# realtimeradio/caltech-bifrost-dsp

Hardware: AMD Instinct MI355X
Metric: xengine_ingest_gbps_704in_96ch (higher is better)
Workload: dtype int8 (4+4-bit samples) -> int32

## Files before the change

caltech-bifrost-dsp_amd/csrc/ring.hip:

```cpp
#include <time.h>

#include <atomic>
#include <chrono>
#include <condition_variable>
#include <deque>
#include <map>
#include <memory>
#include <mutex>
#include <string>
#include <vector>

#include "xeng_common.h"

namespace xeng {

struct RingCore;

struct Buf {
    std::atomic<long> refs{1};
    void* ptr = nullptr;
    size_t nbytes = 0;
    int space = XENG_SPACE_SYSTEM;
    int dev = -1;
    bool owned = true;
    RingCore* ring = nullptr;
    Stamp stamp;
    unsigned long long hook_stamp[2] = {0, 0};
};

struct Chunk {
    uint64_t offset;
    size_t nbytes;
    Buf* buf;
    size_t boff;
};

struct Seq {
    long long index = 0, time_tag = 0;
    int nringlet = 1;
    std::string header;
    std::deque<Chunk> chunks;
    uint64_t committed = 0;
    bool ended = false;
};

struct Reader {
    bool open = false, guarantee = true, in_seq = false;
    long long seq_index = 0;
    uint64_t offset = 0;
};

struct RingCore {
    std::atomic<long> refs{1};
    std::mutex mu;
    std::condition_variable cv;
    std::string name;
    int space = XENG_SPACE_SYSTEM;
    std::deque<std::unique_ptr<Seq>> seqs;
    long long seq_base = 0;
    long long nseq = 0;
    Seq* open_seq = nullptr;
    bool writing_ended = false, destroyed = false;
    std::vector<Reader> readers;
    size_t capacity = 0, live_bytes = 0;
    std::mutex pool_mu;
    std::map<size_t, std::deque<Buf*>> pool;
    std::vector<Buf*> graveyard;
    size_t pool_bytes = 0;
    xengRingStampNowFn hook_now = nullptr;
    xengRingStampDoneFn hook_done = nullptr;
    xengRingStampWaitFn hook_wait = nullptr;
    void* hook_user = nullptr;
    bool recycle_system = false;
    unsigned stream_mask = 0;
    std::atomic<unsigned> declared{0}, users{0};
    bool writer_seen = false;
    std::atomic<size_t> owned_bytes{0};
    std::atomic<unsigned long long> n_alloc{0}, n_free{0}, n_reuse{0}, n_stamp_wait{0}, n_skipped{0};
};

static void ring_unref(RingCore* r) {
    if (r->refs.fetch_sub(1) == 1) delete r;
}

static size_t own_limit(const RingCore* r, size_t nbytes) { return 8 * std::max(r->capacity, 2 * nbytes); }

static bool pooled_space(const RingCore* r) { return r->space != XENG_SPACE_SYSTEM || r->hook_now || r->recycle_system; }

static int raw_alloc(int space, size_t nbytes, void** out) {
    const size_t n = nbytes ? nbytes : 1;
    if (space == XENG_SPACE_SYSTEM) {
        void* p = nullptr;
        if (posix_memalign(&p, 64, (n + 63) & ~(size_t)63) != 0 || !p) XENG_FAIL(XENG_STATUS_MEM_ALLOC_FAILED, "ring: out of host memory (%zu bytes)", n);
        memset(p, 0, n);
        *out = p;
        return XENG_STATUS_SUCCESS;
    }
    int rc = xengMalloc(out, n, space);
    if (rc) return rc;
    rc = xengMemset(*out, 0, n);
    if (rc) { (void)xengFree(*out, space); *out = nullptr; }
    return rc;
}

static void raw_free(int space, void* p) {
    if (!p) return;
    if (space == XENG_SPACE_SYSTEM) free(p);
    else (void)xengFree(p, space);
}

static unsigned effective_mask(const RingCore* r) {
    const unsigned m = r->stream_mask;
    if (!m || r->declared.load() < r->users.load()) return (unsigned)STAMP_ALL;
    return m;
}

static void buf_stamp(Buf* b) {
    RingCore* r = b->ring;
    if (r->hook_now) r->hook_now(r->hook_user, b->hook_stamp);
    else if (b->space != XENG_SPACE_SYSTEM) {
        (void)stamp_now(&b->stamp, b->ptr, effective_mask(r), b->dev);
    }
}

static void buf_poll(Buf* b, bool* done, bool* waitable) {
    RingCore* r = b->ring;
    *done = true;
    *waitable = true;
    if (r->hook_done) {
        *done = r->hook_done(r->hook_user, b->hook_stamp) != 0;
        return;
    }
    if (b->space == XENG_SPACE_SYSTEM) return;
    if (stamp_poll(b->stamp, done, waitable) != XENG_STATUS_SUCCESS) { *done = false; *waitable = false; }
}

static int buf_wait(Buf* b) {
    RingCore* r = b->ring;
    r->n_stamp_wait++;
    if (r->hook_wait) { r->hook_wait(r->hook_user, b->hook_stamp); return XENG_STATUS_SUCCESS; }
    if (b->space == XENG_SPACE_SYSTEM) return XENG_STATUS_SUCCESS;
    return stamp_wait(b->stamp);
}

static void buf_destroy(Buf* b, bool may_wait) {
    RingCore* r = b->ring;
    if (b->owned && b->ptr) {
        bool done = true, waitable = true;
        buf_poll(b, &done, &waitable);
        if (!done && may_wait && waitable) done = buf_wait(b) == XENG_STATUS_SUCCESS;
        if (done) {
            raw_free(b->space, b->ptr);
            r->n_free++;
        }
        r->owned_bytes -= b->nbytes;
    }
    delete b;
    ring_unref(r);
}

static void buf_release(Buf* b) {
    if (b->refs.fetch_sub(1) != 1) return;
    RingCore* r = b->ring;
    if (!b->owned) { delete b; ring_unref(r); return; }
    if (!pooled_space(r)) { raw_free(b->space, b->ptr); r->n_free++; r->owned_bytes -= b->nbytes; delete b; ring_unref(r); return; }
    buf_stamp(b);
    {
        std::lock_guard<std::mutex> lk(r->pool_mu);
        if (!r->destroyed) {
            if (r->owned_bytes.load() > own_limit(r, b->nbytes)) {
                r->graveyard.push_back(b);
            } else {
                r->pool[b->nbytes].push_back(b);
                r->pool_bytes += b->nbytes;
            }
            return;
        }
    }
    buf_destroy(b, true);
}

static void bury(RingCore* r) {
    std::vector<Buf*> dead;
    {
        std::lock_guard<std::mutex> lk(r->pool_mu);
        dead.swap(r->graveyard);
    }
    for (Buf* b : dead) buf_destroy(b, true);
}

static int buf_obtain(RingCore* r, size_t nbytes, int may_block, Buf** out) {
    *out = nullptr;
    if (pooled_space(r)) {
        Buf* cand = nullptr;
        {
            std::lock_guard<std::mutex> lk(r->pool_mu);
            auto it = r->pool.find(nbytes);
            if (it != r->pool.end() && !it->second.empty()) {
                cand = it->second.front();
                it->second.pop_front();
                r->pool_bytes -= nbytes;
            }
        }
        if (cand) {
            bool done, waitable;
            buf_poll(cand, &done, &waitable);
            const bool grow = !done && r->owned_bytes.load() + nbytes <= own_limit(r, nbytes) && !r->hook_now;
            if (!done && waitable && may_block && !grow) done = buf_wait(cand) == XENG_STATUS_SUCCESS;
            if (done) {
                *out = cand;
            } else {
                std::lock_guard<std::mutex> lk(r->pool_mu);
                if (waitable) r->pool[nbytes].push_front(cand);
                else r->pool[nbytes].push_back(cand);
                r->pool_bytes += nbytes;
                if (waitable && !may_block && !grow) return XENG_STATUS_WOULD_BLOCK;
            }
        }
        if (*out) {
            (*out)->refs.store(1);
            r->n_reuse++;
            return XENG_STATUS_SUCCESS;
        }
    }
    if (!may_block && (r->space != XENG_SPACE_SYSTEM || nbytes > (1u << 20))) return XENG_STATUS_WOULD_BLOCK;
    void* p = nullptr;
    int rc = raw_alloc(r->space, nbytes, &p);
    if (rc) return rc;
    Buf* b = new Buf();
    b->ptr = p; b->nbytes = nbytes; b->space = r->space; b->ring = r;
    if (r->space != XENG_SPACE_SYSTEM && hipGetDevice(&b->dev) != hipSuccess) { (void)hipGetLastError(); b->dev = -1; }
    r->refs.fetch_add(1);
    r->n_alloc++;
    r->owned_bytes += nbytes;
    *out = b;
    return XENG_STATUS_SUCCESS;
}

static Seq* seq_at(RingCore* r, long long index) {
    if (index < r->seq_base || index >= r->seq_base + (long long)r->seqs.size()) return nullptr;
    return r->seqs[(size_t)(index - r->seq_base)].get();
}

static void drop_chunk(RingCore* r, Seq* s, std::vector<Buf*>* released) {
    Chunk c = s->chunks.front();
    s->chunks.pop_front();
    r->live_bytes -= c.nbytes;
    released->push_back(c.buf);
}

static void gc(RingCore* r, std::vector<Buf*>* released) {
    bool any = false;
    long long lo_seq = 0;
    uint64_t lo_off = 0;
    for (const Reader& rd : r->readers) {
        if (!rd.open) continue;
        if (!any || rd.seq_index < lo_seq || (rd.seq_index == lo_seq && rd.offset < lo_off)) { lo_seq = rd.seq_index; lo_off = rd.offset; }
        any = true;
    }
    if (!any) return;
    while (!r->seqs.empty() && r->seq_base < lo_seq) {
        Seq* s = r->seqs.front().get();
        while (!s->chunks.empty()) drop_chunk(r, s, released);
        if (s == r->open_seq) break;
        r->seqs.pop_front();
        r->seq_base++;
    }
    if (Seq* s = seq_at(r, lo_seq))
        while (!s->chunks.empty() && s->chunks.front().offset + s->chunks.front().nbytes <= lo_off) drop_chunk(r, s, released);
}

static bool drop_oldest(RingCore* r, std::vector<Buf*>* released) {
    for (auto& sp : r->seqs)
        if (!sp->chunks.empty()) { drop_chunk(r, sp.get(), released); return true; }
    r->live_bytes = 0;
    return false;
}

static void release_all(std::vector<Buf*>& v) {
    for (Buf* b : v) buf_release(b);
    v.clear();
}

static int wait_for_room(RingCore* r, std::unique_lock<std::mutex>& lk, size_t nbytes, int nonblocking, int may_block) {
    if (r->capacity == 0) r->capacity = 4 * nbytes;
    std::vector<Buf*> released;
    for (;;) {
        const size_t cap = std::max(r->capacity, nbytes);
        if (r->live_bytes + nbytes <= cap) break;
        gc(r, &released);
        if (r->live_bytes + nbytes <= cap) break;
        bool guaranteed = false;
        for (const Reader& rd : r->readers) guaranteed |= rd.open && rd.guarantee;
        if (!guaranteed) {
            if (!drop_oldest(r, &released)) break;
            continue;
        }
        if (nonblocking || !may_block || r->destroyed) {
            lk.unlock(); release_all(released); lk.lock();
            if (r->destroyed) XENG_FAIL(XENG_STATUS_INVALID_STATE, "ring '%s' was destroyed", r->name.c_str());
            if (nonblocking) XENG_FAIL(XENG_STATUS_WOULD_BLOCK, "ring '%s' full", r->name.c_str());
            return XENG_STATUS_WOULD_BLOCK;
        }
        if (!released.empty()) { lk.unlock(); release_all(released); lk.lock(); continue; }
        r->cv.wait_for(lk, std::chrono::milliseconds(100));
    }
    if (!released.empty()) { lk.unlock(); release_all(released); lk.lock(); }
    return XENG_STATUS_SUCCESS;
}

static int copy_bytes(int space, void* dst, const void* src, size_t n) {
    if (space == XENG_SPACE_SYSTEM) { memcpy(dst, src, n); return XENG_STATUS_SUCCESS; }
    return xengMemcpy(dst, src, n);
}

}

using namespace xeng;

#define RING_ARG(r_) \
    RingCore* r = (RingCore*)(r_); \
    if (!r) XENG_FAIL(XENG_STATUS_INVALID_ARGUMENT, "ring: null handle")

extern "C" {

int xengRingCreate(xengRing** ring, const char* name, int space) {
    if (!ring) XENG_FAIL(XENG_STATUS_INVALID_ARGUMENT, "RingCreate: null handle pointer");
    if (space != XENG_SPACE_SYSTEM && space != XENG_SPACE_CUDA && space != XENG_SPACE_CUDA_HOST)
        XENG_FAIL(XENG_STATUS_INVALID_ARGUMENT, "RingCreate: unknown space %d", space);
    RingCore* r = new RingCore();
    r->name = name ? name : "";
    r->space = space;
    *ring = (xengRing*)r;
    return XENG_STATUS_SUCCESS;
}

int xengRingDestroy(xengRing* ring) {
    RING_ARG(ring);
    std::vector<Buf*> released;
    {
        std::unique_lock<std::mutex> lk(r->mu);
        if (r->destroyed) return XENG_STATUS_SUCCESS;
        r->destroyed = true;
        r->writing_ended = true;
        for (auto& sp : r->seqs) {
            sp->ended = true;
            while (!sp->chunks.empty()) drop_chunk(r, sp.get(), &released);
        }
        r->open_seq = nullptr;
        r->cv.notify_all();
    }
    release_all(released);
    std::vector<Buf*> dead;
    {
        std::lock_guard<std::mutex> lk(r->pool_mu);
        for (auto& kv : r->pool)
            for (Buf* b : kv.second) dead.push_back(b);
        r->pool.clear();
        r->pool_bytes = 0;
        for (Buf* b : r->graveyard) dead.push_back(b);
        r->graveyard.clear();
    }
    for (Buf* b : dead) buf_destroy(b, true);
    ring_unref(r);
    return XENG_STATUS_SUCCESS;
}

int xengRingSetStampHooks(xengRing* ring, xengRingStampNowFn now, xengRingStampDoneFn done, xengRingStampWaitFn wait, void* user) {
    RING_ARG(ring);
    std::lock_guard<std::mutex> lk(r->pool_mu);
    r->hook_now = now; r->hook_done = done; r->hook_wait = wait; r->hook_user = user;
    return XENG_STATUS_SUCCESS;
}

int xengRingDeclareStreams(xengRing* ring, unsigned classes) {
    RING_ARG(ring);
    std::lock_guard<std::mutex> lk(r->pool_mu);
    r->stream_mask |= classes & (STAMP_ALL | STAMP_XGPU_OUT);
    r->declared.fetch_add(1);
    return XENG_STATUS_SUCCESS;
}

int xengRingGetStampClasses(xengRing* ring, unsigned* classes, unsigned* declared, unsigned* users) {
    RING_ARG(ring);
    if (classes) *classes = effective_mask(r);
    if (declared) *declared = r->declared.load();
    if (users) *users = r->users.load();
    return XENG_STATUS_SUCCESS;
}

int xengRingSetRecycle(xengRing* ring, int on) {
    RING_ARG(ring);
    std::lock_guard<std::mutex> lk(r->pool_mu);
    r->recycle_system = on != 0;
    return XENG_STATUS_SUCCESS;
}

int xengRingResize(xengRing* ring, size_t contig_bytes, size_t total_span) {
    RING_ARG(ring);
    const size_t want = total_span ? total_span : 4 * contig_bytes;
    std::lock_guard<std::mutex> lk(r->mu);
    r->capacity = std::max(r->capacity, std::max(want, contig_bytes));
    return XENG_STATUS_SUCCESS;
}

int xengRingGetInfo(xengRing* ring, size_t* capacity, size_t* live_bytes, size_t* pool_bytes, int* nreaders, long long* nseq,
                    unsigned long long counters[5]) {
    RING_ARG(ring);
    {
        std::lock_guard<std::mutex> lk(r->mu);
        if (capacity) *capacity = r->capacity;
        if (live_bytes) *live_bytes = r->live_bytes;
        if (nreaders) {
            int n = 0;
            for (const Reader& rd : r->readers) n += rd.open;
            *nreaders = n;
        }
        if (nseq) *nseq = r->nseq;
    }
    if (pool_bytes) {
        std::lock_guard<std::mutex> lk(r->pool_mu);
        *pool_bytes = r->pool_bytes;
    }
    if (counters) {
        counters[0] = r->n_alloc; counters[1] = r->n_free; counters[2] = r->n_reuse; counters[3] = r->n_stamp_wait; counters[4] = r->n_skipped;
    }
    return XENG_STATUS_SUCCESS;
}

int xengRingBeginSequence(xengRing* ring, long long time_tag, const void* header, size_t header_len, int nringlet, long long* seq) {
    RING_ARG(ring);
    if (!seq) XENG_FAIL(XENG_STATUS_INVALID_ARGUMENT, "BeginSequence: null seq");
    std::lock_guard<std::mutex> lk(r->mu);
    if (r->destroyed) XENG_FAIL(XENG_STATUS_INVALID_STATE, "ring '%s' was destroyed", r->name.c_str());
    if (r->open_seq) r->open_seq->ended = true;
    if (!r->writer_seen) { r->writer_seen = true; r->users.fetch_add(1); }
    std::unique_ptr<Seq> s(new Seq());
    s->index = r->nseq++;
    s->time_tag = time_tag;
    s->nringlet = nringlet;
    if (header && header_len) s->header.assign((const char*)header, header_len);
    r->open_seq = s.get();
    *seq = s->index;
    if (r->seqs.empty()) r->seq_base = s->index;
    r->seqs.push_back(std::move(s));
    r->cv.notify_all();
    return XENG_STATUS_SUCCESS;
}

int xengRingEndSequence(xengRing* ring, long long seq) {
    RING_ARG(ring);
    std::lock_guard<std::mutex> lk(r->mu);
    if (Seq* s = seq_at(r, seq)) {
        s->ended = true;
        if (r->open_seq == s) r->open_seq = nullptr;
    }
    r->cv.notify_all();
    return XENG_STATUS_SUCCESS;
}

int xengRingEndWriting(xengRing* ring) {
    RING_ARG(ring);
    std::lock_guard<std::mutex> lk(r->mu);
    if (r->open_seq) { r->open_seq->ended = true; r->open_seq = nullptr; }
    r->writing_ended = true;
    r->cv.notify_all();
    return XENG_STATUS_SUCCESS;
}

int xengRingReserve(xengRing* ring, long long seq, size_t nbytes, int nonblocking, int may_block, void** data, long long* span) {
    RING_ARG(ring);
    if (!data || !span) XENG_FAIL(XENG_STATUS_INVALID_ARGUMENT, "Reserve: null output");
    if (may_block) bury(r);
    {
        std::unique_lock<std::mutex> lk(r->mu);
        Seq* s = seq < 0 ? r->open_seq : seq_at(r, seq);
        if (!s || s->ended) XENG_FAIL(XENG_STATUS_INVALID_STATE, "WriteSpan: no open sequence on ring '%s'", r->name.c_str());
        int rc = wait_for_room(r, lk, nbytes, nonblocking, may_block);
        if (rc) return rc;
    }
    Buf* b = nullptr;
    int rc = buf_obtain(r, nbytes, may_block, &b);
    if (rc) return rc;
    *data = b->ptr;
    *span = (long long)(intptr_t)b;
    return XENG_STATUS_SUCCESS;
}

int xengRingCommit(xengRing* ring, long long seq, long long span, size_t nbytes) {
    RING_ARG(ring);
    Buf* b = (Buf*)(intptr_t)span;
    if (!b || b->ring != r) XENG_FAIL(XENG_STATUS_INVALID_ARGUMENT, "Commit: not a span of ring '%s'", r->name.c_str());
    if (nbytes > b->nbytes) XENG_FAIL(XENG_STATUS_INVALID_ARGUMENT, "Commit: %zu bytes of a %zu-byte span", nbytes, b->nbytes);
    if (nbytes == 0) return XENG_STATUS_SUCCESS;
    std::lock_guard<std::mutex> lk(r->mu);
    Seq* s = seq < 0 ? r->open_seq : seq_at(r, seq);
    if (!s) return XENG_STATUS_SUCCESS;
    b->refs.fetch_add(1);
    s->chunks.push_back(Chunk{s->committed, nbytes, b, 0});
    s->committed += nbytes;
    r->live_bytes += nbytes;
    r->cv.notify_all();
    return XENG_STATUS_SUCCESS;
}

int xengRingCommitExternal(xengRing* ring, long long seq, void* data, size_t nbytes, int may_block) {
    RING_ARG(ring);
    if (!data || nbytes == 0) XENG_FAIL(XENG_STATUS_INVALID_ARGUMENT, "CommitExternal: empty span");
    std::unique_lock<std::mutex> lk(r->mu);
    Seq* s = seq < 0 ? r->open_seq : seq_at(r, seq);
    if (!s || s->ended) XENG_FAIL(XENG_STATUS_INVALID_STATE, "commit_external: no open sequence on ring '%s'", r->name.c_str());
    int rc = wait_for_room(r, lk, nbytes, 0, may_block);
    if (rc) return rc;
    s = seq < 0 ? r->open_seq : seq_at(r, seq);
    if (!s) XENG_FAIL(XENG_STATUS_INVALID_STATE, "commit_external: the sequence is gone (ring '%s')", r->name.c_str());
    Buf* b = new Buf();
    b->ptr = data; b->nbytes = nbytes; b->space = r->space; b->owned = false; b->ring = r;
    r->refs.fetch_add(1);
    s->chunks.push_back(Chunk{s->committed, nbytes, b, 0});
    s->committed += nbytes;
    r->live_bytes += nbytes;
    r->cv.notify_all();
    return XENG_STATUS_SUCCESS;
}

int xengRingOpenReader(xengRing* ring, int guarantee, int* reader) {
    RING_ARG(ring);
    if (!reader) XENG_FAIL(XENG_STATUS_INVALID_ARGUMENT, "OpenReader: null reader");
    std::lock_guard<std::mutex> lk(r->mu);
    size_t k = 0;
    while (k < r->readers.size() && r->readers[k].open) k++;
    if (k == r->readers.size()) r->readers.emplace_back();
    Reader& rd = r->readers[k];
    rd = Reader();
    rd.open = true;
    r->users.fetch_add(1);
    rd.guarantee = guarantee != 0;
    rd.seq_index = r->nseq;
    for (auto& sp : r->seqs)
        if (!sp->chunks.empty() || !sp->ended) { rd.seq_index = sp->index; break; }
    *reader = (int)k;
    return XENG_STATUS_SUCCESS;
}

int xengRingCloseReader(xengRing* ring, int reader) {
    RING_ARG(ring);
    std::vector<Buf*> released;
    {
        std::lock_guard<std::mutex> lk(r->mu);
        if (reader < 0 || reader >= (int)r->readers.size()) XENG_FAIL(XENG_STATUS_INVALID_ARGUMENT, "CloseReader: bad reader %d", reader);
        r->readers[reader].open = false;
        gc(r, &released);
        r->cv.notify_all();
    }
    release_all(released);
    return XENG_STATUS_SUCCESS;
}

int xengRingNextSequence(xengRing* ring, int reader, int may_block, long long* seq, long long* time_tag, int* nringlet,
                         const void** header, size_t* header_len) {
    RING_ARG(ring);
    std::vector<Buf*> released;
    int rc = XENG_STATUS_SUCCESS;
    {
        std::unique_lock<std::mutex> lk(r->mu);
        if (reader < 0 || reader >= (int)r->readers.size() || !r->readers[reader].open)
            XENG_FAIL(XENG_STATUS_INVALID_ARGUMENT, "NextSequence: bad reader %d", reader);
        Reader* rd = &r->readers[reader];
        if (rd->in_seq) {
            rd->in_seq = false;
            rd->seq_index++;
            rd->offset = 0;
            gc(r, &released);
            r->cv.notify_all();
        }
        for (;;) {
            rd = &r->readers[reader];
            if (rd->seq_index < r->seq_base) rd->seq_index = r->seq_base;
            if (rd->seq_index < r->nseq) break;
            if (r->writing_ended || r->destroyed) { rc = XENG_STATUS_END_OF_DATA; break; }
            if (!may_block) { rc = XENG_STATUS_WOULD_BLOCK; break; }
            r->cv.wait_for(lk, std::chrono::milliseconds(100));
        }
        if (rc == XENG_STATUS_SUCCESS) {
            Seq* s = seq_at(r, rd->seq_index);
            rd->in_seq = true;
            rd->offset = 0;
            if (seq) *seq = s->index;
            if (time_tag) *time_tag = s->time_tag;
            if (nringlet) *nringlet = s->nringlet;
            if (header) *header = s->header.data();
            if (header_len) *header_len = s->header.size();
        }
    }
    release_all(released);
    return rc;
}

static int acquire_common(xengRing* ring, int reader, size_t advance, size_t gulp_nbytes, int may_block, int max_parts, void** data,
                          size_t* nbytes, long long* span, int* nparts, size_t* skipped) {
    RING_ARG(ring);
    if (!data || !nbytes || !span || gulp_nbytes == 0) XENG_FAIL(XENG_STATUS_INVALID_ARGUMENT, "Acquire: bad argument");
    std::vector<Buf*> released;
    std::vector<Chunk> pieces;
    int rc = XENG_STATUS_SUCCESS;
    size_t n = 0, skip_total = 0;
    {
        std::unique_lock<std::mutex> lk(r->mu);
        if (reader < 0 || reader >= (int)r->readers.size() || !r->readers[reader].open || !r->readers[reader].in_seq)
            XENG_FAIL(XENG_STATUS_INVALID_ARGUMENT, "Acquire: reader %d has no open sequence", reader);
        if (advance) {
            r->readers[reader].offset += advance;
            gc(r, &released);
            r->cv.notify_all();
        }
        for (;;) {
            Reader& rd = r->readers[reader];
            Seq* s = seq_at(r, rd.seq_index);
            if (!s) { rc = XENG_STATUS_END_OF_DATA; break; }
            const uint64_t lo = s->chunks.empty() ? s->committed : s->chunks.front().offset;
            if (rd.offset < lo) {
                const uint64_t sk = ((lo - rd.offset + gulp_nbytes - 1) / gulp_nbytes) * gulp_nbytes;
                rd.offset += sk;
                skip_total += sk;
                r->n_skipped += sk;
            }
            const uint64_t avail = s->committed > rd.offset ? s->committed - rd.offset : 0;
            if (avail >= gulp_nbytes || s->ended || r->destroyed) {
                n = (size_t)std::min<uint64_t>(avail, gulp_nbytes);
                if (n == 0) { rc = XENG_STATUS_END_OF_DATA; break; }
                for (const Chunk& c : s->chunks) {
                    if (c.offset >= rd.offset + n) break;
                    const uint64_t a = std::max<uint64_t>(rd.offset, c.offset), b = std::min<uint64_t>(rd.offset + n, c.offset + c.nbytes);
                    if (a < b) {
                        c.buf->refs.fetch_add(1);
                        pieces.push_back(Chunk{a, (size_t)(b - a), c.buf, c.boff + (size_t)(a - c.offset)});
                    }
                }
                break;
            }
            if (!may_block) { rc = XENG_STATUS_WOULD_BLOCK; break; }
            r->cv.wait_for(lk, std::chrono::milliseconds(100));
        }
    }
    release_all(released);
    if (skipped) *skipped = skip_total;
    if (rc) return rc;
    if ((int)pieces.size() <= max_parts) {
        for (size_t k = 0; k < pieces.size(); k++) {
            data[k] = (uint8_t*)pieces[k].buf->ptr + pieces[k].boff;
            nbytes[k] = pieces[k].nbytes;
            span[k] = (long long)(intptr_t)pieces[k].buf;
        }
        if (nparts) *nparts = (int)pieces.size();
        return XENG_STATUS_SUCCESS;
    }
    if (!may_block) {
        for (Chunk& c : pieces) buf_release(c.buf);
        return XENG_STATUS_WOULD_BLOCK;
    }
    *nbytes = n;
    if (nparts) *nparts = 1;
    Buf* g = nullptr;
    rc = buf_obtain(r, n, 1, &g);
    size_t pos = 0;
    for (Chunk& c : pieces) {
        if (!rc) rc = copy_bytes(r->space, (uint8_t*)g->ptr + pos, (const uint8_t*)c.buf->ptr + c.boff, c.nbytes);
        pos += c.nbytes;
        buf_release(c.buf);
    }
    if (rc) { if (g) buf_release(g); return rc; }
    *data = g->ptr;
    *span = (long long)(intptr_t)g;
    return XENG_STATUS_SUCCESS;
}

int xengRingAcquire(xengRing* ring, int reader, size_t advance, size_t gulp_nbytes, int may_block, void** data, size_t* nbytes,
                    long long* span, size_t* skipped) {
    return acquire_common(ring, reader, advance, gulp_nbytes, may_block, 1, data, nbytes, span, nullptr, skipped);
}

int xengRingAcquireParts(xengRing* ring, int reader, size_t advance, size_t gulp_nbytes, int may_block, void* data[2], size_t nbytes[2],
                         long long span[2], int* nparts, size_t* skipped) {
    if (!nparts) XENG_FAIL(XENG_STATUS_INVALID_ARGUMENT, "AcquireParts: null nparts");
    return acquire_common(ring, reader, advance, gulp_nbytes, may_block, 2, data, nbytes, span, nparts, skipped);
}

int xengRingSpanRelease(long long span) {
    Buf* b = (Buf*)(intptr_t)span;
    if (!b) XENG_FAIL(XENG_STATUS_INVALID_ARGUMENT, "SpanRelease: null span");
    buf_release(b);
    return XENG_STATUS_SUCCESS;
}

}
```

caltech-bifrost-dsp_amd/csrc/xcorr.hip:

```cpp
#include <algorithm>
#include <cstdlib>
#include <map>
#include <mutex>
#include <vector>

#include "xcorr_kernels.h"
#include "slab.h"
#include "xeng_common.h"

namespace xeng {

struct XgpuConfig {
    int nstand = 352, npol = 2, nchan = 96, ntime_gulp = 480, max_gulps = 0;
};

struct XgpuContext {
    bool live = false;
    int gpu = 0;
    XgpuConfig cfg;
    int ncu = 256;
    int ninput = 0, nblk64 = 0, gkt = 0, cap_kt = 0, cap_gulps = 0, kt_stage = 1;
    int ct_pitch = 0;
    bool raw = false;
    bool kloop16 = false;
    FragGroup* fgroups_dev = nullptr;
    int nfg = 0;
    WorkList work;
    WorkList work_pairs;
    size_t gulp_bytes = 0;
    const uint8_t* gulp_ptr[XC_MAX_GULPS] = {};
    int64_t per_chan = 0, matlen = 0;
    uint8_t* stash[2] = {nullptr, nullptr};
    size_t stash_bytes = 0;
    int cur = 0;
    WgDesc* descs_dev = nullptr;
    int nwg = 0;
    hipStream_t stream = nullptr;
    static constexpr int NMM = 8;
    hipStream_t stream_mm2[NMM] = {};
    int nmm = 2;
    unsigned long long nlaunch = 0;
    hipStream_t stream_mm = nullptr;
    struct Writer { unsigned long long seq; int stream; };
    std::map<const void*, Writer> writers;
    static constexpr int NEV = 256;
    hipEvent_t ev_ring[NEV] = {};
    const void* ring_buf[NEV][2] = {};
    unsigned long long last_seq[NMM] = {};
    hipEvent_t ev_ct = nullptr;
    unsigned long long staging_seen = ~0ull;
    unsigned long long area_seq[2] = {0, 0};
    unsigned long long dump_seq[4] = {0, 0, 0, 0};
    unsigned long long ndump = 0;
    int nfilled = 0;
    bool acc_started = false;
    void* acc_out = nullptr;
    uint8_t* in_dev = nullptr;
    int32_t* out_dev = nullptr;
    unsigned long long* stamps = nullptr;
    GulpDesc* gdesc_dev[2] = {nullptr, nullptr};
    SlabArgs* gargs_dev[2] = {nullptr, nullptr};
    SlabSite slab_site;
    SlabIndexSite slab_index;
    SlabIndexJob slab_job;
    int slab_forced = 0;
    int slab_hint_seen = 0;
    int slab_recent_irr[8] = {}, slab_recent_n[8] = {}, slab_recent_pos = 0;
    unsigned long long slab_tables_until = 0;
    int slab_force_tables = -1;
    bool slab_mode = false;
    EventTimer timer;
};

static std::mutex g_mu;
static XgpuConfig g_cfg;
static XgpuContext g_ctx;
static unsigned long long g_epoch = 1;
static unsigned long long g_ctx_gen = 1;

static int destroy_locked() {
    XgpuContext& x = g_ctx;
    (void)hipSetDevice(x.gpu);
    if (x.stream) (void)hipStreamSynchronize(x.stream);
    for (int b = 0; b < XgpuContext::NMM; b++) {
        if (x.stream_mm2[b]) (void)hipStreamSynchronize(x.stream_mm2[b]);
    }
    for (int k = 0; k < XgpuContext::NEV; k++)
        if (x.ev_ring[k]) (void)hipEventDestroy(x.ev_ring[k]);
    for (int b = 0; b < 2; b++)
        if (x.stash[b]) (void)hipFree(x.stash[b]);
    if (x.ev_ct) (void)hipEventDestroy(x.ev_ct);
    if (x.descs_dev) (void)hipFree(x.descs_dev);
    if (x.fgroups_dev) (void)hipFree(x.fgroups_dev);
    if (x.work.dev) (void)hipFree(x.work.dev);
    if (x.work_pairs.dev) (void)hipFree(x.work_pairs.dev);
    if (x.in_dev) (void)hipFree(x.in_dev);
    if (x.stamps) (void)hipFree(x.stamps);
    if (x.out_dev) (void)hipFree(x.out_dev);
    for (int b = 0; b < 2; b++)
        if (x.gdesc_dev[b]) (void)hipFree(x.gdesc_dev[b]);
    for (int b = 0; b < 2; b++)
        if (x.gargs_dev[b]) (void)hipFree(x.gargs_dev[b]);
    slab_site_destroy(&x.slab_site);
    slab_index_site_destroy(&x.slab_index);
    x.timer.destroy();
    x = XgpuContext();
    g_epoch++;
    g_ctx_gen++;
    return XENG_STATUS_SUCCESS;
}

static void launch_xcorr(const XcorrParams& p, hipStream_t s, bool raw, int grid_size, bool kloop16) {
    if (raw) {
        const dim3 grid(grid_size);
        if (kloop16 && !p.acc2_mode && !(p.gdesc && p.by_table)) {
            if (p.gdesc) hipLaunchKernelGGL(HIP_KERNEL_NAME(xcorr_fused16_kernel<true>), grid, dim3(512), 0, s, p);
            else hipLaunchKernelGGL(HIP_KERNEL_NAME(xcorr_fused16_kernel<>), grid, dim3(512), 0, s, p);
            return;
        }
        if (p.gdesc && p.by_table) {
            if (p.acc2_mode) hipLaunchKernelGGL(HIP_KERNEL_NAME(xcorr_fused_kernel<true, true, true>), grid, dim3(256), 0, s, p);
            else hipLaunchKernelGGL(HIP_KERNEL_NAME(xcorr_fused_kernel<false, true, true>), grid, dim3(256), 0, s, p);
            return;
        }
        if (p.gdesc) {
            if (p.acc2_mode) hipLaunchKernelGGL(HIP_KERNEL_NAME(xcorr_fused_kernel<true, true>), grid, dim3(256), 0, s, p);
            else hipLaunchKernelGGL(HIP_KERNEL_NAME(xcorr_fused_kernel<false, true>), grid, dim3(256), 0, s, p);
            return;
        }
        if (p.acc2_mode) hipLaunchKernelGGL(HIP_KERNEL_NAME(xcorr_fused_kernel<true>), grid, dim3(256), 0, s, p);
        else hipLaunchKernelGGL(HIP_KERNEL_NAME(xcorr_fused_kernel<>), grid, dim3(256), 0, s, p);
        return;
    }
    hipLaunchKernelGGL(xcorr_mfma_kernel, dim3(p.nchan * p.nwg), dim3(256), 0, s, p);
}

static hipEvent_t launch_event(unsigned long long seq) {
    XgpuContext& x = g_ctx;
    if (seq == 0 || x.nlaunch - seq >= (unsigned long long)XgpuContext::NEV) return nullptr;
    return x.ev_ring[seq % XgpuContext::NEV];
}

static int order_after_writer(hipStream_t s, int self, const void* buf) {
    XgpuContext& x = g_ctx;
    auto it = x.writers.find(buf);
    if (it == x.writers.end() || it->second.stream == self) return XENG_STATUS_SUCCESS;
    if (hipEvent_t ev = launch_event(it->second.seq)) XENG_HIP(hipStreamWaitEvent(s, ev, 0));
    return XENG_STATUS_SUCCESS;
}

static int flush_locked(void* out, bool dump, void* acc = nullptr, int acc_mode = 0) {
    XgpuContext& x = g_ctx;
    if (x.nfilled == 0) return XENG_STATUS_SUCCESS;
    if (!dump) { acc = nullptr; acc_mode = 0; }
    if (x.acc_started && x.acc_out != out)
        XENG_FAIL(XENG_STATUS_INVALID_STATE,
                  "xgpu: output buffer changed inside one integration (partial sums live in %p, got %p)",
                  x.acc_out, out);
    int nkt = x.nfilled * x.gkt;
    const int rem = x.raw ? 0 : nkt % x.kt_stage;
    if (rem) {
        const int padk = x.kt_stage - rem;
        XENG_HIP(hipMemset2DAsync(x.stash[x.cur] + (size_t)nkt * KT_BYTES, (size_t)x.cap_kt * KT_BYTES, 0,
                                  (size_t)padk * KT_BYTES, (size_t)x.cfg.nchan * x.nblk64, x.stream));
        stream_tick(STREAM_XGPU);
        nkt += padk;
    }
    const bool slab_tables = x.slab_mode && x.slab_index.tab32 != nullptr;
    bool slab_by_table = false;
    if (slab_tables) {
        x.slab_job.ngulp = x.nfilled;
        {
            const int seen = *(volatile int*)x.slab_index.hint_host;
            x.slab_recent_irr[x.slab_recent_pos] = seen - x.slab_hint_seen;
            x.slab_recent_n[x.slab_recent_pos] = x.nfilled;
            x.slab_recent_pos = (x.slab_recent_pos + 1) & 7;
            x.slab_hint_seen = seen;
            int irr = 0, n = 0;
            for (int k = 0; k < 8; k++) { irr += x.slab_recent_irr[k]; n += x.slab_recent_n[k]; }
            if (4 * irr > n) x.slab_tables_until = x.nlaunch + 16;
            slab_by_table = x.slab_force_tables > 0 || (x.slab_force_tables < 0 && x.nlaunch < x.slab_tables_until);
        }
        if (int rcs = slab_index_enqueue(x.stream, x.slab_index, x.cur, x.slab_job, slab_by_table, x.gdesc_dev[x.cur], x.gargs_dev[x.cur])) return rcs;
        staging_stream_touched();
    } else if (x.slab_mode) {
        if (int rcs = slab_fallback_enqueue(x.stream, x.gdesc_dev[x.cur], x.gargs_dev[x.cur], x.nfilled)) return rcs;
        staging_stream_touched();
    }
    XcorrParams p;
    p.stash = x.stash[x.cur]; p.out = (int32_t*)out; p.descs = x.descs_dev;
    p.nwg = x.raw ? x.nfg : x.nwg; p.nchan = x.cfg.nchan; p.nblk64 = x.nblk64; p.cap_kt = x.cap_kt; p.nkt = nkt;
    p.nstand = x.cfg.nstand; p.per_chan = x.per_chan; p.matlen = x.matlen;
    p.accumulate = x.acc_started ? 1 : 0;
    p.stamps = x.stamps;
    p.spg = x.raw ? x.cfg.ntime_gulp / (XC_KT * 32) : 0;
    p.ninput = x.ninput;
    p.fgroups = x.fgroups_dev; p.work = x.work.dev; p.maxi = x.work.maxi; p.nstage = nkt / XC_KT;
    p.acc2 = (int32_t*)acc; p.acc2_mode = acc ? acc_mode : 0;
    p.gdesc = slab_tables ? x.gdesc_dev[x.cur] : nullptr;
    p.by_table = slab_by_table ? 1 : 0;
    if (slab_tables && !diag_env("XENG_SLAB_PLAIN_ORDER")) { p.work = x.work_pairs.dev; p.maxi = x.work_pairs.maxi; }
    for (int g = 0; g < XC_MAX_GULPS; g++) p.gulps[g] = g < x.nfilled ? x.gulp_ptr[g] : nullptr;
    const int si = (int)(x.nlaunch++ % x.nmm);
    hipStream_t smm = x.stream_mm2[si];
    if (const unsigned long long ops = staging_stream_ops(); ops != x.staging_seen) {
        XENG_HIP(hipEventRecord(x.ev_ct, x.stream));
        XENG_HIP(hipStreamWaitEvent(smm, x.ev_ct, 0));
        x.staging_seen = ops;
    }
    const unsigned long long seq = x.nlaunch;
    {
        const int k = (int)(seq % XgpuContext::NEV);
        if (seq > (unsigned long long)XgpuContext::NEV) {
            if (hipEventQuery(x.ev_ring[k]) != hipSuccess) {
                (void)hipGetLastError();
                XENG_HIP(hipEventSynchronize(x.ev_ring[k]));
            }
            for (const void* buf : x.ring_buf[k]) {
                auto it = buf ? x.writers.find(buf) : x.writers.end();
                if (it != x.writers.end() && it->second.seq == seq - XgpuContext::NEV) x.writers.erase(it);
            }
        }
        x.ring_buf[k][0] = out; x.ring_buf[k][1] = acc;
    }
    for (const void* buf : {(const void*)out, (const void*)acc}) {
        if (!buf) continue;
        int rc = order_after_writer(smm, si, buf);
        if (rc) return rc;
        x.writers[buf] = XgpuContext::Writer{seq, si};
    }
    int slot = x.timer.begin(smm, 1);
    launch_xcorr(p, smm, x.raw, fused_grid(x.cfg.nchan, x.nfg, x.ncu), x.kloop16);
    x.timer.end(smm, slot);
    XENG_HIP(hipGetLastError());
    XENG_HIP(hipEventRecord(x.ev_ring[seq % XgpuContext::NEV], smm));
    x.area_seq[x.cur] = seq;
    x.last_seq[si] = seq;
    if (dump) {
        x.dump_seq[x.ndump & 3] = seq;
        x.ndump++;
    }
    x.cur ^= 1;
    x.nfilled = 0;
    x.slab_mode = false;
    x.acc_started = !dump;
    x.acc_out = dump ? nullptr : out;
    return XENG_STATUS_SUCCESS;
}

struct PendingWait {
    int gpu = 0;
    hipStream_t staging = nullptr;
    hipEvent_t dump = nullptr;
};

static int wait_unlocked(const PendingWait& w) {
    XENG_HIP(hipSetDevice(w.gpu));
    if (w.staging) XENG_HIP(hipStreamSynchronize(w.staging));
    if (w.dump) XENG_HIP(hipEventSynchronize(w.dump));
    return XENG_STATUS_SUCCESS;
}

static int kernel_locked(const void* in_dev, void* out_dev, int doDump, bool sync, PendingWait* pw, void* acc = nullptr,
                         int acc_mode = 0) {
    XgpuContext& x = g_ctx;
    if (!x.live) XENG_FAIL(XENG_STATUS_INVALID_STATE, "xgpu: not initialized (call xengXgpuInitialize)");
    if (!in_dev || !out_dev) XENG_FAIL(XENG_STATUS_INVALID_ARGUMENT, "xgpu: null buffer");
    if (acc) {
        if (!x.raw)
            XENG_FAIL(XENG_STATUS_UNSUPPORTED, "xgpu: the fused long accumulation needs the default contraction kernel (use xengMapAddI32)");
        if (acc_mode != 1 && acc_mode != 2) XENG_FAIL(XENG_STATUS_INVALID_ARGUMENT, "xgpu: acc_mode must be 1 (assign) or 2 (add)");
        if (((uintptr_t)acc & 15) || acc == out_dev) XENG_FAIL(XENG_STATUS_INVALID_ARGUMENT, "xgpu: accumulator must be 16-byte aligned and distinct from out");
    }
    if (((uintptr_t)out_dev & 15) || ((uintptr_t)in_dev & (x.raw ? 15 : 3)))
        XENG_FAIL(XENG_STATUS_INVALID_ARGUMENT, "xgpu: out must be 16-byte and in %d-byte aligned", x.raw ? 16 : 4);
    XENG_HIP(hipSetDevice(x.gpu));
    if (x.nfilled > 0 && x.slab_mode)
        XENG_FAIL(XENG_STATUS_INVALID_STATE, "xgpu: packet slabs and plain gulps cannot be mixed between two flushes");
    if (x.nfilled == 0)
        if (hipEvent_t ev = launch_event(x.area_seq[x.cur])) XENG_HIP(hipStreamWaitEvent(x.stream, ev, 0));
    uint8_t* const stash = x.stash[x.cur];
    int slot = -1;
    if (x.raw) {
        if (sync && !doDump) {
            uint8_t* copy = stash + (size_t)x.nfilled * x.gulp_bytes;
            slot = x.timer.begin(x.stream, 0);
            if (x.gulp_bytes % 16 == 0) {
                const size_t n16 = x.gulp_bytes / 16;
                const unsigned blocks = (unsigned)std::min<size_t>(2048, (n16 + 1023) / 1024);
                hipLaunchKernelGGL(HIP_KERNEL_NAME(gulp_copy_kernel<4>), dim3(blocks), dim3(256), 0, x.stream, (v4i*)copy, (const v4i*)in_dev, n16);
                XENG_HIP(hipGetLastError());
            } else {
                XENG_HIP(hipMemcpyAsync(copy, in_dev, x.gulp_bytes, hipMemcpyDeviceToDevice, x.stream));
            }
            x.gulp_ptr[x.nfilled] = copy;
        } else {
            x.gulp_ptr[x.nfilled] = (const uint8_t*)in_dev;
        }
    } else if (x.ct_pitch > 0) {
        slot = x.timer.begin(x.stream, 0);
        const size_t l8 = (((size_t)16 * x.ct_pitch + 1023) & ~(size_t)1023);
        hipLaunchKernelGGL(corner_turn_tr8_kernel, dim3(x.cfg.nchan, x.gkt, 2), dim3(256), l8, x.stream,
                           (const uint8_t*)in_dev, stash, x.cfg.ntime_gulp, x.cfg.nchan, x.ninput, x.nblk64,
                           x.cap_kt, x.nfilled * x.gkt, x.ct_pitch);
    } else {
        slot = x.timer.begin(x.stream, 0);
        const int ct_items = 2 * x.nblk64 * 16;
        const int ct_threads = std::min(1024, ((ct_items + 63) / 64) * 64);
        hipLaunchKernelGGL(corner_turn_kernel, dim3(x.gkt, x.cfg.nchan), dim3(ct_threads), 0, x.stream,
                           (const uint8_t*)in_dev, stash, x.cfg.ntime_gulp, x.cfg.nchan, x.ninput, x.nblk64,
                           x.cap_kt, x.nfilled * x.gkt);
    }
    x.timer.end(x.stream, slot);
    XENG_HIP(hipGetLastError());
    if (!x.raw || (sync && !doDump)) staging_stream_touched();
    x.nfilled++;
    if (doDump || x.nfilled == x.cap_gulps) {
        int rc = flush_locked(out_dev, doDump != 0, acc, acc_mode);
        if (rc) return rc;
    } else if (x.acc_started && x.acc_out != out_dev) {
        XENG_FAIL(XENG_STATUS_INVALID_STATE, "xgpu: output buffer changed inside one integration");
    }
    if (sync && pw) {
        pw->gpu = x.gpu;
        pw->staging = x.stream;
        if (doDump) pw->dump = launch_event(x.dump_seq[(x.ndump - 1) & 3]);
    }
    return XENG_STATUS_SUCCESS;
}

void xgpu_pending_launch(unsigned long long* seq, unsigned long long* epoch, unsigned long long* nlaunch, unsigned long long* ctx) {
    std::lock_guard<std::mutex> lk(g_mu);
    XgpuContext& x = g_ctx;
    *seq = (x.live && x.nfilled > 0) ? x.nlaunch + 1 : 0;
    *epoch = g_epoch;
    *nlaunch = x.live ? x.nlaunch : 0;
    *ctx = g_ctx_gen;
}

unsigned long long xgpu_last_writer(const void* buf) {
    std::lock_guard<std::mutex> lk(g_mu);
    XgpuContext& x = g_ctx;
    if (!x.live || !buf) return 0;
    auto it = x.writers.find(buf);
    return it == x.writers.end() ? 0 : it->second.seq;
}

int xgpu_launches_poll(unsigned long long upto, unsigned long long ctx, bool* done, hipEvent_t* ev, bool exact) {
    std::lock_guard<std::mutex> lk(g_mu);
    XgpuContext& x = g_ctx;
    *done = true;
    if (ev) *ev = nullptr;
    if (upto == 0 || !x.live || ctx != g_ctx_gen) return XENG_STATUS_SUCCESS;
    for (int k = 0; k < (exact ? 1 : x.nmm) && (unsigned long long)k < upto; k++) {
        if (hipEvent_t e = launch_event(upto - k)) {
            const hipError_t q = hipEventQuery(e);
            if (q == hipErrorNotReady) {
                (void)hipGetLastError();
                *done = false;
                if (ev && !*ev) *ev = e;
            } else if (q != hipSuccess) {
                XENG_HIP(q);
            }
        }
    }
    return XENG_STATUS_SUCCESS;
}

int xgpu_pending_poll(unsigned long long seq, unsigned long long epoch, bool* done, bool* launched, hipEvent_t* ev, int* gpu) {
    std::lock_guard<std::mutex> lk(g_mu);
    XgpuContext& x = g_ctx;
    *done = true;
    *launched = true;
    if (ev) *ev = nullptr;
    if (seq == 0 || !x.live || epoch != g_epoch) return XENG_STATUS_SUCCESS;
    if (x.nlaunch < seq) {
        *done = false;
        *launched = false;
        return XENG_STATUS_SUCCESS;
    }
    if (hipEvent_t e = launch_event(seq)) {
        const hipError_t q = hipEventQuery(e);
        if (q == hipErrorNotReady) {
            (void)hipGetLastError();
            *done = false;
            if (ev) *ev = e;
            if (gpu) *gpu = x.gpu;
        } else if (q != hipSuccess) {
            XENG_HIP(q);
        }
    }
    return XENG_STATUS_SUCCESS;
}

}

using namespace xeng;

extern "C" {

int xengXgpuConfigure(int nstand, int npol, int nchan, int ntime_gulp, int max_gulps_per_flush) {
    if (npol != 2) XENG_FAIL(XENG_STATUS_UNSUPPORTED, "xgpu: npol must be 2 (got %d)", npol);
    if (nstand <= 0 || nstand % 4) XENG_FAIL(XENG_STATUS_INVALID_ARGUMENT, "xgpu: nstand must be a positive multiple of 4 (got %d)", nstand);
    if (nstand * npol > 255 * 64) XENG_FAIL(XENG_STATUS_UNSUPPORTED, "xgpu: too many inputs (%d)", nstand * npol);
    if (nchan <= 0 || ntime_gulp <= 0 || max_gulps_per_flush < 0)
        XENG_FAIL(XENG_STATUS_INVALID_ARGUMENT, "xgpu: bad sizes nchan=%d ntime_gulp=%d max_gulps=%d", nchan, ntime_gulp, max_gulps_per_flush);
    std::lock_guard<std::mutex> lk(g_mu);
    g_cfg.nstand = nstand; g_cfg.npol = npol; g_cfg.nchan = nchan; g_cfg.ntime_gulp = ntime_gulp;
    g_cfg.max_gulps = max_gulps_per_flush;
    return XENG_STATUS_SUCCESS;
}

static int initialize_locked(int gpu);

int xengXgpuInitialize(int gpu) {
    std::lock_guard<std::mutex> lk(g_mu);
    destroy_locked();
    const int rc = initialize_locked(gpu);
    if (rc) destroy_locked();
    return rc;
}

static int initialize_locked(int gpu) {
    XgpuContext& x = g_ctx;
    x.cfg = g_cfg;
    x.gpu = gpu < 0 ? 0 : gpu;
    XENG_HIP(hipSetDevice(x.gpu));
    {
        int ncu = 0;
        XENG_HIP(hipDeviceGetAttribute(&ncu, hipDeviceAttributeMultiprocessorCount, x.gpu));
        const char* e = diag_env("XENG_GRID");
        x.ncu = e ? atoi(e) : ncu;
        if (x.ncu < 1) x.ncu = 1;
    }
    x.ninput = x.cfg.nstand * x.cfg.npol;
    x.nblk64 = (x.ninput + 63) / 64;
    x.gkt = (x.cfg.ntime_gulp + 31) / 32;
    x.kt_stage = XC_KT;
    int cap = x.cfg.max_gulps > 0 ? x.cfg.max_gulps : std::max(1, 4800 / (x.gkt * 32));
    cap = std::min(cap, std::max(1, 65535 / (x.gkt * 32)));
    {
        const char* r = getenv("XENG_RAW");
        x.gulp_bytes = (size_t)x.cfg.ntime_gulp * x.cfg.nchan * x.ninput;
        x.raw = !(r && !strcmp(r, "0")) && x.ninput % 16 == 0 &&
                x.cfg.ntime_gulp % (XC_KT * 32) == 0 && x.gulp_bytes + (size_t)16 * x.cfg.nchan * x.ninput < (1ull << 32) &&
                (size_t)x.cfg.nchan * x.ninput >= 128;
        if (x.raw) cap = std::min(cap, XC_MAX_GULPS);
        const char* kl = getenv("XENG_KLOOP");
        x.kloop16 = x.raw && kl && !strcmp(kl, "16");
        const char* st = getenv("XENG_SLAB_TABLES");
        x.slab_force_tables = st ? (strcmp(st, "0") ? 1 : 0) : -1;
        x.slab_hint_seen = 0; x.slab_recent_pos = 0; x.slab_tables_until = 0;
        for (int k = 0; k < 8; k++) x.slab_recent_irr[k] = x.slab_recent_n[k] = 0;
    }
    x.cap_gulps = cap;
    x.cap_kt = ((cap * x.gkt + x.kt_stage - 1) / x.kt_stage) * x.kt_stage;
    x.per_chan = (int64_t)(x.cfg.nstand / 2 + 1) * (x.cfg.nstand / 4) * x.cfg.npol * x.cfg.npol * 4;
    x.matlen = x.per_chan * x.cfg.nchan;
    x.stash_bytes = (size_t)x.cfg.nchan * x.nblk64 * x.cap_kt * KT_BYTES;
    if (x.ninput % 16 == 0) {
        int pitch = x.ninput;
        while (((pitch / 4) & 63) != 8) pitch += 16;
        if ((size_t)16 * pitch + 1024 <= 64 * 1024) x.ct_pitch = pitch;
    }
    if (x.raw) x.stash_bytes = (size_t)cap * x.gulp_bytes;

    for (int b = 0; b < 2; b++) {
        XENG_HIP(hipMalloc((void**)&x.stash[b], x.stash_bytes));
        XENG_HIP(hip_memset_now(x.stash[b], 0, x.stash_bytes));
    }
    XENG_HIP(hipEventCreateWithFlags(&x.ev_ct, hipEventDisableTiming));
    if (x.raw) {
        for (int b = 0; b < 2; b++) {
            XENG_HIP(hipMalloc((void**)&x.gdesc_dev[b], XC_MAX_GULPS * sizeof(GulpDesc)));
            XENG_HIP(hip_memset_now(x.gdesc_dev[b], 0, XC_MAX_GULPS * sizeof(GulpDesc)));
            XENG_HIP(hipMalloc((void**)&x.gargs_dev[b], XC_MAX_GULPS * sizeof(SlabArgs)));
            XENG_HIP(hip_memset_now(x.gargs_dev[b], 0, XC_MAX_GULPS * sizeof(SlabArgs)));
        }
        if (int rcs = slab_site_create(&x.slab_site)) return rcs;
    }
    std::vector<WgDesc> descs = build_wg_descs(x.nblk64);
    x.nwg = (int)descs.size();
    if (x.raw) {
        const bool tiles64 = getenv("XENG_TILING") && !strcmp(getenv("XENG_TILING"), "64");
        const bool plain_order = diag_env("XENG_ITEM_ORDER") && !strcmp(diag_env("XENG_ITEM_ORDER"), "plain");
        const std::vector<FragGroup> groups = tiles64 ? frag_groups_from_tiles(x.nblk64) : build_frag_groups(x.nblk64);
        if (check_frag_groups(groups, x.nblk64) != -1) XENG_FAIL(XENG_STATUS_DEVICE_ERROR, "xgpu: the tiling of %d blocks is not an exact cover", x.nblk64);
        x.nfg = (int)groups.size();
        XENG_HIP(hipMalloc((void**)&x.fgroups_dev, groups.size() * sizeof(FragGroup)));
        XENG_HIP(hipMemcpy(x.fgroups_dev, groups.data(), groups.size() * sizeof(FragGroup), hipMemcpyHostToDevice));
        const std::vector<uint64_t> masks = group_block_masks(groups);
        x.work = build_work(fused_grid(x.cfg.nchan, x.nfg, x.ncu), x.cfg.nchan, x.nfg, plain_order ? nullptr : &masks);
        XENG_HIP(hipMalloc((void**)&x.work.dev, x.work.entries.size() * sizeof(WorkEntry)));
        XENG_HIP(hipMemcpy(x.work.dev, x.work.entries.data(), x.work.entries.size() * sizeof(WorkEntry), hipMemcpyHostToDevice));
        x.work_pairs = build_work(fused_grid(x.cfg.nchan, x.nfg, x.ncu), x.cfg.nchan, x.nfg, plain_order ? nullptr : &masks, true);
        XENG_HIP(hipMalloc((void**)&x.work_pairs.dev, x.work_pairs.entries.size() * sizeof(WorkEntry)));
        XENG_HIP(hipMemcpy(x.work_pairs.dev, x.work_pairs.entries.data(), x.work_pairs.entries.size() * sizeof(WorkEntry), hipMemcpyHostToDevice));
    }
    XENG_HIP(hipMalloc((void**)&x.descs_dev, descs.size() * sizeof(WgDesc)));
    XENG_HIP(hipMemcpy(x.descs_dev, descs.data(), descs.size() * sizeof(WgDesc), hipMemcpyHostToDevice));
    if (const char* o = diag_env("XENG_STREAM_ORDER")) {
        hipStream_t tmp;
        for (const char* c = o; *c; c++) {
            const StreamId id = *c == 'c' ? STREAM_COPY : *c == 'm' ? STREAM_MAP : *c == 'b' ? STREAM_BEAM : *c == 'k' ? STREAM_CONSUMER : STREAM_XGPU;
            int rc0 = get_stream(id, &tmp);
            if (rc0) return rc0;
        }
    }
    int rc = get_stream(STREAM_XGPU, &x.stream);
    if (rc) return rc;
    if (const char* e = diag_env("XENG_MM_STREAMS")) x.nmm = std::max(1, std::min(XgpuContext::NMM, atoi(e)));
    for (int t = 0; t < x.nmm; t++) {
        rc = get_stream(mm_stream_id(t), &x.stream_mm2[t]);
        if (rc) return rc;
    }
    for (int k = 0; k < XgpuContext::NEV; k++) XENG_HIP(hipEventCreateWithFlags(&x.ev_ring[k], hipEventDisableTiming));
    x.stream_mm = x.stream_mm2[0];
    if (diag_env("XENG_DBG_STAMPS")) {
        const int ng = std::max(x.nwg, x.nfg);
        XENG_HIP(hipMalloc((void**)&x.stamps, (size_t)x.cfg.nchan * ng * 4 * 8 * sizeof(unsigned long long)));
        XENG_HIP(hip_memset_now(x.stamps, 0, (size_t)x.cfg.nchan * ng * 4 * 8 * sizeof(unsigned long long)));
    }
    XENG_HIP(hipStreamSynchronize(nullptr));
    x.live = true;
    return XENG_STATUS_SUCCESS;
}

int xengXgpuDestroy(void) {
    std::lock_guard<std::mutex> lk(g_mu);
    return destroy_locked();
}

static void drain_timer() {
    std::lock_guard<std::mutex> lk(g_mu);
    if (g_ctx.live) g_ctx.timer.drain();
}

static int wait_for_event_slot(bool may_block = true) {
    for (;;) {
        hipEvent_t ev = nullptr;
        int gpu = 0;
        {
            std::lock_guard<std::mutex> lk(g_mu);
            XgpuContext& x = g_ctx;
            if (!x.live) return XENG_STATUS_SUCCESS;
            const unsigned long long next = x.nlaunch + 1;
            if (next <= (unsigned long long)XgpuContext::NEV) return XENG_STATUS_SUCCESS;
            ev = x.ev_ring[next % XgpuContext::NEV];
            gpu = x.gpu;
            if (hipEventQuery(ev) == hipSuccess) return XENG_STATUS_SUCCESS;
            (void)hipGetLastError();
        }
        if (!may_block) XENG_FAIL(XENG_STATUS_WOULD_BLOCK, "xgpu: %d launches in flight (xengXgpuWaitLaunchSlot, then retry)", XgpuContext::NEV);
        XENG_HIP(hipSetDevice(gpu));
        XENG_HIP(hipEventSynchronize(ev));
    }
}

int xengXgpuKernel(const void* in_dev, void* out_dev, int doDump) {
    PendingWait pw;
    int rc0 = wait_for_event_slot();
    if (rc0) return rc0;
    {
        std::lock_guard<std::mutex> lk(g_mu);
        int rc = kernel_locked(in_dev, out_dev, doDump, true, &pw);
        if (rc) return rc;
    }
    int rc = wait_unlocked(pw);
    if (rc) return rc;
    if (doDump) drain_timer();
    return XENG_STATUS_SUCCESS;
}

int xengXgpuKernelAsync(const void* in_dev, void* out_dev, int doDump) {
    int rc0 = wait_for_event_slot();
    if (rc0) return rc0;
    std::lock_guard<std::mutex> lk(g_mu);
    return kernel_locked(in_dev, out_dev, doDump, false, nullptr);
}

int xengXgpuKernelAsyncAcc(const void* in_dev, void* out_dev, int doDump, void* acc_dev, int acc_mode) {
    int rc0 = wait_for_event_slot();
    if (rc0) return rc0;
    std::lock_guard<std::mutex> lk(g_mu);
    return kernel_locked(in_dev, out_dev, doDump, false, nullptr, acc_dev, acc_dev ? acc_mode : 0);
}

int xengXgpuTryKernelAsyncAcc(const void* in_dev, void* out_dev, int doDump, void* acc_dev, int acc_mode) {
    int rc0 = wait_for_event_slot(false);
    if (rc0) return rc0;
    std::lock_guard<std::mutex> lk(g_mu);
    return kernel_locked(in_dev, out_dev, doDump, false, nullptr, acc_dev, acc_dev ? acc_mode : 0);
}

int xengXgpuWaitLaunchSlot(void) { return wait_for_event_slot(true); }

static int kernel_slab(const void* packets_dev, int npkt, size_t pkt_stride, uint64_t seq0, int chan0_pipeline, void* out_dev,
                       int doDump, void* acc_dev, int acc_mode, bool may_block) {
    int rc0 = wait_for_event_slot(may_block);
    if (rc0) return rc0;
    std::lock_guard<std::mutex> lk(g_mu);
    XgpuContext& x = g_ctx;
    if (!x.live) XENG_FAIL(XENG_STATUS_INVALID_STATE, "xgpu: not initialized (call xengXgpuInitialize)");
    if (!x.raw) XENG_FAIL(XENG_STATUS_UNSUPPORTED, "xgpu: packet slabs need the default contraction kernel (unpack with xengSnap2UnpackAsync instead)");
    if (!packets_dev || !out_dev || npkt < 0 || pkt_stride < 32 || pkt_stride > 0x7FFFFFFFu)
        XENG_FAIL(XENG_STATUS_INVALID_ARGUMENT, "xgpu: bad slab (npkt %d, stride %zu)", npkt, pkt_stride);
    if (acc_dev) {
        if (acc_mode != 1 && acc_mode != 2) XENG_FAIL(XENG_STATUS_INVALID_ARGUMENT, "xgpu: acc_mode must be 1 (assign) or 2 (add)");
        if (((uintptr_t)acc_dev & 15) || acc_dev == out_dev) XENG_FAIL(XENG_STATUS_INVALID_ARGUMENT, "xgpu: accumulator must be 16-byte aligned and distinct from out");
    }
    if ((uintptr_t)out_dev & 15) XENG_FAIL(XENG_STATUS_INVALID_ARGUMENT, "xgpu: out must be 16-byte aligned");
    if (x.nfilled > 0 && !x.slab_mode)
        XENG_FAIL(XENG_STATUS_INVALID_STATE, "xgpu: packet slabs and plain gulps cannot be mixed between two flushes");
    if (x.acc_started && x.acc_out != out_dev) XENG_FAIL(XENG_STATUS_INVALID_STATE, "xgpu: output buffer changed inside one integration");
    XENG_HIP(hipSetDevice(x.gpu));
    if (x.nfilled == 0)
        if (hipEvent_t ev = launch_event(x.area_seq[x.cur])) XENG_HIP(hipStreamWaitEvent(x.stream, ev, 0));
    const int k = x.nfilled;
    SlabArgs a;
    a.pkts = (const uint8_t*)packets_dev; a.npkt = npkt; a.stride = (uint32_t)pkt_stride; a.seq0 = seq0;
    a.ntime = x.cfg.ntime_gulp; a.chan0 = chan0_pipeline; a.nchan = x.cfg.nchan; a.ninput = x.ninput; a.nblk = x.ninput / 64;
    uint8_t* scratch = x.stash[x.cur] + (size_t)k * x.gulp_bytes;
    if (x.ninput % 64 == 0) {
        if (!x.slab_index.tab32)
            if (int rcs = slab_index_site_create(&x.slab_index, x.cfg.ntime_gulp, x.cfg.nchan, x.ninput)) return rcs;
        x.slab_job.a[k] = a; x.slab_job.scratch[k] = scratch; x.slab_job.force[k] = slab_indexable(a) ? 0 : 1;
        x.gulp_ptr[k] = nullptr;
    } else {
        const bool maybe = false;
        if (int rcs = slab_prepare_enqueue(x.stream, x.slab_site, &a, &maybe, 1, x.gdesc_dev[x.cur] + k, x.gargs_dev[x.cur] + k, &scratch, false)) return rcs;
        XENG_HIP(hipGetLastError());
        staging_stream_touched();
        x.slab_forced++;
        x.gulp_ptr[k] = scratch;
    }
    x.slab_mode = true;
    x.nfilled++;
    if (doDump || x.nfilled == x.cap_gulps) return flush_locked(out_dev, doDump != 0, acc_dev, acc_dev ? acc_mode : 0);
    return XENG_STATUS_SUCCESS;
}

int xengXgpuKernelAsyncSlab(const void* packets_dev, int npkt, size_t pkt_stride, uint64_t seq0, int chan0_pipeline, void* out_dev,
                            int doDump, void* acc_dev, int acc_mode) {
    return kernel_slab(packets_dev, npkt, pkt_stride, seq0, chan0_pipeline, out_dev, doDump, acc_dev, acc_mode, true);
}

int xengXgpuTryKernelAsyncSlab(const void* packets_dev, int npkt, size_t pkt_stride, uint64_t seq0, int chan0_pipeline, void* out_dev,
                               int doDump, void* acc_dev, int acc_mode) {
    return kernel_slab(packets_dev, npkt, pkt_stride, seq0, chan0_pipeline, out_dev, doDump, acc_dev, acc_mode, false);
}

static int slab_stats_locked(int* nscattered, int* nirregular) {
    XgpuContext& x = g_ctx;
    int ns = x.slab_forced, ni = 0;
    x.slab_forced = 0;
    if (x.slab_index.tab32) {
        XENG_HIP(hipSetDevice(x.gpu));
        stream_tick(STREAM_XGPU);
        int a = 0, b = 0;
        if (int rcs = slab_index_site_read(x.stream, x.slab_index, &a, &b)) return rcs;
        ns += a; ni += b;
    }
    if (nscattered) *nscattered = ns;
    if (nirregular) *nirregular = ni;
    return XENG_STATUS_SUCCESS;
}

int xengXgpuGetSlabFallbacks(int* nfallback) {
    std::lock_guard<std::mutex> lk(g_mu);
    XgpuContext& x = g_ctx;
    if (!x.live) XENG_FAIL(XENG_STATUS_INVALID_STATE, "xgpu: not initialized");
    if (!nfallback) XENG_FAIL(XENG_STATUS_INVALID_ARGUMENT, "GetSlabFallbacks: null pointer");
    *nfallback = 0;
    return slab_stats_locked(nfallback, nullptr);
}

int xengXgpuGetSlabStats(int* nscattered, int* nirregular) {
    std::lock_guard<std::mutex> lk(g_mu);
    XgpuContext& x = g_ctx;
    if (!x.live) XENG_FAIL(XENG_STATUS_INVALID_STATE, "xgpu: not initialized");
    if (!nscattered || !nirregular) XENG_FAIL(XENG_STATUS_INVALID_ARGUMENT, "GetSlabStats: null pointer");
    *nscattered = *nirregular = 0;
    return slab_stats_locked(nscattered, nirregular);
}

int xengXgpuSync(void) {
    int gpu, nmm;
    hipStream_t st, mm[XgpuContext::NMM];
    {
        std::lock_guard<std::mutex> lk(g_mu);
        XgpuContext& x = g_ctx;
        if (!x.live) XENG_FAIL(XENG_STATUS_INVALID_STATE, "xgpu: not initialized");
        gpu = x.gpu; nmm = x.nmm; st = x.stream;
        for (int t = 0; t < nmm; t++) mm[t] = x.stream_mm2[t];
    }
    XENG_HIP(hipSetDevice(gpu));
    XENG_HIP(hipStreamSynchronize(st));
    for (int t = 0; t < nmm; t++) XENG_HIP(hipStreamSynchronize(mm[t]));
    drain_timer();
    return XENG_STATUS_SUCCESS;
}

int xengXgpuSyncLag(int lag) {
    PendingWait pw;
    {
        std::lock_guard<std::mutex> lk(g_mu);
        XgpuContext& x = g_ctx;
        if (!x.live) XENG_FAIL(XENG_STATUS_INVALID_STATE, "xgpu: not initialized");
        if (lag < 0 || lag > 3) XENG_FAIL(XENG_STATUS_INVALID_ARGUMENT, "SyncLag: lag must be 0..3 (got %d)", lag);
        pw.gpu = x.gpu;
        if (x.ndump > (unsigned long long)lag) pw.dump = launch_event(x.dump_seq[(x.ndump - 1 - lag) & 3]);
    }
    int rc = wait_unlocked(pw);
    if (rc) return rc;
    drain_timer();
    return XENG_STATUS_SUCCESS;
}

int xengXgpuDumpDone(int lag, int* done) {
    std::lock_guard<std::mutex> lk(g_mu);
    XgpuContext& x = g_ctx;
    if (!x.live) XENG_FAIL(XENG_STATUS_INVALID_STATE, "xgpu: not initialized");
    if (!done || lag < 0 || lag > 3) XENG_FAIL(XENG_STATUS_INVALID_ARGUMENT, "DumpDone: lag must be 0..3 (got %d)", lag);
    *done = 1;
    if (x.ndump > (unsigned long long)lag)
        if (hipEvent_t ev = launch_event(x.dump_seq[(x.ndump - 1 - lag) & 3])) {
            XENG_HIP(hipSetDevice(x.gpu));
            const hipError_t e = hipEventQuery(ev);
            if (e != hipSuccess && e != hipErrorNotReady) XENG_HIP(e);
            if (e == hipErrorNotReady) (void)hipGetLastError();
            *done = e == hipSuccess;
        }
    if (*done) x.timer.drain();
    return XENG_STATUS_SUCCESS;
}

int xengXgpuReset(void) {
    int gpu, nmm;
    hipStream_t st, mm[XgpuContext::NMM];
    {
        std::lock_guard<std::mutex> lk(g_mu);
        XgpuContext& x = g_ctx;
        if (!x.live) XENG_FAIL(XENG_STATUS_INVALID_STATE, "xgpu: not initialized");
        x.nfilled = 0;
        x.slab_mode = false;
        x.acc_started = false;
        x.acc_out = nullptr;
        g_epoch++;
        gpu = x.gpu; nmm = x.nmm; st = x.stream;
        for (int t = 0; t < nmm; t++) mm[t] = x.stream_mm2[t];
    }
    XENG_HIP(hipSetDevice(gpu));
    XENG_HIP(hipStreamSynchronize(st));
    for (int t = 0; t < nmm; t++) XENG_HIP(hipStreamSynchronize(mm[t]));
    drain_timer();
    return XENG_STATUS_SUCCESS;
}

static std::mutex g_correlate_mu;
int xengXgpuCorrelate(const void* in_host, void* out_host, int doDump) {
    std::lock_guard<std::mutex> clk(g_correlate_mu);
    PendingWait pw;
    hipStream_t st;
    int32_t* out_dev;
    size_t out_bytes;
    {
        std::lock_guard<std::mutex> lk(g_mu);
        XgpuContext& x = g_ctx;
        if (!x.live) XENG_FAIL(XENG_STATUS_INVALID_STATE, "xgpu: not initialized");
        if (!in_host || !out_host) XENG_FAIL(XENG_STATUS_INVALID_ARGUMENT, "xgpu: null buffer");
        XENG_HIP(hipSetDevice(x.gpu));
        const size_t in_bytes = (size_t)x.cfg.ntime_gulp * x.cfg.nchan * x.ninput;
        out_bytes = (size_t)x.matlen * 2 * sizeof(int32_t);
        if (!x.in_dev) XENG_HIP(hipMalloc((void**)&x.in_dev, in_bytes));
        if (!x.out_dev) XENG_HIP(hipMalloc((void**)&x.out_dev, out_bytes));
        XENG_HIP(hipMemcpyAsync(x.in_dev, in_host, in_bytes, hipMemcpyHostToDevice, x.stream));
        staging_stream_touched();
        int rc = kernel_locked(x.in_dev, x.out_dev, doDump, true, &pw);
        if (rc) return rc;
        st = x.stream; out_dev = x.out_dev;
    }
    int rc = wait_unlocked(pw);
    if (rc) return rc;
    if (doDump) {
        XENG_HIP(hipMemcpyAsync(out_host, out_dev, out_bytes, hipMemcpyDeviceToHost, st));
        stream_tick(STREAM_XGPU);
        XENG_HIP(hipStreamSynchronize(st));
        drain_timer();
    }
    return XENG_STATUS_SUCCESS;
}

int xengXgpuGetOrder(const int32_t* antpol_to_input, int32_t* antpol_to_bl, int32_t* is_conj) {
    XgpuConfig cfg;
    {
        std::lock_guard<std::mutex> lk(g_mu);
        cfg = g_ctx.live ? g_ctx.cfg : g_cfg;
    }
    if (!antpol_to_input || !antpol_to_bl || !is_conj) XENG_FAIL(XENG_STATUS_INVALID_ARGUMENT, "GetOrder: null array");
    const int bad = get_order_host(antpol_to_input, antpol_to_bl, is_conj, cfg.nstand, cfg.npol);
    if (bad >= 0) XENG_FAIL(XENG_STATUS_INVALID_ARGUMENT, "GetOrder: input id %d out of range at [%d]", antpol_to_input[bad], bad);
    return XENG_STATUS_SUCCESS;
}

static std::mutex g_evpool_mu;
static std::vector<hipEvent_t> g_evpool;
static int take_event(hipEvent_t* ev) {
    {
        std::lock_guard<std::mutex> lk(g_evpool_mu);
        if (!g_evpool.empty()) { *ev = g_evpool.back(); g_evpool.pop_back(); return XENG_STATUS_SUCCESS; }
    }
    XENG_HIP(hipEventCreateWithFlags(ev, hipEventDisableTiming));
    return XENG_STATUS_SUCCESS;
}
static void give_event(hipEvent_t ev) {
    std::lock_guard<std::mutex> lk(g_evpool_mu);
    g_evpool.push_back(ev);
}
static int finish_consumer(hipEvent_t ev) {
    const hipError_t e = hipEventSynchronize(ev);
    give_event(ev);
    XENG_HIP(e);
    return XENG_STATUS_SUCCESS;
}

int xengXgpuSubSelect(const void* in_dev, void* out_dev, const int32_t* vismap_dev, const int32_t* conj_dev,
                      int nvis, int nchan_sum) {
    hipEvent_t ev;
    {
        std::lock_guard<std::mutex> lk(g_mu);
        XgpuContext& x = g_ctx;
        if (!x.live) XENG_FAIL(XENG_STATUS_INVALID_STATE, "xgpu: not initialized");
        if (!in_dev || !out_dev || !vismap_dev || !conj_dev) XENG_FAIL(XENG_STATUS_INVALID_ARGUMENT, "SubSelect: null buffer");
        if (nvis <= 0 || nchan_sum <= 0 || x.cfg.nchan % nchan_sum)
            XENG_FAIL(XENG_STATUS_INVALID_ARGUMENT, "SubSelect: nvis=%d nchan_sum=%d nchan=%d", nvis, nchan_sum, x.cfg.nchan);
        XENG_HIP(hipSetDevice(x.gpu));
        hipStream_t s;
        int rc = get_stream(STREAM_CONSUMER, &s);
        if (rc) return rc;
        rc = order_after_writer(s, -1, in_dev);
        if (rc) return rc;
        hipLaunchKernelGGL(subselect_kernel, dim3((nvis + 255) / 256, x.cfg.nchan / nchan_sum), dim3(256), 0, s,
                           (const int32_t*)in_dev, (int32_t*)out_dev, vismap_dev, conj_dev, nvis, nchan_sum,
                           x.per_chan, x.matlen);
        XENG_HIP(hipGetLastError());
        stream_tick(STREAM_CONSUMER);
        rc = take_event(&ev);
        if (rc) return rc;
        const hipError_t re = hipEventRecord(ev, s);
        if (re != hipSuccess) { give_event(ev); XENG_HIP(re); }
    }
    return finish_consumer(ev);
}

int xengXgpuPacketize(const void* in_dev, void* out_dev, const int32_t* antpol_to_bl_dev, const int32_t* is_conj_dev,
                      int fmt) {
    hipEvent_t ev;
    {
        std::lock_guard<std::mutex> lk(g_mu);
        XgpuContext& x = g_ctx;
        if (!x.live) XENG_FAIL(XENG_STATUS_INVALID_STATE, "xgpu: not initialized");
        if (!in_dev || !out_dev || !antpol_to_bl_dev || !is_conj_dev) XENG_FAIL(XENG_STATUS_INVALID_ARGUMENT, "Packetize: null buffer");
        if (fmt != 0 && fmt != 1) XENG_FAIL(XENG_STATUS_INVALID_ARGUMENT, "Packetize: fmt must be 0 ([pol][pol][chan][2]) or 1 ([chan][pol][pol][2])");
        if ((uintptr_t)out_dev & 7) XENG_FAIL(XENG_STATUS_INVALID_ARGUMENT, "Packetize: out must be 8-byte aligned");
        int pitch = x.cfg.nchan;
        while ((pitch & 31) != 1) pitch++;
        const size_t lds = (size_t)64 * pitch * sizeof(int2);
        if (lds > 160 * 1024) XENG_FAIL(XENG_STATUS_UNSUPPORTED, "Packetize: nchan=%d needs %zu B of LDS", x.cfg.nchan, lds);
        XENG_HIP(hipSetDevice(x.gpu));
        if (lds > 64 * 1024)
            XENG_HIP(hipFuncSetAttribute((const void*)packetize_kernel, hipFuncAttributeMaxDynamicSharedMemorySize, (int)lds));
        hipStream_t s;
        int rc = get_stream(STREAM_CONSUMER, &s);
        if (rc) return rc;
        rc = order_after_writer(s, -1, in_dev);
        if (rc) return rc;
        hipLaunchKernelGGL(packetize_kernel, dim3(x.cfg.nstand, (x.cfg.nstand + 15) / 16), dim3(256), lds, s,
                           (const int32_t*)in_dev, (int2*)out_dev, antpol_to_bl_dev, is_conj_dev, x.cfg.nstand, x.cfg.nchan,
                           x.per_chan, x.matlen, pitch, fmt);
        XENG_HIP(hipGetLastError());
        stream_tick(STREAM_CONSUMER);
        rc = take_event(&ev);
        if (rc) return rc;
        const hipError_t re = hipEventRecord(ev, s);
        if (re != hipSuccess) { give_event(ev); XENG_HIP(re); }
    }
    return finish_consumer(ev);
}

int xengXgpuReorder(const void* in_host, void* out_host, const int32_t* bl, const int32_t* conj) {
    XgpuConfig cfg;
    {
        std::lock_guard<std::mutex> lk(g_mu);
        cfg = g_ctx.live ? g_ctx.cfg : g_cfg;
    }
    if (!in_host || !out_host || !bl || !conj) XENG_FAIL(XENG_STATUS_INVALID_ARGUMENT, "Reorder: null buffer");
    const int64_t per_chan = (int64_t)(cfg.nstand / 2 + 1) * (cfg.nstand / 4) * cfg.npol * cfg.npol * 4;
    const int64_t matlen = per_chan * cfg.nchan;
    const size_t nbl = (size_t)cfg.nstand * cfg.nstand * cfg.npol * cfg.npol;
    const long bad = reorder_host((const int32_t*)in_host, (int32_t*)out_host, bl, conj, nbl, cfg.nchan, per_chan, matlen);
    if (bad >= 0) XENG_FAIL(XENG_STATUS_INVALID_ARGUMENT, "Reorder: baseline index %d out of range", bl[bad]);
    return XENG_STATUS_SUCCESS;
}

int xengXgpuGetInfo(int* nstand, int* npol, int* nchan, int* ntime_gulp, int64_t* matlen, int* max_gulps) {
    std::lock_guard<std::mutex> lk(g_mu);
    XgpuContext& x = g_ctx;
    if (!x.live) XENG_FAIL(XENG_STATUS_INVALID_STATE, "xgpu: not initialized");
    if (nstand) *nstand = x.cfg.nstand;
    if (npol) *npol = x.cfg.npol;
    if (nchan) *nchan = x.cfg.nchan;
    if (ntime_gulp) *ntime_gulp = x.cfg.ntime_gulp;
    if (matlen) *matlen = x.matlen;
    if (max_gulps) *max_gulps = x.cap_gulps;
    return XENG_STATUS_SUCCESS;
}

int xengXgpuGetPath(int* fused_corner_turn, int* fp6) {
    std::lock_guard<std::mutex> lk(g_mu);
    XgpuContext& x = g_ctx;
    if (!x.live) XENG_FAIL(XENG_STATUS_INVALID_STATE, "xgpu: not initialized");
    if (fused_corner_turn) *fused_corner_turn = x.raw ? 1 : 0;
    if (fp6) *fp6 = 0;
    return XENG_STATUS_SUCCESS;
}

int xengXgpuGetKernel(int* waves_per_group, int* mfma_k) {
    std::lock_guard<std::mutex> lk(g_mu);
    XgpuContext& x = g_ctx;
    if (!x.live) XENG_FAIL(XENG_STATUS_INVALID_STATE, "xgpu: not initialized");
    const bool k16 = x.raw && x.kloop16;
    if (waves_per_group) *waves_per_group = k16 ? 8 : 4;
    if (mfma_k) *mfma_k = k16 ? 64 : 32;
    return XENG_STATUS_SUCCESS;
}

int xengXgpuSetProfiling(int enable) {
    std::lock_guard<std::mutex> lk(g_mu);
    g_ctx.timer.enabled = enable != 0;
    return XENG_STATUS_SUCCESS;
}

int xengXgpuGetTimes(double ms[2], int count[2]) {
    std::lock_guard<std::mutex> lk(g_mu);
    XgpuContext& x = g_ctx;
    if (x.live && x.stream) {
        XENG_HIP(hipStreamSynchronize(x.stream));
        for (int t = 0; t < x.nmm; t++) XENG_HIP(hipStreamSynchronize(x.stream_mm2[t]));
        x.timer.drain();
    }
    for (int k = 0; k < 2; k++) {
        if (ms) ms[k] = x.timer.total_ms[k];
        if (count) count[k] = x.timer.count[k];
        x.timer.total_ms[k] = 0;
        x.timer.count[k] = 0;
    }
    return XENG_STATUS_SUCCESS;
}

int xengXgpuDebugReadStamps(unsigned long long* host, size_t nwords, int* nwaves) {
    std::lock_guard<std::mutex> lk(g_mu);
    XgpuContext& x = g_ctx;
    if (!x.live || !x.stamps) XENG_FAIL(XENG_STATUS_INVALID_STATE, "stamps not enabled");
    const int ng = x.raw ? x.nfg : x.nwg;
    const size_t n = (size_t)x.cfg.nchan * ng * 4 * 8;
    if (nwaves) *nwaves = x.cfg.nchan * ng * 4;
    for (int t = 0; t < x.nmm; t++) XENG_HIP(hipStreamSynchronize(x.stream_mm2[t]));
// ... 19 lines not shown
```

caltech-bifrost-dsp_amd/csrc/xeng_util.hip:

```cpp
#include <time.h>

#include <atomic>
#include <mutex>
#include <utility>

#include "xeng_common.h"

namespace xeng {

static thread_local char g_err[512] = "";

void set_error(const char* fmt, ...) {
    va_list ap;
    va_start(ap, fmt);
    vsnprintf(g_err, sizeof(g_err), fmt, ap);
    va_end(ap);
}

static constexpr int MAXDEV = 16;
static std::mutex g_stream_mu;
static hipStream_t g_streams[MAXDEV][STREAM_COUNT];
static bool g_stream_ok[MAXDEV][STREAM_COUNT];

static std::atomic<unsigned long long> g_staging_ops{0};
void staging_stream_touched() {
    g_staging_ops.fetch_add(1, std::memory_order_relaxed);
    stream_tick(STREAM_XGPU);
}
unsigned long long staging_stream_ops() { return g_staging_ops.load(std::memory_order_relaxed); }

int get_stream(StreamId which, hipStream_t* out) {
    int dev = 0;
    XENG_HIP(hipGetDevice(&dev));
    if (dev < 0 || dev >= MAXDEV) XENG_FAIL(XENG_STATUS_INVALID_ARGUMENT, "device %d out of range", dev);
    std::lock_guard<std::mutex> lk(g_stream_mu);
    if (!g_stream_ok[dev][which]) {
        int lo = 0, hi = 0;
        XENG_HIP(hipDeviceGetStreamPriorityRange(&lo, &hi));
        const bool high = which == STREAM_MAP || which == STREAM_BEAM || which == STREAM_CONSUMER || which == STREAM_COPY;
        XENG_HIP(hipStreamCreateWithPriority(&g_streams[dev][which], hipStreamNonBlocking, high ? hi : 0 < lo ? 0 : lo));
        g_stream_ok[dev][which] = true;
    }
    *out = g_streams[dev][which];
    return XENG_STATUS_SUCCESS;
}

struct StreamClock {
    std::atomic<unsigned long long> enq{0};
    std::mutex mu;
    unsigned long long done = 0;
    static constexpr int NMARK = 64;
    struct Mark { unsigned long long upto = 0; hipEvent_t ev = nullptr; bool pending = false; hipEvent_t own = nullptr; } marks[NMARK];
};
static StreamClock g_clock[MAXDEV][STREAM_COUNT];

struct DeviceGuard {
    int prev = -1, want;
    explicit DeviceGuard(int d) : want(d) {
        if (hipGetDevice(&prev) != hipSuccess) prev = -1;
        if (prev != want) (void)hipSetDevice(want);
    }
    ~DeviceGuard() {
        if (prev >= 0 && prev != want) (void)hipSetDevice(prev);
    }
};

void stream_tick(StreamId which) {
    int dev = 0;
    if (hipGetDevice(&dev) != hipSuccess || dev < 0 || dev >= MAXDEV) return;
    g_clock[dev][which].enq.fetch_add(1, std::memory_order_release);
}

void stream_clocks_forget(int dev, StreamId which) {
    if (dev < 0 || dev >= MAXDEV) return;
    StreamClock& c = g_clock[dev][which];
    std::lock_guard<std::mutex> lk(c.mu);
    c.done = c.enq.load(std::memory_order_acquire);
    for (auto& m : c.marks) m.pending = false;
}

unsigned long long stream_clock_now(StreamId which) {
    int dev = 0;
    if (hipGetDevice(&dev) != hipSuccess || dev < 0 || dev >= MAXDEV) return 0;
    return g_clock[dev][which].enq.load(std::memory_order_acquire);
}

void stream_clock_external_mark(StreamId which, hipEvent_t ev, unsigned long long upto) {
    int dev = 0;
    if (hipGetDevice(&dev) != hipSuccess || dev < 0 || dev >= MAXDEV) return;
    StreamClock& c = g_clock[dev][which];
    std::lock_guard<std::mutex> lk(c.mu);
    if (upto <= c.done) return;
    StreamClock::Mark* slot = nullptr;
    for (auto& m : c.marks) {
        if (m.pending && m.ev == ev) { slot = &m; break; }
        if (!m.pending && !slot) slot = &m;
    }
    if (!slot) {
        for (auto& m : c.marks)
            if (m.ev != m.own && (!slot || m.upto < slot->upto)) slot = &m;
        if (!slot) return;
    }
    slot->ev = ev;
    slot->upto = upto;
    slot->pending = true;
}

static int clock_poll(int dev, StreamId which, unsigned long long t, bool* done, hipEvent_t* wait_ev) {
    *done = true;
    if (wait_ev) *wait_ev = nullptr;
    if (t == 0) return XENG_STATUS_SUCCESS;
    StreamClock& c = g_clock[dev][which];
    std::lock_guard<std::mutex> lk(c.mu);
    if (t <= c.done) return XENG_STATUS_SUCCESS;
    StreamClock::Mark* cover = nullptr;
    StreamClock::Mark* free_slot = nullptr;
    StreamClock::Mark* oldest = nullptr;
    for (;;) {
        oldest = nullptr;
        for (auto& m : c.marks)
            if (m.pending && (!oldest || m.upto < oldest->upto)) oldest = &m;
        if (!oldest) break;
        const hipError_t e = hipEventQuery(oldest->ev);
        if (e == hipSuccess) {
            oldest->pending = false;
            if (oldest->upto > c.done) c.done = oldest->upto;
            continue;
        }
        if (e != hipErrorNotReady) XENG_HIP(e);
        (void)hipGetLastError();
        break;
    }
    for (auto& m : c.marks) {
        if (m.pending) {
            if (m.upto >= t && (!cover || m.upto < cover->upto)) cover = &m;
        } else if (!free_slot) {
            free_slot = &m;
        }
    }
    if (t <= c.done) return XENG_STATUS_SUCCESS;
    *done = false;
    if (!cover && free_slot) {
        hipStream_t s;
        {
            std::lock_guard<std::mutex> slk(g_stream_mu);
            if (!g_stream_ok[dev][which]) {
                *done = true;
                return XENG_STATUS_SUCCESS;
            }
            s = g_streams[dev][which];
        }
        DeviceGuard g(dev);
        const unsigned long long upto = c.enq.load(std::memory_order_acquire);
        if (!free_slot->own) XENG_HIP(hipEventCreateWithFlags(&free_slot->own, hipEventDisableTiming));
        free_slot->ev = free_slot->own;
        XENG_HIP(hipEventRecord(free_slot->ev, s));
        free_slot->upto = upto;
        free_slot->pending = true;
        cover = free_slot;
        if (hipEventQuery(cover->ev) == hipSuccess) {
            cover->pending = false;
            if (upto > c.done) c.done = upto;
            *done = true;
            return XENG_STATUS_SUCCESS;
        }
        (void)hipGetLastError();
    }
    if (wait_ev) *wait_ev = cover ? cover->ev : (oldest ? oldest->ev : nullptr);
    return XENG_STATUS_SUCCESS;
}

static unsigned class_of(int stream) {
    switch (stream) {
        case STREAM_XGPU: return STAMP_XGPU;
        case STREAM_MAP: return STAMP_MAP;
        case STREAM_BEAM: return STAMP_BEAM;
        case STREAM_COPY: return STAMP_COPY;
        case STREAM_CONSUMER: return STAMP_CONSUMER;
        default: return 0;
    }
}

int stamp_now(Stamp* s, const void* buf, unsigned mask, int of_dev) {
    *s = Stamp();
    s->mask = mask;
    int dev = of_dev;
    if (dev < 0 && hipGetDevice(&dev) != hipSuccess) {
        (void)hipGetLastError();
        return XENG_STATUS_SUCCESS;
    }
    if (dev < 0 || dev >= MAXDEV) return XENG_STATUS_SUCCESS;
    s->dev = dev;
    for (int k = 0; k < STREAM_COUNT; k++) s->clk[k] = g_clock[dev][k].enq.load(std::memory_order_acquire);
    xgpu_pending_launch(&s->xgpu_seq, &s->xgpu_epoch, &s->xgpu_launch, &s->xgpu_ctx);
    if ((mask & STAMP_XGPU_OUT) && !(mask & STAMP_XGPU) && buf) {
        s->xgpu_launch = xgpu_last_writer(buf);
        s->xgpu_exact = true;
        s->xgpu_seq = 0;
    }
    return XENG_STATUS_SUCCESS;
}

static int stamp_pass(const Stamp& s, bool* done, bool* waitable, hipEvent_t* wait_ev) {
    *done = true;
    if (waitable) *waitable = true;
    if (wait_ev) *wait_ev = nullptr;
    if (s.dev < 0) return XENG_STATUS_SUCCESS;
    for (int k = 0; k < STREAM_COUNT; k++) {
        if (!(class_of(k) & s.mask)) continue;
        bool d = true;
        hipEvent_t ev = nullptr;
        int rc = clock_poll(s.dev, (StreamId)k, s.clk[k], &d, wait_ev ? &ev : nullptr);
        if (rc) return rc;
        if (!d) {
            *done = false;
            if (wait_ev && !*wait_ev) *wait_ev = ev;
        }
    }
    if (s.mask & (STAMP_XGPU | STAMP_XGPU_OUT)) {
        bool d = true;
        hipEvent_t ev = nullptr;
        int rc = xgpu_launches_poll(s.xgpu_launch, s.xgpu_ctx, &d, &ev, s.xgpu_exact);
        if (rc) return rc;
        if (!d) {
            *done = false;
            if (wait_ev && !*wait_ev) *wait_ev = ev;
        }
        if (s.xgpu_seq) {
            bool launched = true;
            ev = nullptr;
            rc = xgpu_pending_poll(s.xgpu_seq, s.xgpu_epoch, &d, &launched, &ev, nullptr);
            if (rc) return rc;
            if (!d) {
                *done = false;
                if (wait_ev && !*wait_ev) *wait_ev = ev;
            }
            if (!launched && waitable) *waitable = false;
        }
    }
    return XENG_STATUS_SUCCESS;
}

int stamp_poll(const Stamp& s, bool* done, bool* waitable) { return stamp_pass(s, done, waitable, nullptr); }

int stamp_wait(const Stamp& s) {
    for (int spins = 0;; spins++) {
        bool done = true, waitable = true;
        hipEvent_t ev = nullptr;
        int rc = stamp_pass(s, &done, &waitable, &ev);
        if (rc) return rc;
        if (done) return XENG_STATUS_SUCCESS;
        if (ev) {
            XENG_HIP(hipEventSynchronize(ev));
            continue;
        }
        if (!waitable && spins > 40000) XENG_FAIL(XENG_STATUS_INVALID_STATE, "stamp: waiting for an X-engine launch that was never enqueued");
        struct timespec ts = {0, 50000};
        nanosleep(&ts, nullptr);
    }
}

int sync_all_streams() {
    int dev = 0;
    XENG_HIP(hipGetDevice(&dev));
    for (int s = 0; s < STREAM_COUNT; s++) {
        hipStream_t st;
        bool ok;
        {
            std::lock_guard<std::mutex> lk(g_stream_mu);
            ok = g_stream_ok[dev][s];
            st = g_streams[dev][s];
        }
        if (ok) XENG_HIP(hipStreamSynchronize(st));
    }
    return XENG_STATUS_SUCCESS;
}

int EventTimer::begin(hipStream_t s, int k) {
    if (!enabled || npend >= MAXPEND) return -1;
    if (npend >= ncreated) {
        if (hipEventCreate(&start[ncreated]) != hipSuccess) return -1;
        if (hipEventCreate(&stop[ncreated]) != hipSuccess) return -1;
        ncreated++;
    }
    int slot = npend++;
    kind[slot] = k;
    (void)hipEventRecord(start[slot], s);
    return slot;
}
void EventTimer::end(hipStream_t s, int slot) {
    if (slot >= 0) (void)hipEventRecord(stop[slot], s);
}
int EventTimer::drain() {
    int keep = 0;
    for (int i = 0; i < npend; i++) {
        float ms = 0;
        if (hipEventQuery(stop[i]) == hipSuccess && hipEventElapsedTime(&ms, start[i], stop[i]) == hipSuccess) {
            total_ms[kind[i]] += ms;
            count[kind[i]]++;
        } else {
            if (keep != i) {
                std::swap(start[keep], start[i]);
                std::swap(stop[keep], stop[i]);
                std::swap(kind[keep], kind[i]);
            }
            keep++;
        }
    }
    npend = keep;
    (void)hipGetLastError();
    return 0;
}
void EventTimer::destroy() {
    for (int i = 0; i < ncreated; i++) {
        (void)hipEventDestroy(start[i]);
        (void)hipEventDestroy(stop[i]);
    }
    ncreated = npend = 0;
}

int TicketRing::mark(hipStream_t s, StreamId which, unsigned long long* ticket) {
    hipEvent_t& e = ev[n % NMARK];
    if (!e) XENG_HIP(hipEventCreateWithFlags(&e, hipEventDisableTiming));
    const unsigned long long upto = stream_clock_now(which);
    XENG_HIP(hipEventRecord(e, s));
    stream_clock_external_mark(which, e, upto);
    *ticket = ++n;
    return XENG_STATUS_SUCCESS;
}

int TicketRing::query(hipEvent_t e, int* done) {
    const hipError_t r = hipEventQuery(e);
    if (r != hipSuccess && r != hipErrorNotReady) XENG_HIP(r);
    if (r == hipErrorNotReady) (void)hipGetLastError();
    *done = r == hipSuccess;
    return XENG_STATUS_SUCCESS;
}

void TicketRing::destroy() {
    for (int k = 0; k < NMARK; k++)
        if (ev[k]) (void)hipEventDestroy(ev[k]);
}

int beam_context_open(BeamStreamContext& c, int gpu) {
    c.gpu = gpu < 0 ? 0 : gpu;
    XENG_HIP(hipSetDevice(c.gpu));
    return get_stream(STREAM_BEAM, &c.stream);
}

void beam_context_close(BeamStreamContext& c) {
    (void)hipSetDevice(c.gpu);
    if (c.stream) (void)hipStreamSynchronize(c.stream);
    stream_clocks_forget(c.gpu, STREAM_BEAM);
    c.tickets.destroy();
}

int beam_context_mark(std::mutex& mu, BeamStreamContext& c, const char* who, unsigned long long* ticket) {
    if (!ticket) XENG_FAIL(XENG_STATUS_INVALID_ARGUMENT, "%sMark: null ticket", who);
    std::lock_guard<std::mutex> lk(mu);
    if (!c.live) XENG_FAIL(XENG_STATUS_INVALID_STATE, "%s: not initialized", who);
    XENG_HIP(hipSetDevice(c.gpu));
    return c.tickets.mark(c.stream, STREAM_BEAM, ticket);
}

int beam_context_wait(std::mutex& mu, const BeamStreamContext& c, const char* who, unsigned long long ticket) {
    hipEvent_t ev = nullptr;
    int gpu = 0;
    {
        std::lock_guard<std::mutex> lk(mu);
        if (!c.live) XENG_FAIL(XENG_STATUS_INVALID_STATE, "%s: not initialized", who);
        if (!(ev = c.tickets.find(ticket))) XENG_FAIL(XENG_STATUS_INVALID_ARGUMENT, "%sWait: unknown ticket %llu", who, ticket);
        gpu = c.gpu;
    }
    XENG_HIP(hipSetDevice(gpu));
    XENG_HIP(hipEventSynchronize(ev));
    return XENG_STATUS_SUCCESS;
}

int beam_context_ticket_done(std::mutex& mu, const BeamStreamContext& c, const char* who, unsigned long long ticket, int* done) {
    if (!done) XENG_FAIL(XENG_STATUS_INVALID_ARGUMENT, "%sTicketDone: null result", who);
    std::lock_guard<std::mutex> lk(mu);
    if (!c.live) XENG_FAIL(XENG_STATUS_INVALID_STATE, "%s: not initialized", who);
    const hipEvent_t ev = c.tickets.find(ticket);
    if (!ev) XENG_FAIL(XENG_STATUS_INVALID_ARGUMENT, "%sTicketDone: unknown ticket %llu", who, ticket);
    XENG_HIP(hipSetDevice(c.gpu));
    return TicketRing::query(ev, done);
}

int beam_context_sync(std::mutex& mu, const BeamStreamContext& c, const char* who) {
    std::lock_guard<std::mutex> lk(mu);
    if (!c.live) XENG_FAIL(XENG_STATUS_INVALID_STATE, "%s: not initialized", who);
    XENG_HIP(hipSetDevice(c.gpu));
    XENG_HIP(hipStreamSynchronize(c.stream));
    return XENG_STATUS_SUCCESS;
}

}

using namespace xeng;

extern "C" {

const char* xengGetLastError(void) { return g_err; }
const char* xengVersion(void) { return "xeng-mi355x 0.1 (gfx950)"; }

int xengGetDeviceCount(int* count) {
    if (!count) XENG_FAIL(XENG_STATUS_INVALID_ARGUMENT, "null count");
    XENG_HIP(hipGetDeviceCount(count));
    return XENG_STATUS_SUCCESS;
}
int xengSetDevice(int gpu) {
    XENG_HIP(hipSetDevice(gpu));
    return XENG_STATUS_SUCCESS;
}
int xengGetDevice(int* gpu) {
    if (!gpu) XENG_FAIL(XENG_STATUS_INVALID_ARGUMENT, "null gpu");
    XENG_HIP(hipGetDevice(gpu));
    return XENG_STATUS_SUCCESS;
}
int xengDeviceSynchronize(void) {
    XENG_HIP(hipDeviceSynchronize());
    return XENG_STATUS_SUCCESS;
}
int xengGetDeviceInfo(int gpu, int* num_cu, int* clock_khz, size_t* total_mem, char* name, int name_len) {
    hipDeviceProp_t p;
    XENG_HIP(hipGetDeviceProperties(&p, gpu));
    if (num_cu) *num_cu = p.multiProcessorCount;
    if (clock_khz) *clock_khz = p.clockRate;
    if (total_mem) *total_mem = p.totalGlobalMem;
    if (name && name_len > 0) {
        snprintf(name, name_len, "%s (%s)", p.name, p.gcnArchName);
    }
    return XENG_STATUS_SUCCESS;
}
int xengGetDevicePciBusId(int gpu, char* bus_id, int len) {
    if (!bus_id || len < 16) XENG_FAIL(XENG_STATUS_INVALID_ARGUMENT, "bus id buffer of at least 16 bytes needed");
    XENG_HIP(hipDeviceGetPCIBusId(bus_id, len, gpu));
    return XENG_STATUS_SUCCESS;
}
int xengMalloc(void** ptr, size_t nbytes, int space) {
    if (!ptr) XENG_FAIL(XENG_STATUS_INVALID_ARGUMENT, "null ptr");
    if (space == XENG_SPACE_CUDA) {
        XENG_HIP(hipMalloc(ptr, nbytes ? nbytes : 1));
    } else if (space == XENG_SPACE_CUDA_HOST) {
        XENG_HIP(hipHostMalloc(ptr, nbytes ? nbytes : 1, hipHostMallocDefault));
    } else {
        XENG_FAIL(XENG_STATUS_INVALID_ARGUMENT, "xengMalloc: space %d is not device or pinned host", space);
    }
    return XENG_STATUS_SUCCESS;
}
int xengFree(void* ptr, int space) {
    if (!ptr) return XENG_STATUS_SUCCESS;
    if (space == XENG_SPACE_CUDA) {
        XENG_HIP(hipFree(ptr));
    } else if (space == XENG_SPACE_CUDA_HOST) {
        XENG_HIP(hipHostFree(ptr));
    } else {
        XENG_FAIL(XENG_STATUS_INVALID_ARGUMENT, "xengFree: bad space %d", space);
    }
    return XENG_STATUS_SUCCESS;
}
int xengMemcpy(void* dst, const void* src, size_t nbytes) {
    hipStream_t s;
    int rc = get_stream(STREAM_COPY, &s);
    if (rc) return rc;
    XENG_HIP(hipMemcpyAsync(dst, src, nbytes, hipMemcpyDefault, s));
    stream_tick(STREAM_COPY);
    XENG_HIP(hipStreamSynchronize(s));
    return XENG_STATUS_SUCCESS;
}
int xengMemcpyAsync(void* dst, const void* src, size_t nbytes) {
    hipStream_t s;
    int rc = get_stream(STREAM_COPY, &s);
    if (rc) return rc;
    XENG_HIP(hipMemcpyAsync(dst, src, nbytes, hipMemcpyDefault, s));
    stream_tick(STREAM_COPY);
    return XENG_STATUS_SUCCESS;
}
int xengMemset(void* dst, int value, size_t nbytes) {
    hipStream_t s;
    int rc = get_stream(STREAM_COPY, &s);
    if (rc) return rc;
    XENG_HIP(hipMemsetAsync(dst, value, nbytes, s));
    stream_tick(STREAM_COPY);
    XENG_HIP(hipStreamSynchronize(s));
    return XENG_STATUS_SUCCESS;
}
int xengStreamSynchronize(void) { return sync_all_streams(); }

static const int PACKED_STREAMS[5] = {STREAM_XGPU, STREAM_MAP, STREAM_BEAM, STREAM_COPY, STREAM_CONSUMER};
static void stamp_pack(const Stamp& s, xengStamp* o) {
    memset(o, 0, sizeof(*o));
    o->w[0] = (unsigned long long)(s.dev + 1) | ((unsigned long long)s.mask << 32);
    for (int k = 0; k < 5; k++) o->w[1 + k] = s.clk[PACKED_STREAMS[k]];
    o->w[6] = s.xgpu_seq; o->w[7] = s.xgpu_epoch; o->w[8] = s.xgpu_launch; o->w[9] = s.xgpu_ctx; o->w[10] = s.xgpu_exact ? 1 : 0;
}
static void stamp_unpack(const xengStamp* o, Stamp* s) {
    *s = Stamp();
    s->dev = (int)(o->w[0] & 0xFFFFFFFFull) - 1;
    s->mask = (unsigned)(o->w[0] >> 32) & (STAMP_ALL | STAMP_XGPU_OUT);
    s->xgpu_exact = o->w[10] != 0;
    for (int k = 0; k < 5; k++) s->clk[PACKED_STREAMS[k]] = o->w[1 + k];
    s->xgpu_seq = o->w[6]; s->xgpu_epoch = o->w[7]; s->xgpu_launch = o->w[8]; s->xgpu_ctx = o->w[9];
}

int xengStampNow(xengStamp* stamp) {
    if (!stamp) XENG_FAIL(XENG_STATUS_INVALID_ARGUMENT, "StampNow: null stamp");
    Stamp s;
    int rc = stamp_now(&s);
    if (rc) return rc;
    stamp_pack(s, stamp);
    return XENG_STATUS_SUCCESS;
}
int xengStampNowFor(xengStamp* stamp, const void* buf, unsigned classes) {
    if (!stamp) XENG_FAIL(XENG_STATUS_INVALID_ARGUMENT, "StampNowFor: null stamp");
    Stamp s;
    int rc = stamp_now(&s, buf, classes ? (classes & (STAMP_ALL | STAMP_XGPU_OUT)) : (unsigned)STAMP_ALL);
    if (rc) return rc;
    stamp_pack(s, stamp);
    return XENG_STATUS_SUCCESS;
}
int xengStampDone(const xengStamp* stamp, int* done, int* waitable) {
    if (!stamp || !done) XENG_FAIL(XENG_STATUS_INVALID_ARGUMENT, "StampDone: null argument");
    Stamp s;
    stamp_unpack(stamp, &s);
    if (s.dev >= MAXDEV) XENG_FAIL(XENG_STATUS_INVALID_ARGUMENT, "StampDone: not a stamp");
    bool d = true, w = true;
    int rc = stamp_poll(s, &d, &w);
    if (rc) return rc;
    *done = d;
    if (waitable) *waitable = w;
    return XENG_STATUS_SUCCESS;
}
int xengStampWait(const xengStamp* stamp) {
    if (!stamp) XENG_FAIL(XENG_STATUS_INVALID_ARGUMENT, "StampWait: null stamp");
    Stamp s;
    stamp_unpack(stamp, &s);
    if (s.dev >= MAXDEV) XENG_FAIL(XENG_STATUS_INVALID_ARGUMENT, "StampWait: not a stamp");
    return stamp_wait(s);
}

}
```

caltech-bifrost-dsp_amd/ffi.py:

```python
import ctypes
import os

import numpy as np

_HERE = os.path.dirname(os.path.abspath(__file__))
LIB_PATH = os.environ.get("XENG_LIB") or os.path.join(_HERE, "libxeng.so")

STATUS_SUCCESS = 0
SPACE_SYSTEM, SPACE_CUDA, SPACE_CUDA_HOST = 1, 2, 3

_lib = None


class XengError(RuntimeError):
    def __init__(self, fn, status, msg):
        super().__init__("%s returned %d: %s" % (fn, status, msg))
        self.status = status


class XENGarray(ctypes.Structure):
    _fields_ = [("data", ctypes.c_void_p), ("space", ctypes.c_int), ("dtype", ctypes.c_int),
                ("ndim", ctypes.c_int), ("shape", ctypes.c_long * 8), ("strides", ctypes.c_long * 8),
                ("immutable", ctypes.c_int), ("big_endian", ctypes.c_int), ("conjugated", ctypes.c_int)]


class XengStamp(ctypes.Structure):
    _fields_ = [("w", ctypes.c_ulonglong * 16)]


STATUS_WOULD_BLOCK, STATUS_END_OF_DATA = 6, 7
STREAMS = {"xgpu": 1, "map": 2, "beam": 4, "copy": 8, "consumer": 16, "xgpu_out": 32}
STAMP_NOW_FN = ctypes.CFUNCTYPE(None, ctypes.c_void_p, ctypes.POINTER(ctypes.c_ulonglong))
STAMP_DONE_FN = ctypes.CFUNCTYPE(ctypes.c_int, ctypes.c_void_p, ctypes.POINTER(ctypes.c_ulonglong))
STAMP_WAIT_FN = ctypes.CFUNCTYPE(None, ctypes.c_void_p, ctypes.POINTER(ctypes.c_ulonglong))

_vp, _i, _sz = ctypes.c_void_p, ctypes.c_int, ctypes.c_size_t
_pi = ctypes.POINTER(ctypes.c_int)
_pa = ctypes.POINTER(XENGarray)
_ll, _pll, _psz, _pvp = ctypes.c_longlong, ctypes.POINTER(ctypes.c_longlong), ctypes.POINTER(ctypes.c_size_t), ctypes.POINTER(ctypes.c_void_p)
_pst = ctypes.POINTER(XengStamp)
SYMBOLS = {
    "xengStampNow": [_pst], "xengStampNowFor": [_pst, _vp, ctypes.c_uint], "xengStampDone": [_pst, _pi, _pi], "xengStampWait": [_pst],
    "xengRingCreate": [_pvp, ctypes.c_char_p, _i], "xengRingDestroy": [_vp], "xengRingResize": [_vp, _sz, _sz], "xengRingSetRecycle": [_vp, _i], "xengRingDeclareStreams": [_vp, ctypes.c_uint], "xengRingGetStampClasses": [_vp, ctypes.POINTER(ctypes.c_uint), ctypes.POINTER(ctypes.c_uint), ctypes.POINTER(ctypes.c_uint)],
    "xengRingGetInfo": [_vp, _psz, _psz, _psz, _pi, _pll, ctypes.POINTER(ctypes.c_ulonglong)],
    "xengRingBeginSequence": [_vp, _ll, ctypes.c_char_p, _sz, _i, _pll], "xengRingEndSequence": [_vp, _ll], "xengRingEndWriting": [_vp],
    "xengRingReserve": [_vp, _ll, _sz, _i, _i, _pvp, _pll], "xengRingCommit": [_vp, _ll, _ll, _sz],
    "xengRingCommitExternal": [_vp, _ll, _vp, _sz, _i],
    "xengRingOpenReader": [_vp, _i, _pi], "xengRingCloseReader": [_vp, _i],
    "xengRingNextSequence": [_vp, _i, _i, _pll, _pll, _pi, _pvp, _psz],
    "xengRingAcquire": [_vp, _i, _sz, _sz, _i, _pvp, _psz, _pll, _psz], "xengRingSpanRelease": [_ll],
    "xengRingAcquireParts": [_vp, _i, _sz, _sz, _i, _pvp, _psz, _pll, _pi, _psz],
    "xengRingSetStampHooks": [_vp, STAMP_NOW_FN, STAMP_DONE_FN, STAMP_WAIT_FN, _vp],
    "xengGetDeviceCount": [_pi], "xengSetDevice": [_i], "xengGetDevice": [_pi], "xengDeviceSynchronize": [],
    "xengGetDeviceInfo": [_i, _pi, _pi, ctypes.POINTER(_sz), ctypes.c_char_p, _i], "xengGetDevicePciBusId": [_i, ctypes.c_char_p, _i],
    "xengMalloc": [ctypes.POINTER(_vp), _sz, _i], "xengFree": [_vp, _i], "xengMemcpy": [_vp, _vp, _sz],
    "xengMemcpyAsync": [_vp, _vp, _sz], "xengMemset": [_vp, _i, _sz], "xengStreamSynchronize": [],
    "xengXgpuConfigure": [_i, _i, _i, _i, _i], "xengXgpuInitialize": [_i], "xengXgpuDestroy": [],
    "xengXgpuKernel": [_vp, _vp, _i], "xengXgpuKernelAsync": [_vp, _vp, _i], "xengXgpuKernelAsyncAcc": [_vp, _vp, _i, _vp, _i], "xengXgpuTryKernelAsyncAcc": [_vp, _vp, _i, _vp, _i], "xengXgpuWaitLaunchSlot": [],
    "xengXgpuKernelAsyncSlab": [_vp, _i, _sz, ctypes.c_uint64, _i, _vp, _i, _vp, _i], "xengXgpuTryKernelAsyncSlab": [_vp, _i, _sz, ctypes.c_uint64, _i, _vp, _i, _vp, _i], "xengXgpuGetSlabFallbacks": [_pi], "xengXgpuGetSlabStats": [_pi, _pi], "xengXgpuSync": [], "xengXgpuSyncLag": [_i], "xengXgpuDumpDone": [_i, _pi], "xengXgpuReset": [],
    "xengXgpuCorrelate": [_vp, _vp, _i], "xengXgpuGetOrder": [_vp, _vp, _vp],
    "xengXgpuSubSelect": [_vp, _vp, _vp, _vp, _i, _i], "xengXgpuReorder": [_vp, _vp, _vp, _vp],
    "xengXgpuGetInfo": [_pi, _pi, _pi, _pi, ctypes.POINTER(ctypes.c_int64), _pi],
    "xengXgpuGetPath": [_pi, _pi], "xengXgpuGetKernel": [_pi, _pi],
    "xengXgpuPacketize": [_vp, _vp, _vp, _vp, _i],
    "xengSnap2Unpack": [_vp, _i, ctypes.c_size_t, _vp, ctypes.c_uint64, _i, _i, _i, _i, _i, _pi, _pi],
    "xengSnap2UnpackAsync": [_vp, _i, ctypes.c_size_t, _vp, ctypes.c_uint64, _i, _i, _i, _i, _i],
    "xengSnap2GetAsyncDrops": [_pi], "xengSnap2StampSeq": [_vp, _i, _sz, ctypes.c_uint64, _i],
    "xengXgpuSetProfiling": [_i], "xengXgpuGetTimes": [ctypes.POINTER(ctypes.c_double), _pi],
    "xengMapAssignI32": [_vp, _vp, _sz], "xengMapAddI32": [_vp, _vp, _sz], "xengMapSync": [],
    "xengMapSumI32": [_vp, _pvp, _i, _sz, _i],
    "xengBeamformInitialize": [_i, _i, _i, _i, _i, _i], "xengBeamformDestroy": [],
    "xengBeamformRun": [_vp, _vp, _vp], "xengBeamformRunVersioned": [_vp, _vp, _vp, ctypes.c_longlong], "xengBeamformTryRunVersioned": [_vp, _vp, _vp, ctypes.c_longlong],
    "xengBeamformRunParts": [_vp, _i, _vp, _vp, _vp, ctypes.c_longlong], "xengBeamformTryRunParts": [_vp, _i, _vp, _vp, _vp, ctypes.c_longlong],
    "xengBeamformRunSlabs": [_vp, _i, _i, _vp, _i, _sz, ctypes.c_uint64, _i, _vp, _vp, ctypes.c_longlong], "xengBeamformTryRunSlabs": [_vp, _i, _i, _vp, _i, _sz, ctypes.c_uint64, _i, _vp, _vp, ctypes.c_longlong], "xengBeamformGetSlabFallbacks": [_pi], "xengBeamformGetSlabStats": [_pi, _pi],
    "xengBeamformIntegrate": [_vp, _vp, _i],
    "xengBeamformIntegrateSingleBeam": [_vp, _vp, _i, _i], "xengBeamformMark": [ctypes.POINTER(ctypes.c_ulonglong)], "xengBeamformWait": [ctypes.c_ulonglong], "xengBeamformTicketDone": [ctypes.c_ulonglong, _pi], "xengBeamformSync": [],
    "xengBeamformPacketizeVoltages": [_vp, _vp, _i, _i, _i, _i, _i, _sz, _i, _i, _i, _i, _i, ctypes.c_uint64],
    "xengBeamformSetProfiling": [_i], "xengBeamformGetTimes": [ctypes.POINTER(ctypes.c_double), _pi],
    "xengBeamformGetRouteInfo": [_pi, _pi, _pi],
    "xengUpchanInitialize": [_i, _i, _i, _i, _i, _i, _i], "xengUpchanInitializeDualPol": [_i, _i, _i, _i, _i, _i, _i], "xengUpchanRun": [_vp, _vp, _vp, _ll], "xengUpchanRunParts": [_vp, _i, _vp, _vp, _vp, _ll],
    "xengUpchanMark": [ctypes.POINTER(ctypes.c_ulonglong)], "xengUpchanWait": [ctypes.c_ulonglong], "xengUpchanTicketDone": [ctypes.c_ulonglong, _pi],
    "xengUpchanSync": [], "xengUpchanDestroy": [], "xengUpchanSetPfb": [_i, ctypes.POINTER(ctypes.c_float)], "xengUpchanReset": [],
    "xengUpchanCorrInitialize": [_i, _i, _i, _i, _i, _i, _i, _i], "xengUpchanCorrGetInfo": [_pi, _pi],
    "xengUpchanCorrAccumulate": [_vp], "xengUpchanCorrAccumulateParts": [_vp, _i, _vp], "xengUpchanCorrDump": [_vp], "xengUpchanCorrReset": [],
    "xengUpchanCorrMark": [ctypes.POINTER(ctypes.c_ulonglong)], "xengUpchanCorrWait": [ctypes.c_ulonglong], "xengUpchanCorrTicketDone": [ctypes.c_ulonglong, _pi],
    "xengUpchanCorrSync": [], "xengUpchanCorrDestroy": [], "xengUpchanCorrSetPfb": [_i, ctypes.POINTER(ctypes.c_float)],
    "xengUpchanCorrPrime": [_vp], "xengUpchanCorrPrimeParts": [_vp, _i, _vp],
    "xengUpchanSumBeamsInitialize": [_i, _i, _i, _i, _i, _i, _i, _i], "xengUpchanSumBeamsGetInfo": [_pi, _pi, _pi],
    "xengUpchanSumBeamsRun": [_vp, _vp], "xengUpchanSumBeamsSetPfb": [_i, ctypes.POINTER(ctypes.c_float)], "xengUpchanSumBeamsPrime": [_vp],
    "xengUpchanSumBeamsReset": [], "xengUpchanSumBeamsMark": [ctypes.POINTER(ctypes.c_ulonglong)], "xengUpchanSumBeamsWait": [ctypes.c_ulonglong],
    "xengUpchanSumBeamsTicketDone": [ctypes.c_ulonglong, _pi], "xengUpchanSumBeamsSync": [], "xengUpchanSumBeamsDestroy": [],
    "xengUpchanSpectraInitialize": [_i, _i, _i, _i, _i, _i], "xengUpchanSpectraGetInfo": [_pi, _pi, _pi],
    "xengUpchanSpectraRun": [_vp, _vp], "xengUpchanSpectraRunParts": [_vp, _i, _vp, _vp], "xengUpchanSpectraSetPfb": [_i, ctypes.POINTER(ctypes.c_float)],
    "xengUpchanSpectraPrime": [_vp], "xengUpchanSpectraPrimeParts": [_vp, _i, _vp], "xengUpchanSpectraReset": [],
    "xengUpchanSpectraMark": [ctypes.POINTER(ctypes.c_ulonglong)], "xengUpchanSpectraWait": [ctypes.c_ulonglong],
    "xengUpchanSpectraTicketDone": [ctypes.c_ulonglong, _pi], "xengUpchanSpectraSync": [], "xengUpchanSpectraDestroy": [],
    "xengDedispInitialize": [_i, _i, _i, _i, _i, _i, _i], "xengDedispSetDelays": [_pi], "xengDedispSetWeights": [ctypes.POINTER(ctypes.c_float)],
    "xengDedispRun": [_vp, _i, _vp], "xengDedispReset": [], "xengDedispGetInfo": [_pi, ctypes.POINTER(ctypes.c_longlong)],
    "xengDedispMark": [ctypes.POINTER(ctypes.c_ulonglong)], "xengDedispWait": [ctypes.c_ulonglong], "xengDedispTicketDone": [ctypes.c_ulonglong, _pi],
    "xengDedispSync": [], "xengDedispDestroy": [], "xengDedispCheckGuards": [_pi],
    "xengPulseInitialize": [_i, _i, _i, _i, _i, _i, _i], "xengPulseRun": [_vp, _i, _vp], "xengPulseReset": [],
    "xengPulseGetInfo": [ctypes.POINTER(ctypes.c_longlong), ctypes.POINTER(ctypes.c_longlong)],
    "xengPulseGetBaseline": [ctypes.POINTER(ctypes.c_float), ctypes.POINTER(ctypes.c_float), ctypes.POINTER(ctypes.c_float)],
    "xengPulseCheckGuards": [_pi], "xengPulseMark": [ctypes.POINTER(ctypes.c_ulonglong)], "xengPulseWait": [ctypes.c_ulonglong],
    "xengPulseTicketDone": [ctypes.c_ulonglong, _pi], "xengPulseSync": [], "xengPulseDestroy": [],
    "xengFoldInitialize": [_i, _i, _i, _i, _i, _i],
    "xengFoldSetPhase": [ctypes.POINTER(ctypes.c_ulonglong), ctypes.POINTER(ctypes.c_ulonglong), _pll, ctypes.POINTER(ctypes.c_ubyte), _ll],
    "xengFoldSetRotations": [_pi], "xengFoldSetWeights": [ctypes.POINTER(ctypes.c_float)], "xengFoldRun": [_vp, _i],
    "xengFoldDump": [_vp, ctypes.POINTER(ctypes.c_uint), _i, _i, _i], "xengFoldReset": [], "xengFoldGetInfo": [_pll, _pll],
    "xengFoldCheckGuards": [_pi], "xengFoldMark": [ctypes.POINTER(ctypes.c_ulonglong)], "xengFoldWait": [ctypes.c_ulonglong],
    "xengFoldTicketDone": [ctypes.c_ulonglong, _pi], "xengFoldSync": [], "xengFoldDestroy": [],
    "xengPeriodInitialize": [_i, _i, _i, _i, _i, _i, _i, _i, _i, _i], "xengPeriodSetMask": [ctypes.POINTER(ctypes.c_ubyte)],
    "xengPeriodRun": [_vp, _i, _vp, _pi], "xengPeriodReset": [], "xengPeriodGetInfo": [_pll, _pi, _pll],
    "xengPeriodGetSpectrum": [ctypes.POINTER(ctypes.c_float), _pi], "xengPeriodCheckGuards": [_pi],
    "xengPeriodMark": [ctypes.POINTER(ctypes.c_ulonglong)], "xengPeriodWait": [ctypes.c_ulonglong],
    "xengPeriodTicketDone": [ctypes.c_ulonglong, _pi], "xengPeriodSync": [], "xengPeriodDestroy": [],
    "xengCdedispInitialize": [_i, _i, _i, _i, _i, _i, _i, _i], "xengCdedispSetChirp": [ctypes.POINTER(ctypes.c_float)],
    "xengCdedispRun": [_vp, _vp, _pi], "xengCdedispReset": [], "xengCdedispGetInfo": [_pi, _pi, _pll, _pll], "xengCdedispCheckGuards": [_pi],
    "xengCdedispMark": [ctypes.POINTER(ctypes.c_ulonglong)], "xengCdedispWait": [ctypes.c_ulonglong],
    "xengCdedispTicketDone": [ctypes.c_ulonglong, _pi], "xengCdedispSync": [], "xengCdedispDestroy": [],
    "xengCdlongInitialize": [_i, _i, _i, _i, _i, _i, _i, _i], "xengCdlongSetChirp": [_i, ctypes.POINTER(ctypes.c_float)],
    "xengCdlongRun": [_vp, _vp, _pi], "xengCdlongReset": [], "xengCdlongGetInfo": [_pi, _pi, _pll, _pll], "xengCdlongCheckGuards": [_pi],
    "xengCdlongMark": [ctypes.POINTER(ctypes.c_ulonglong)], "xengCdlongWait": [ctypes.c_ulonglong],
    "xengCdlongTicketDone": [ctypes.c_ulonglong, _pi], "xengCdlongSync": [], "xengCdlongDestroy": [],
    "xengImageInitialize": [_i, _i, _i, _i, _i], "xengImageGetInfo": [_pi, _pi, _pi, ctypes.POINTER(ctypes.c_double)],
    "xengImageSetGeometry": [ctypes.POINTER(ctypes.c_double), ctypes.POINTER(ctypes.c_double)], "xengImageSetWeights": [ctypes.POINTER(ctypes.c_float), _i],
    "xengImageRun": [_vp, _vp], "xengImageCheckGuards": [_pi], "xengImageMark": [ctypes.POINTER(ctypes.c_ulonglong)], "xengImageWait": [ctypes.c_ulonglong],
    "xengImageTicketDone": [ctypes.c_ulonglong, _pi], "xengImageSync": [], "xengImageDestroy": [],
    "xengGaincalInitialize": [_i, _i, _i, _i], "xengGaincalGetInfo": [_pi, _pi, ctypes.POINTER(ctypes.c_double), _pi],
    "xengGaincalSetModel": [ctypes.POINTER(ctypes.c_double), ctypes.POINTER(ctypes.c_double), ctypes.POINTER(ctypes.c_float)],
    "xengGaincalSetWeights": [ctypes.POINTER(ctypes.c_float), _i], "xengGaincalSetSolver": [_i, ctypes.c_double], "xengGaincalRun": [_vp, _vp, _vp, _i],
    "xengGaincalCheckGuards": [_pi], "xengGaincalMark": [ctypes.POINTER(ctypes.c_ulonglong)], "xengGaincalWait": [ctypes.c_ulonglong],
    "xengGaincalTicketDone": [ctypes.c_ulonglong, _pi], "xengGaincalSync": [], "xengGaincalDestroy": [],
    "xengCalapplyInitialize": [_i, _i, _i, _i], "xengCalapplyGetInfo": [_pi, _pi, _pi, _pll],
    "xengCalapplySetModel": [ctypes.POINTER(ctypes.c_double), ctypes.POINTER(ctypes.c_double), ctypes.POINTER(ctypes.c_float)],
    "xengCalapplySetFactors": [_vp], "xengCalapplyRun": [_vp, _vp], "xengCalapplyCheckGuards": [_pi],
    "xengCalapplyMark": [ctypes.POINTER(ctypes.c_ulonglong)], "xengCalapplyWait": [ctypes.c_ulonglong],
    "xengCalapplyTicketDone": [ctypes.c_ulonglong, _pi], "xengCalapplySync": [], "xengCalapplyDestroy": [],
    "xengPeelInitialize": [_i, _i, _i, _i], "xengPeelGetInfo": [_pi, _pi, ctypes.POINTER(ctypes.c_double), _pi, _pll],
    "xengPeelSetModel": [ctypes.POINTER(ctypes.c_double), ctypes.POINTER(ctypes.c_double), ctypes.POINTER(ctypes.c_float)],
    "xengPeelSetWeights": [ctypes.POINTER(ctypes.c_float), _i], "xengPeelSetSolver": [_i, ctypes.c_double], "xengPeelRun": [_vp, _vp, _vp, _vp, _i],
    "xengPeelCheckGuards": [_pi], "xengPeelMark": [ctypes.POINTER(ctypes.c_ulonglong)], "xengPeelWait": [ctypes.c_ulonglong],
    "xengPeelTicketDone": [ctypes.c_ulonglong, _pi], "xengPeelSync": [], "xengPeelDestroy": [],
    "xengCleanInitialize": [_i, _i, _i, _i, _i, _i], "xengCleanGetInfo": [_pi, _pi, _pll, _pll, _pll, ctypes.POINTER(ctypes.c_double)],
    "xengCleanSetGeometry": [ctypes.POINTER(ctypes.c_double), ctypes.POINTER(ctypes.c_double)], "xengCleanSetWeights": [ctypes.POINTER(ctypes.c_float), _i],
    "xengCleanSetWindow": [ctypes.POINTER(ctypes.c_ubyte)], "xengCleanSetControl": [_i, ctypes.c_float, ctypes.c_float, ctypes.c_float],
    "xengCleanRun": [_vp, _vp], "xengCleanCheckGuards": [_pi], "xengCleanMark": [ctypes.POINTER(ctypes.c_ulonglong)], "xengCleanWait": [ctypes.c_ulonglong],
    "xengCleanTicketDone": [ctypes.c_ulonglong, _pi], "xengCleanSync": [], "xengCleanDestroy": [],
    "xengFlagInitialize": [_i, _i, _i], "xengFlagGetInfo": [_pll, _pll, _pll, _pi], "xengFlagSetWeights": [ctypes.POINTER(ctypes.c_float)],
    "xengFlagSetControl": [ctypes.c_double, ctypes.c_double, ctypes.c_double, _i],
    "xengFlagGetControl": [ctypes.POINTER(ctypes.c_double), ctypes.POINTER(ctypes.c_double), ctypes.POINTER(ctypes.c_double), _pi],
    "xengFlagRun": [_vp, _vp, _vp, _vp], "xengFlagCheckGuards": [_pi], "xengFlagMark": [ctypes.POINTER(ctypes.c_ulonglong)], "xengFlagWait": [ctypes.c_ulonglong],
    "xengFlagTicketDone": [ctypes.c_ulonglong, _pi], "xengFlagSync": [], "xengFlagDestroy": [],
    "xengPredictInitialize": [_i, _i, _i, _i, _i, _i, _i], "xengPredictGetInfo": [_pi, _pi, _pi, _pll, _pll, _pll, _pi],
    "xengPredictSetGeometry": [ctypes.POINTER(ctypes.c_double), ctypes.POINTER(ctypes.c_double)], "xengPredictSetComponents": [_vp], "xengPredictSetMode": [_i],
    "xengPredictRun": [_vp, _vp], "xengPredictCheckGuards": [_pi], "xengPredictMark": [ctypes.POINTER(ctypes.c_ulonglong)], "xengPredictWait": [ctypes.c_ulonglong],
    "xengPredictTicketDone": [ctypes.c_ulonglong, _pi], "xengPredictSync": [], "xengPredictDestroy": [],
    "xengImsearchInitialize": [_i, _i, _i, _i, _i, _i, _i], "xengImsearchSetDelays": [_pi], "xengImsearchSetWeights": [ctypes.POINTER(ctypes.c_float)],
    "xengImsearchRun": [_vp, _vp], "xengImsearchReset": [], "xengImsearchGetInfo": [_pll, _pi],
    "xengImsearchGetBaseline": [ctypes.POINTER(ctypes.c_float), ctypes.POINTER(ctypes.c_float), ctypes.POINTER(ctypes.c_float)],
    "xengImsearchCheckGuards": [_pi], "xengImsearchMark": [ctypes.POINTER(ctypes.c_ulonglong)], "xengImsearchWait": [ctypes.c_ulonglong],
    "xengImsearchTicketDone": [ctypes.c_ulonglong, _pi], "xengImsearchSync": [], "xengImsearchDestroy": [],
    "bfXgpuInitialize": [_pa, _pa, _i], "bfXgpuKernel": [_pa, _pa, _i], "bfXgpuCorrelate": [_pa, _pa, _i],
    "bfXgpuGetOrder": [_pa, _pa, _pa], "bfXgpuSubSelect": [_pa, _pa, _pa, _pa, _i, _i],
    "bfXgpuReorder": [_pa, _pa, _pa, _pa], "bfBeamformInitialize": [_i, _i, _i, _i, _i, _i],
    "bfBeamformRun": [_pa, _pa, _pa], "bfBeamformIntegrate": [_pa, _pa, _i],
    "bfBeamformIntegrateSingleBeam": [_pa, _pa, _i, _i],
}
STRING_SYMBOLS = ["xengGetLastError", "xengVersion"]


def lib():
    global _lib
    if _lib is None:
        if not os.path.exists(LIB_PATH):
            raise ImportError("HIP extension %s is missing: run `python -c 'import __graft_entry__ as g; g.build()'` "
                              "(or make -C caltech-bifrost-dsp_amd/csrc). There is no CPU fallback." % LIB_PATH)
        L = ctypes.CDLL(LIB_PATH)
        for name, args in SYMBOLS.items():
            if os.environ.get("XENG_LIB") and not hasattr(L, name):
                continue
            f = getattr(L, name)
            f.argtypes = args
            f.restype = ctypes.c_int
        for name in STRING_SYMBOLS:
            getattr(L, name).restype = ctypes.c_char_p
            getattr(L, name).argtypes = []
        _lib = L
    return _lib


ENQUEUE_ONLY = ["xengXgpuTryKernelAsyncAcc", "xengXgpuTryKernelAsyncSlab", "xengBeamformTryRunVersioned", "xengBeamformTryRunParts", "xengBeamformTryRunSlabs",
                "xengBeamformIntegrate", "xengBeamformIntegrateSingleBeam", "xengBeamformPacketizeVoltages", "xengBeamformMark",
                "xengUpchanRun", "xengUpchanRunParts", "xengUpchanMark", "xengUpchanTicketDone", "xengUpchanCorrAccumulate",
                "xengUpchanCorrAccumulateParts", "xengUpchanCorrDump", "xengUpchanCorrReset", "xengUpchanCorrMark", "xengUpchanCorrTicketDone", "xengMapAssignI32",
                "xengUpchanReset", "xengUpchanCorrPrime", "xengUpchanCorrPrimeParts",
                "xengUpchanSumBeamsRun", "xengUpchanSumBeamsPrime", "xengUpchanSumBeamsReset", "xengUpchanSumBeamsMark", "xengUpchanSumBeamsTicketDone",
                "xengUpchanSpectraRun", "xengUpchanSpectraRunParts", "xengUpchanSpectraPrime", "xengUpchanSpectraPrimeParts", "xengUpchanSpectraReset",
                "xengUpchanSpectraMark", "xengUpchanSpectraTicketDone",
                "xengDedispRun", "xengDedispReset", "xengDedispMark", "xengDedispTicketDone",
                "xengPulseRun", "xengPulseReset", "xengPulseMark", "xengPulseTicketDone",
                "xengFoldRun", "xengFoldReset", "xengFoldMark", "xengFoldTicketDone",
                "xengPeriodRun", "xengPeriodReset", "xengPeriodMark", "xengPeriodTicketDone",
                "xengCdedispRun", "xengCdedispReset", "xengCdedispMark", "xengCdedispTicketDone",
                "xengCdlongRun", "xengCdlongReset", "xengCdlongMark", "xengCdlongTicketDone",
                "xengImageRun", "xengImageMark", "xengImageTicketDone",
                "xengGaincalRun", "xengGaincalMark", "xengGaincalTicketDone",
                "xengCalapplyRun", "xengCalapplyMark", "xengCalapplyTicketDone",
                "xengPeelRun", "xengPeelMark", "xengPeelTicketDone",
                "xengCleanRun", "xengCleanMark", "xengCleanTicketDone",
                "xengFlagRun", "xengFlagMark", "xengFlagTicketDone",
                "xengPredictRun", "xengPredictMark", "xengPredictTicketDone",
                "xengImsearchRun", "xengImsearchReset", "xengImsearchMark", "xengImsearchTicketDone",
                "xengMapAddI32", "xengMapSumI32", "xengXgpuDumpDone", "xengBeamformTicketDone", "bfBeamformIntegrate", "bfBeamformIntegrateSingleBeam",
                "xengRingBeginSequence", "xengRingEndSequence", "xengRingEndWriting", "xengRingReserve", "xengRingCommit",
                "xengRingCommitExternal", "xengRingNextSequence", "xengRingAcquire", "xengRingAcquireParts", "xengRingSpanRelease", "xengRingGetInfo",
                "xengRingOpenReader", "xengRingCloseReader", "xengRingResize",
                "xengStampNow", "xengStampNowFor", "xengStampDone", "xengGetDevice", "xengSetDevice"]
_enq = None


def enqueue_lib():
    global _enq
    if _enq is None:
        lib()
        E = ctypes.PyDLL(LIB_PATH)
        for name in ENQUEUE_ONLY:
            f = getattr(E, name)
            f.argtypes = SYMBOLS[name]
            f.restype = ctypes.c_int
        _enq = E
    return _enq


def check(name, status):
    if status != STATUS_SUCCESS:
        raise XengError(name, status, lib().xengGetLastError().decode())


def call(name, *args):
    check(name, getattr(lib(), name)(*args))


class DeviceBuffer:

    def __init__(self, nbytes, space=SPACE_CUDA):
        self.nbytes = int(nbytes)
        self.space = space
        p = ctypes.c_void_p()
        call("xengMalloc", ctypes.byref(p), self.nbytes, space)
        self.ptr = p.value

    def free(self):
        if self.ptr:
            call("xengFree", self.ptr, self.space)
            self.ptr = None

    def __del__(self):
        try:
            self.free()
        except Exception:
            pass

    def upload(self, arr, offset=0):
        arr = np.ascontiguousarray(arr)
        assert offset + arr.nbytes <= self.nbytes
        call("xengMemcpy", self.ptr + offset, arr.ctypes.data, arr.nbytes)
        return self

    def download(self, dtype, count=None, offset=0):
        dtype = np.dtype(dtype)
        if count is None:
            count = (self.nbytes - offset) // dtype.itemsize
        out = np.empty(count, dtype=dtype)
        call("xengMemcpy", out.ctypes.data, self.ptr + offset, out.nbytes)
        return out

    def as_host_array(self, dtype):
        assert self.space == SPACE_CUDA_HOST
        dtype = np.dtype(dtype)
        buf = (ctypes.c_char * self.nbytes).from_address(self.ptr)
        buf._owner = self
        return np.frombuffer(buf, dtype=dtype)


def device_count():
    n = ctypes.c_int(0)
    call("xengGetDeviceCount", ctypes.byref(n))
    return n.value


def device_pci_bus_id(gpu=0):
    buf = ctypes.create_string_buffer(32)
    call("xengGetDevicePciBusId", gpu, buf, 32)
    return buf.value.decode().lower()


def device_info(gpu=0):
    cu, clk, mem = ctypes.c_int(), ctypes.c_int(), ctypes.c_size_t()
    name = ctypes.create_string_buffer(128)
    call("xengGetDeviceInfo", gpu, ctypes.byref(cu), ctypes.byref(clk), ctypes.byref(mem), name, 128)
    return {"num_cu": cu.value, "clock_khz": clk.value, "total_mem": mem.value, "name": name.value.decode()}
```

caltech-bifrost-dsp_amd/ring.py:

```python
import collections
import ctypes
import os
import threading
import weakref

import numpy as np

from . import ffi
from .ndarray import XArray, copy_array, to_dtype, _SPACE_ID

IMPLEMENTATION = os.environ.get("XENG_RING", "native")


def _stream_mask(classes):
    m = 0
    for c in classes:
        m |= ffi.STREAMS[c]
    return m


class LibraryStamps:
    mask = 0
    declared = 0
    users = 0
# ... 412 lines not shown
            self._cond.notify_all()

    def _end_writing(self):
        with self._cond:
            if self._open_seq is not None:
                self._open_seq.ended = True
                self._open_seq = None
            self._writing_ended = True
            self._cond.notify_all()

    def _wait_for_room(self, nbytes, nonblocking):
        with self._cond:
            if self._capacity == 0:
                self._capacity = 4 * nbytes
            while self._live_bytes + nbytes > max(self._capacity, nbytes):
                self._gc()
                if self._live_bytes + nbytes <= max(self._capacity, nbytes):
                    break
                if not any(r.guarantee for r in self._readers):
                    self._drop_oldest()
                    continue
                if nonblocking:
                    raise BlockingIOError("ring %r full" % self.name)
                self._cond.wait(0.5)

    def _commit(self, seq, data, nbytes):
        with self._cond:
            seq.chunks.append(_Chunk(seq.committed, nbytes, data))
            seq.committed += nbytes
            self._live_bytes += nbytes
            self._cond.notify_all()

    def _gc(self):
        readers = self._readers
        if not readers:
            return
        if len(readers) == 1:
            lo_seq, lo_off = readers[0].seq_index, readers[0].offset
        else:
            lo_seq, lo_off = min([(r.seq_index, r.offset) for r in readers])
        seqs, g, freed = self._seqs, self._gc_seq, 0
        while g < lo_seq:
            ch = seqs[g].chunks
            while ch:
                c = ch.popleft()
                if c.data is not None:
                    c.data = None
                    freed += c.nbytes
            g += 1
        self._gc_seq = g
        if lo_seq < len(seqs):
            ch = seqs[lo_seq].chunks
            while ch and ch[0].offset + ch[0].nbytes <= lo_off:
                c = ch.popleft()
                if c.data is not None:
                    c.data = None
                    freed += c.nbytes
        self._live_bytes -= freed

    def _drop_oldest(self):
        for seq in self._seqs[self._gc_seq:]:
            if seq.chunks:
                ch = seq.chunks.popleft()
                if ch.data is not None:
                    ch.data = None
                    self._live_bytes -= ch.nbytes
                return
        self._live_bytes = 0

    def _pieces(self, seq, offset, nbytes):
        pieces = []
        for ch in seq.chunks:
            if ch.offset >= offset + nbytes:
                break
            lo, hi = max(offset, ch.offset), min(offset + nbytes, ch.offset + ch.nbytes)
            if lo < hi:
                pieces.append(ch.data if (lo == ch.offset and hi == ch.offset + ch.nbytes) else ch.data.byte_slice(lo - ch.offset, hi - lo))
        return pieces

    def _assemble(self, seq, offset, nbytes):
        c0 = seq.chunks[0]
        if c0.offset == offset and c0.nbytes == nbytes:
            return c0.data
        pieces = self._pieces(seq, offset, nbytes)
        if len(pieces) == 1:
            return pieces[0]
        out = XArray(shape=(nbytes,), dtype=np.uint8, space=self.space)
        pos = 0
        for p in pieces:
            copy_array(out.byte_slice(pos, p.nbytes), p)
            pos += p.nbytes
        return out

    def read(self, guarantee=True):
        rd = _Reader(guarantee)
        self._count_user()
        with self._cond:
            rd.seq_index = len(self._seqs)
            for seq in self._seqs[self._gc_seq:]:
                if seq.chunks or not seq.ended:
                    rd.seq_index = seq.index
                    break
            self._readers.append(rd)
        return _SequenceReader(self._read_sequences(rd), lambda: self._close_reader(rd))

    def _close_reader(self, rd):
        with self._cond:
            if rd in self._readers:
                self._readers.remove(rd)
                self._gc()
            self._cond.notify_all()

    def _read_sequences(self, rd):
        while True:
            with self._cond:
                while len(self._seqs) <= rd.seq_index and not self._writing_ended:
                    self._cond.wait(0.5)
                if len(self._seqs) <= rd.seq_index:
                    return
                seq = self._seqs[rd.seq_index]
                rd.offset = 0
            yield ReadSequence(seq, rd)
            with self._cond:
                rd.seq_index += 1
                rd.offset = 0
                self._gc()
                self._cond.notify_all()


_WOULD_BLOCK, _END = ffi.STATUS_WOULD_BLOCK, ffi.STATUS_END_OF_DATA
_xf = None


def _xfast():
    global _xf
    if _xf is None:
        try:
            from . import _xfast as m
        except ImportError as e:
            raise ImportError("the _xfast extension is missing: run `python -c 'import __graft_entry__ as g; g.build()'` "
                              "(or make -C caltech-bifrost-dsp_amd/csrc): %s" % e)
        _xf = m
    return _xf


class _NWriteSpan(_SpanViews):
    __slots__ = ("ring", "_seq_id", "size", "_span", "data", "_closed")

    def __init__(self, ring, seq_id, nbytes, nonblocking):
        self.ring, self._seq_id, self.size = ring, seq_id, int(nbytes)
        ptr, ref, self._span = ring._x.ring_reserve(ring, ring._h, seq_id, self.size, bool(nonblocking))
        self.data = XArray.window(ptr, self.size, ring.space, ref)
        self._closed = False

    def commit(self, nbytes=None):
        if self._closed:
            return
        self._closed = True
        n = self.size if nbytes is None else int(nbytes)
        if n > 0:
            self.ring._x.ring_commit(self.ring._h, self._seq_id, self._span, n)

    def close(self):
        self.commit()

    def __enter__(self):
        return self

    def __exit__(self, *exc):
        self.close()
        return False


class _NWriteSequence:
    def __init__(self, ring, seq_id):
        self.ring, self._seq_id = ring, seq_id

    def reserve(self, nbytes, nonblocking=False):
        return _NWriteSpan(self.ring, self._seq_id, nbytes, nonblocking)

    def commit_external(self, data):
        ring = self.ring
        assert data.space == ring.space, (data.space, ring.space)
        ring._external[data.ptr] = data
        ring._x.ring_commit_external(ring._h, self._seq_id, data.ptr, data.nbytes)

    def end(self):
        self.ring._enq.xengRingEndSequence(self.ring._h, self._seq_id)

    def __enter__(self):
        return self

    def __exit__(self, *exc):
        self.end()
        return False


class _NWriter:
    def __init__(self, ring):
        self.ring = ring

    def begin_sequence(self, time_tag=0, header="", nringlet=1, name=None):
        ring = self.ring
        hdr = header.encode() if isinstance(header, str) else bytes(header)
        seq = ctypes.c_longlong()
        ffi.check("xengRingBeginSequence", ring._enq.xengRingBeginSequence(ring._h, int(time_tag), hdr, len(hdr), int(nringlet), ctypes.byref(seq)))
        return _NWriteSequence(ring, seq.value)

    def __enter__(self):
        return self

    def __exit__(self, *exc):
        self.ring._enq.xengRingEndWriting(self.ring._h)
        return False


class _NReadSequence:
    def __init__(self, ring, rid, header, time_tag, nringlet):
        self.ring, self._rid = ring, rid
        self.header, self.time_tag, self.nringlet = header, time_tag, nringlet

    def read(self, gulp_nbytes):
        ring, rid = self.ring, self._rid
        h, acquire, space, window = ring._h, ring._x.ring_acquire, ring.space, XArray.window
        gulp_nbytes = int(gulp_nbytes)
        advance = offset = 0
        while True:
            got = acquire(ring, h, rid, advance, gulp_nbytes)
            if got is None:
                return
            ptr, size, ref, skipped = got
            offset += advance + skipped
            yield ReadSpan(window(ptr, size, space, ref), size, offset, skipped)
            del ref, got
            advance = size
            if size < gulp_nbytes:
                return


    def read_parts(self, gulp_nbytes):
        ring, rid = self.ring, self._rid
        h, acquire, space, window = ring._h, ring._x.ring_acquire_parts, ring.space, XArray.window
        gulp_nbytes = int(gulp_nbytes)
        advance = offset = 0
        while True:
            got = acquire(ring, h, rid, advance, gulp_nbytes)
            if got is None:
                return
            skipped = got[0]
            parts = [window(ptr, n, space, ref) for ptr, n, ref in got[1:]]
            size = sum(p.nbytes for p in parts)
            offset += advance + skipped
            yield ReadSpan(None, size, offset, skipped, parts)
            del parts, got
            advance = size
            if size < gulp_nbytes:
                return


class _ReaderCount:
    def __init__(self, ring):
        self._ring = ring

    def __len__(self):
        return self._ring.info()["nreaders"]


class NativeRing:
    span_memory_outlives_release = True

    def __init__(self, name="", space="system", core=None):
        self.name, self.space = name, space
        self._lib, self._enq, self._x = ffi.lib(), ffi.enqueue_lib(), _xfast()
        h = ctypes.c_void_p()
        ffi.call("xengRingCreate", ctypes.byref(h), name.encode(), _SPACE_ID[space])
        self._h = h.value
        self._external = {}
        self._hooks = None

    def __del__(self):
        h, self._h = getattr(self, "_h", None), None
        if h:
            try:
                self._lib.xengRingDestroy(h)
            except Exception:
                pass

    @property
    def _readers(self):
        return _ReaderCount(self)

    def info(self):
        cap, live, pool, nrd, nseq = ctypes.c_size_t(), ctypes.c_size_t(), ctypes.c_size_t(), ctypes.c_int(), ctypes.c_longlong()
        cnt = (ctypes.c_ulonglong * 5)()
        ffi.check("xengRingGetInfo", self._enq.xengRingGetInfo(self._h, ctypes.byref(cap), ctypes.byref(live), ctypes.byref(pool), ctypes.byref(nrd),
                                                               ctypes.byref(nseq), cnt))
        return {"capacity": cap.value, "live_bytes": live.value, "pool_bytes": pool.value, "nreaders": nrd.value, "nseq": nseq.value,
                "alloc": cnt[0], "free": cnt[1], "reuse": cnt[2], "stamp_wait": cnt[3], "skipped_bytes": cnt[4]}

    @property
    def counters(self):
        return self.info()

    def set_stamp_source(self, src):
        def now(user, out):
            out[0] = int(src.now())

        def done(user, st):
            return int(bool(src.done(st[0])[0]))

        def wait(user, st):
            src.wait(st[0])
        self._hooks = (ffi.STAMP_NOW_FN(now), ffi.STAMP_DONE_FN(done), ffi.STAMP_WAIT_FN(wait))
        ffi.call("xengRingSetStampHooks", self._h, self._hooks[0], self._hooks[1], self._hooks[2], None)

    def declare_streams(self, *classes):
        ffi.call("xengRingDeclareStreams", self._h, _stream_mask(classes))

    def stamp_classes(self):
        c, d, u = ctypes.c_uint(), ctypes.c_uint(), ctypes.c_uint()
        ffi.call("xengRingGetStampClasses", self._h, ctypes.byref(c), ctypes.byref(d), ctypes.byref(u))
        return c.value, d.value, u.value

    def set_recycle(self, on=True):
        ffi.call("xengRingSetRecycle", self._h, int(bool(on)))

    def resize(self, contig_bytes, total_span=None, nringlet=1):
        ffi.check("xengRingResize", self._enq.xengRingResize(self._h, int(contig_bytes), int(total_span) if total_span else 0))

    def begin_writing(self):
        return _NWriter(self)

    def _write_span(self, nbytes, nonblocking):
        return _NWriteSpan(self, -1, nbytes, nonblocking)

    def read(self, guarantee=True):
        rid = ctypes.c_int()
        ffi.check("xengRingOpenReader", self._enq.xengRingOpenReader(self._h, int(bool(guarantee)), ctypes.byref(rid)))
        rid = rid.value
        return _SequenceReader(self._read_sequences(rid), lambda: self._close_reader(rid))

    def _close_reader(self, rid):
        if self._h:
            self._enq.xengRingCloseReader(self._h, rid)

    def _read_sequences(self, rid):
        nxt = self._x.ring_next_sequence
        while True:
            got = nxt(self._h, rid)
            if got is None:
                return
            yield _NReadSequence(self, rid, _Header(got[0]), got[1], got[2])


def Ring(name="", space="system", core=None):
    if IMPLEMENTATION == "python":
        return PyRing(name=name, space=space, core=core)
    return NativeRing(name=name, space=space, core=core)


__all__ = ["Ring", "NativeRing", "PyRing", "WriteSpan", "to_dtype"]
```

include/xeng.h:

```cpp
#ifndef XENG_H_
#define XENG_H_

#include <stddef.h>
#include <stdint.h>

#ifdef __cplusplus
extern "C" {
#endif

#define XENG_STATUS_SUCCESS            0
#define XENG_STATUS_INVALID_ARGUMENT   1
#define XENG_STATUS_INVALID_STATE      2
#define XENG_STATUS_DEVICE_ERROR       3
#define XENG_STATUS_UNSUPPORTED        4
#define XENG_STATUS_MEM_ALLOC_FAILED   5
#define XENG_STATUS_WOULD_BLOCK        6
#define XENG_STATUS_END_OF_DATA        7

#define XENG_SPACE_AUTO       0
#define XENG_SPACE_SYSTEM     1
#define XENG_SPACE_CUDA       2
#define XENG_SPACE_CUDA_HOST  3

#define XENG_MAX_DIMS 8
typedef struct XENGarray_ {
    void *data;
    int   space;
    int   dtype;
    int   ndim;
    long  shape[XENG_MAX_DIMS];
    long  strides[XENG_MAX_DIMS];
    int   immutable;
    int   big_endian;
    int   conjugated;
} XENGarray;

const char *xengGetLastError(void);
const char *xengVersion(void);

int xengGetDeviceCount(int *count);
int xengSetDevice(int gpu);
int xengGetDevice(int *gpu);
int xengDeviceSynchronize(void);
int xengGetDeviceInfo(int gpu, int *num_cu, int *clock_khz, size_t *total_mem, char *name, int name_len);
int xengGetDevicePciBusId(int gpu, char *bus_id, int len);
int xengMalloc(void **ptr, size_t nbytes, int space);
int xengFree(void *ptr, int space);
int xengMemcpy(void *dst, const void *src, size_t nbytes);
int xengMemcpyAsync(void *dst, const void *src, size_t nbytes);
int xengMemset(void *dst, int value, size_t nbytes);
int xengStreamSynchronize(void);

typedef struct xengStamp_ { unsigned long long w[16]; } xengStamp;
#define XENG_STREAMS_XGPU      1u
#define XENG_STREAMS_MAP       2u
#define XENG_STREAMS_BEAM      4u
#define XENG_STREAMS_COPY      8u
#define XENG_STREAMS_CONSUMER 16u
#define XENG_STREAMS_ALL      31u
#define XENG_STREAMS_XGPU_OUT 32u
int xengStampNow(xengStamp *stamp);
int xengStampNowFor(xengStamp *stamp, const void *buf, unsigned classes);
int xengStampDone(const xengStamp *stamp, int *done, int *waitable);
int xengStampWait(const xengStamp *stamp);

typedef struct xengRing_ xengRing;
int xengRingCreate(xengRing **ring, const char *name, int space);
int xengRingDestroy(xengRing *ring);
int xengRingResize(xengRing *ring, size_t contig_bytes, size_t total_span);
int xengRingDeclareStreams(xengRing *ring, unsigned classes);
int xengRingGetStampClasses(xengRing *ring, unsigned *classes, unsigned *declared, unsigned *users);
int xengRingSetRecycle(xengRing *ring, int on);
int xengRingGetInfo(xengRing *ring, size_t *capacity, size_t *live_bytes, size_t *pool_bytes, int *nreaders, long long *nseq,
                    unsigned long long counters[5]);
int xengRingBeginSequence(xengRing *ring, long long time_tag, const void *header, size_t header_len, int nringlet, long long *seq);
int xengRingEndSequence(xengRing *ring, long long seq);
int xengRingEndWriting(xengRing *ring);
int xengRingReserve(xengRing *ring, long long seq, size_t nbytes, int nonblocking, int may_block, void **data, long long *span);
int xengRingCommit(xengRing *ring, long long seq, long long span, size_t nbytes);
int xengRingCommitExternal(xengRing *ring, long long seq, void *data, size_t nbytes, int may_block);
int xengRingOpenReader(xengRing *ring, int guarantee, int *reader);
int xengRingCloseReader(xengRing *ring, int reader);
int xengRingNextSequence(xengRing *ring, int reader, int may_block, long long *seq, long long *time_tag, int *nringlet,
                         const void **header, size_t *header_len);
int xengRingAcquire(xengRing *ring, int reader, size_t advance, size_t gulp_nbytes, int may_block, void **data, size_t *nbytes,
                    long long *span, size_t *skipped);
int xengRingAcquireParts(xengRing *ring, int reader, size_t advance, size_t gulp_nbytes, int may_block, void *data[2], size_t nbytes[2],
                         long long span[2], int *nparts, size_t *skipped);
int xengRingSpanRelease(long long span);
typedef void (*xengRingStampNowFn)(void *user, unsigned long long stamp[2]);
typedef int (*xengRingStampDoneFn)(void *user, const unsigned long long stamp[2]);
typedef void (*xengRingStampWaitFn)(void *user, const unsigned long long stamp[2]);
int xengRingSetStampHooks(xengRing *ring, xengRingStampNowFn now, xengRingStampDoneFn done, xengRingStampWaitFn wait, void *user);


int xengXgpuConfigure(int nstand, int npol, int nchan, int ntime_gulp, int max_gulps_per_flush);

int xengXgpuInitialize(int gpu);
int xengXgpuDestroy(void);

int xengXgpuKernel(const void *in_dev, void *out_dev, int doDump);

int xengXgpuKernelAsync(const void *in_dev, void *out_dev, int doDump);
int xengXgpuKernelAsyncAcc(const void *in_dev, void *out_dev, int doDump, void *acc_dev, int acc_mode);
int xengXgpuTryKernelAsyncAcc(const void *in_dev, void *out_dev, int doDump, void *acc_dev, int acc_mode);
int xengXgpuWaitLaunchSlot(void);
int xengXgpuKernelAsyncSlab(const void *packets_dev, int npkt, size_t pkt_stride, uint64_t seq0, int chan0_pipeline, void *out_dev,
                            int doDump, void *acc_dev, int acc_mode);
int xengXgpuTryKernelAsyncSlab(const void *packets_dev, int npkt, size_t pkt_stride, uint64_t seq0, int chan0_pipeline, void *out_dev,
                               int doDump, void *acc_dev, int acc_mode);
int xengXgpuGetSlabFallbacks(int *nfallback);
int xengXgpuGetSlabStats(int *nscattered, int *nirregular);
int xengXgpuSync(void);
int xengXgpuSyncLag(int lag);
int xengXgpuDumpDone(int lag, int *done);

int xengXgpuReset(void);

int xengXgpuCorrelate(const void *in_host, void *out_host, int doDump);

int xengXgpuGetOrder(const int32_t *antpol_to_input, int32_t *antpol_to_bl, int32_t *is_conj);

int xengXgpuSubSelect(const void *in_dev, void *out_dev, const int32_t *vismap_dev,
                      const int32_t *conj_dev, int nvis, int nchan_sum);

int xengXgpuPacketize(const void *in_dev, void *out_dev, const int32_t *antpol_to_bl_dev,
                      const int32_t *is_conj_dev, int fmt);

int xengXgpuReorder(const void *in_host, void *out_host, const int32_t *antpol_to_bl, const int32_t *is_conj);

int xengXgpuGetInfo(int *nstand, int *npol, int *nchan, int *ntime_gulp, int64_t *matlen, int *max_gulps);

int xengXgpuGetPath(int *fused_corner_turn, int *fp6);
int xengXgpuGetKernel(int *waves_per_group, int *mfma_k);

int xengXgpuSetProfiling(int enable);
int xengXgpuGetTimes(double ms[2], int count[2]);

int xengSnap2Unpack(const void *packets_dev, int npkt, size_t pkt_stride, void *out_dev, uint64_t seq0, int ntime,
                    int chan0_pipeline, int nchan_tot, int npol_tot, int clear, int *nplaced, int *ndropped);
int xengSnap2UnpackAsync(const void *packets_dev, int npkt, size_t pkt_stride, void *out_dev, uint64_t seq0, int ntime,
                         int chan0_pipeline, int nchan_tot, int npol_tot, int clear);
int xengSnap2GetAsyncDrops(int *ndropped);

int xengSnap2StampSeq(void *packets_dev, int npkt, size_t pkt_stride, uint64_t seq0, int pkts_per_seq);

int xengMapAssignI32(void *a_dev, const void *b_dev, size_t nwords);
int xengMapAddI32(void *a_dev, const void *b_dev, size_t nwords);
#define XENG_MAP_SUM_MAX 16
int xengMapSumI32(void *a_dev, const void *const *srcs_dev, int nsrc, size_t nwords, int add);
int xengMapSync(void);


int xengBeamformInitialize(int gpu, int ninput, int nchan, int ntime, int nbeam, int ntime_blocks);
int xengBeamformDestroy(void);

int xengBeamformRun(const void *in_dev, void *out_dev, const void *weights_dev);
int xengBeamformRunVersioned(const void *in_dev, void *out_dev, const void *weights_dev, long long weights_version);
int xengBeamformTryRunVersioned(const void *in_dev, void *out_dev, const void *weights_dev, long long weights_version);
int xengBeamformRunParts(const void *in0_dev, int ntime0, const void *in1_dev, void *out_dev, const void *weights_dev, long long weights_version);
int xengBeamformTryRunParts(const void *in0_dev, int ntime0, const void *in1_dev, void *out_dev, const void *weights_dev, long long weights_version);
int xengBeamformRunSlabs(const void *packets0_dev, int npkt0, int ntime0, const void *packets1_dev, int npkt1, size_t pkt_stride,
                         uint64_t seq0, int chan0_pipeline, void *out_dev, const void *weights_dev, long long weights_version);
int xengBeamformTryRunSlabs(const void *packets0_dev, int npkt0, int ntime0, const void *packets1_dev, int npkt1, size_t pkt_stride,
                            uint64_t seq0, int chan0_pipeline, void *out_dev, const void *weights_dev, long long weights_version);
int xengBeamformGetSlabFallbacks(int *nfallback);
int xengBeamformGetSlabStats(int *nscattered, int *nirregular);

int xengBeamformIntegrate(const void *in_dev, void *out_dev, int ntime_sum);

int xengBeamformIntegrateSingleBeam(const void *in_dev, void *out_dev, int ntime_sum, int beam_id);
int xengBeamformPacketizeVoltages(const void *in_dev, void *out_dev, int nchan, int nbeam, int ntime, int beam0, int nbeam_pkt,
                                  size_t pkt_stride, int server, int gbe, int nbeam_hdr, int nserver, int chan0, uint64_t seq0);
int xengBeamformSync(void);
int xengBeamformMark(unsigned long long *ticket);
int xengBeamformWait(unsigned long long ticket);
int xengBeamformTicketDone(unsigned long long ticket, int *done);
int xengBeamformSetProfiling(int enable);
int xengBeamformGetTimes(double ms[2], int count[2]);
int xengBeamformGetRouteInfo(int *tiles_total, int *tiles_bf16, int *outlier_inputs);

int xengUpchanInitialize(int gpu, int ninput, int nchan, int ntime, int nupchan, int nbeam, int nframe_sum);
int xengUpchanInitializeDualPol(int gpu, int ninput, int nchan, int ntime, int nupchan, int nbeam, int nframe_sum);
int xengUpchanRun(const void *in_dev, void *out_dev, const void *weights_dev, long long weights_version);
int xengUpchanRunParts(const void *in0_dev, int ntime0, const void *in1_dev, void *out_dev, const void *weights_dev,
                       long long weights_version);
int xengUpchanSetPfb(int ntap, const float *coeffs);
int xengUpchanReset(void);
int xengUpchanMark(unsigned long long *ticket);
int xengUpchanWait(unsigned long long ticket);
int xengUpchanTicketDone(unsigned long long ticket, int *done);
int xengUpchanSync(void);
int xengUpchanDestroy(void);

int xengUpchanCorrInitialize(int gpu, int ninput, int nchan, int ntime, int nupchan, int fine_lo, int fine_hi, int nstage);
int xengUpchanCorrGetInfo(int *nfine, int *nstage);
int xengUpchanCorrAccumulate(const void *in_dev);
int xengUpchanCorrAccumulateParts(const void *in0_dev, int ntime0, const void *in1_dev);
int xengUpchanCorrDump(void *out_dev);
int xengUpchanCorrReset(void);
int xengUpchanCorrSetPfb(int ntap, const float *coeffs);
int xengUpchanCorrPrime(const void *in_dev);
int xengUpchanCorrPrimeParts(const void *in0_dev, int ntime0, const void *in1_dev);
int xengUpchanCorrMark(unsigned long long *ticket);
int xengUpchanCorrWait(unsigned long long ticket);
int xengUpchanCorrTicketDone(unsigned long long ticket, int *done);
int xengUpchanCorrSync(void);
int xengUpchanCorrDestroy(void);

int xengUpchanSumBeamsInitialize(int gpu, int nchan, int nbeam, int ntime, int nupchan, int pair0, int npair, int nframe_sum);
int xengUpchanSumBeamsGetInfo(int *gulps_per_window, int *windows_per_gulp, int *pos);
int xengUpchanSumBeamsRun(const void *in_dev, void *out_dev);
int xengUpchanSumBeamsSetPfb(int ntap, const float *coeffs);
int xengUpchanSumBeamsPrime(const void *in_dev);
int xengUpchanSumBeamsReset(void);
int xengUpchanSumBeamsMark(unsigned long long *ticket);
int xengUpchanSumBeamsWait(unsigned long long ticket);
int xengUpchanSumBeamsTicketDone(unsigned long long ticket, int *done);
int xengUpchanSumBeamsSync(void);
int xengUpchanSumBeamsDestroy(void);

int xengUpchanSpectraInitialize(int gpu, int ninput, int nchan, int ntime, int nupchan, int nframe_sum);
int xengUpchanSpectraGetInfo(int *gulps_per_window, int *windows_per_gulp, int *pos);
int xengUpchanSpectraRun(const void *in_dev, void *out_dev);
int xengUpchanSpectraRunParts(const void *in0_dev, int ntime0, const void *in1_dev, void *out_dev);
int xengUpchanSpectraSetPfb(int ntap, const float *coeffs);
int xengUpchanSpectraPrime(const void *in_dev);
int xengUpchanSpectraPrimeParts(const void *in0_dev, int ntime0, const void *in1_dev);
int xengUpchanSpectraReset(void);
int xengUpchanSpectraMark(unsigned long long *ticket);
int xengUpchanSpectraWait(unsigned long long ticket);
int xengUpchanSpectraTicketDone(unsigned long long ticket, int *done);
int xengUpchanSpectraSync(void);
int xengUpchanSpectraDestroy(void);

#define XENG_DEDISP_MAX_HISTORY_BYTES (1LL << 32)
int xengDedispInitialize(int gpu, int npair, int nfine, int nwin, int ndm, int max_delay, int nprod);
int xengDedispSetDelays(const int *delays);
int xengDedispSetWeights(const float *weights);
int xengDedispRun(const void *in_dev, int nwin_call, void *out_dev);
int xengDedispReset(void);
int xengDedispGetInfo(int *max_delay_in_use, long long *nwindows_since_reset);
int xengDedispCheckGuards(int *intact);
int xengDedispMark(unsigned long long *ticket);
int xengDedispWait(unsigned long long ticket);
int xengDedispTicketDone(unsigned long long ticket, int *done);
int xengDedispSync(void);
int xengDedispDestroy(void);

int xengPulseInitialize(int gpu, int npair, int ndm, int nwin, int nprod, int nwidth, int nstat);
int xengPulseRun(const void *in_dev, int nwin_call, void *out_dev);
int xengPulseReset(void);
int xengPulseGetInfo(long long *nwindows_since_reset, long long *nblocks_complete);
int xengPulseGetBaseline(float *c, float *m, float *var);
int xengPulseCheckGuards(int *intact);
int xengPulseMark(unsigned long long *ticket);
int xengPulseWait(unsigned long long ticket);
int xengPulseTicketDone(unsigned long long ticket, int *done);
int xengPulseSync(void);
int xengPulseDestroy(void);

#define XENG_FOLD_MAX_PROFILE_BYTES (1LL << 32)
int xengFoldInitialize(int gpu, int npair, int nfine, int nwin, int nbin, int nprod);
int xengFoldSetPhase(const unsigned long long *phi0, const unsigned long long *dphi, const long long *ddphi, const unsigned char *active,
                     long long n_ref);
int xengFoldSetRotations(const int *rot);
int xengFoldSetWeights(const float *weights);
int xengFoldRun(const void *in_dev, int nwin_call);
int xengFoldDump(void *out_dev, unsigned int *hits_host, int nfscr, int normalise, int clear);
int xengFoldReset(void);
int xengFoldGetInfo(long long *nwindows_since_reset, long long *nwindows_folded);
int xengFoldCheckGuards(int *intact);
int xengFoldMark(unsigned long long *ticket);
int xengFoldWait(unsigned long long ticket);
int xengFoldTicketDone(unsigned long long ticket, int *done);
int xengFoldSync(void);
int xengFoldDestroy(void);

#define XENG_PERIOD_MAX_STATE_BYTES (1LL << 32)
int xengPeriodInitialize(int gpu, int npair, int ndm, int nwin, int nprod, int nt, int nstack, int nlevel, int nwhite, int kmin);
int xengPeriodSetMask(const unsigned char *keep);
int xengPeriodRun(const void *in_dev, int nwin_call, void *out_dev, int *completed);
int xengPeriodReset(void);
int xengPeriodGetInfo(long long *nwindows_since_reset, int *nseg_in_stack, long long *nstacks_complete);
int xengPeriodGetSpectrum(float *A_host, int *nseg);
int xengPeriodCheckGuards(int *intact);
int xengPeriodMark(unsigned long long *ticket);
int xengPeriodWait(unsigned long long ticket);
int xengPeriodTicketDone(unsigned long long ticket, int *done);
int xengPeriodSync(void);
int xengPeriodDestroy(void);

#define XENG_CDEDISP_MAX_STATE_BYTES (1LL << 32)
int xengCdedispInitialize(int gpu, int nchan, int nbeam, int ntime, int pair0, int npair, int nfft, int overlap);
int xengCdedispSetChirp(const float *table);
int xengCdedispRun(const void *in_dev, void *out_dev, int *nblocks);
int xengCdedispReset(void);
int xengCdedispGetInfo(int *step, int *max_blocks_per_call, long long *nsamples_since_reset, long long *nblocks_since_reset);
int xengCdedispCheckGuards(int *intact);
int xengCdedispMark(unsigned long long *ticket);
int xengCdedispWait(unsigned long long ticket);
int xengCdedispTicketDone(unsigned long long ticket, int *done);
int xengCdedispSync(void);
int xengCdedispDestroy(void);

#define XENG_CDLONG_MAX_STATE_BYTES (1LL << 35)
int xengCdlongInitialize(int gpu, int nchan, int nbeam, int ntime, int pair0, int npair, int nfft, int overlap);
int xengCdlongSetChirp(int pair, const float *table);
int xengCdlongRun(const void *in_dev, void *out_dev, int *nblocks);
int xengCdlongReset(void);
int xengCdlongGetInfo(int *step, int *max_blocks_per_call, long long *nsamples_since_reset, long long *nblocks_since_reset);
int xengCdlongCheckGuards(int *intact);
int xengCdlongMark(unsigned long long *ticket);
int xengCdlongWait(unsigned long long ticket);
int xengCdlongTicketDone(unsigned long long ticket, int *done);
int xengCdlongSync(void);
int xengCdlongDestroy(void);

#define XENG_IMAGE_MAX_NSTAND 512
#define XENG_IMAGE_MAX_STATE_BYTES (1LL << 31)
int xengImageInitialize(int gpu, int nstand, int nfine, int nfavg, int npix);
int xengImageGetInfo(int *ngroup, int *pixel_tile, int *lds_bytes, double *norm);
int xengImageSetGeometry(const double *tau, const double *freq);
int xengImageSetWeights(const float *w, int autos);
int xengImageRun(const void *vis_dev, void *out_dev);
int xengImageCheckGuards(int *intact);
int xengImageMark(unsigned long long *ticket);
int xengImageWait(unsigned long long ticket);
int xengImageTicketDone(unsigned long long ticket, int *done);
int xengImageSync(void);
int xengImageDestroy(void);

#define XENG_GAINCAL_MAX_NSRC 32
#define XENG_GAINCAL_MAX_NSTAND 512
#define XENG_GAINCAL_MAX_NITER 1024
#define XENG_GAINCAL_DEFAULT_NITER 60
#define XENG_GAINCAL_DEFAULT_TOL 1e-5
int xengGaincalInitialize(int gpu, int nstand, int nfine, int nsrc);
int xengGaincalGetInfo(int *lds_bytes, int *niter, double *tol, int *refant);
int xengGaincalSetModel(const double *tau, const double *freq, const float *flux);
int xengGaincalSetWeights(const float *w, int refant);
int xengGaincalSetSolver(int niter, double tol);
int xengGaincalRun(const void *vis_dev, void *gains_dev, void *stats_dev, int warm);
int xengGaincalCheckGuards(int *intact);
int xengGaincalMark(unsigned long long *ticket);
int xengGaincalWait(unsigned long long ticket);
int xengGaincalTicketDone(unsigned long long ticket, int *done);
int xengGaincalSync(void);
int xengGaincalDestroy(void);

#define XENG_CALAPPLY_MAX_NSRC 32
#define XENG_CALAPPLY_MAX_NSTAND 512
int xengCalapplyInitialize(int gpu, int nstand, int nfine, int nsrc);
int xengCalapplyGetInfo(int *ntile, int *ngroup, int *lds_bytes, long long *span_bytes);
int xengCalapplySetModel(const double *tau, const double *freq, const float *flux);
int xengCalapplySetFactors(const void *h);
int xengCalapplyRun(const void *vis_dev, void *out_dev);
int xengCalapplyCheckGuards(int *intact);
int xengCalapplyMark(unsigned long long *ticket);
int xengCalapplyWait(unsigned long long ticket);
int xengCalapplyTicketDone(unsigned long long ticket, int *done);
int xengCalapplySync(void);
int xengCalapplyDestroy(void);

#define XENG_PEEL_MAX_NDIR 8
#define XENG_PEEL_MAX_NSTAND 512
#define XENG_PEEL_MAX_NITER 1024
#define XENG_PEEL_DEFAULT_NITER 60
#define XENG_PEEL_DEFAULT_TOL 1e-5
int xengPeelInitialize(int gpu, int nstand, int nfine, int ndir);
int xengPeelGetInfo(int *lds_bytes, int *niter, double *tol, int *refant, long long *span_bytes);
int xengPeelSetModel(const double *tau, const double *freq, const float *flux);
int xengPeelSetWeights(const float *w, int refant);
int xengPeelSetSolver(int niter, double tol);
int xengPeelRun(const void *vis_dev, void *out_dev, void *gains_dev, void *stats_dev, int warm);
int xengPeelCheckGuards(int *intact);
int xengPeelMark(unsigned long long *ticket);
int xengPeelWait(unsigned long long ticket);
int xengPeelTicketDone(unsigned long long ticket, int *done);
int xengPeelSync(void);
int xengPeelDestroy(void);

#define XENG_CLEAN_MAX_NITER 4096
#define XENG_CLEAN_MAX_NSTAND 2048
#define XENG_CLEAN_MAX_STATE_BYTES (1LL << 31)
int xengCleanInitialize(int gpu, int nstand, int nfine, int nfavg, int npix, int niter_max);
int xengCleanGetInfo(int *ngroup, int *pixel_tile, long long *comp_offset, long long *stats_offset, long long *span_bytes, double *norm);
int xengCleanSetGeometry(const double *tau, const double *freq);
int xengCleanSetWeights(const float *w, int autos);
int xengCleanSetWindow(const unsigned char *mask);
int xengCleanSetControl(int niter, float gain, float threshold, float fraction);
int xengCleanRun(const void *image_dev, void *out_dev);
int xengCleanCheckGuards(int *intact);
int xengCleanMark(unsigned long long *ticket);
int xengCleanWait(unsigned long long ticket);
int xengCleanTicketDone(unsigned long long ticket, int *done);
int xengCleanSync(void);
int xengCleanDestroy(void);

#define XENG_FLAG_MAX_NSTAND 512
#define XENG_FLAG_MAX_NFINE 8192
#define XENG_FLAG_MAX_WCHAN 64
#define XENG_FLAG_DEFAULT_NSIG_CROSS 6.0
#define XENG_FLAG_DEFAULT_NSIG_AUTO 6.0
#define XENG_FLAG_DEFAULT_NSIG_CHAN 6.0
#define XENG_FLAG_DEFAULT_WCHAN 0
int xengFlagInitialize(int gpu, int nstand, int nfine);
int xengFlagGetInfo(long long *mask_bytes, long long *stats_bytes, long long *chan_bytes, int *lds_bytes);
int xengFlagSetWeights(const float *w);
int xengFlagSetControl(double nsig_cross, double nsig_auto, double nsig_chan, int wchan);
int xengFlagGetControl(double *nsig_cross, double *nsig_auto, double *nsig_chan, int *wchan);
int xengFlagRun(const void *vis_dev, void *mask_dev, void *stats_dev, void *chan_dev);
int xengFlagCheckGuards(int *intact);
int xengFlagMark(unsigned long long *ticket);
int xengFlagWait(unsigned long long ticket);
// ... 53 lines not shown
```

Before: 6582.

## Scan pool for completed buffers, skip finished writer waits, eager stream creation

Buffer reuse now scans the pooled buffers for one whose stamp has already completed, instead of only looking at the front one, and picks among take, grow or wait through a small policy helper. Writer dependencies whose event has already completed no longer enqueue a stream wait. Streams are created eagerly in a fixed order. Adds reader/writer declaration tokens, a settable pool limit, and timing and wait counters with a trace analysis script. The aim is fewer blocking host waits and fewer stream dependencies, at the cost of extra clock_gettime calls and vector allocations on every buffer obtain.

```diff
diff --git a/caltech-bifrost-dsp_amd/csrc/ring.hip b/caltech-bifrost-dsp_amd/csrc/ring.hip
--- a/caltech-bifrost-dsp_amd/csrc/ring.hip
+++ b/caltech-bifrost-dsp_amd/csrc/ring.hip
@@ -10,6 +10,7 @@
 #include <string>
 #include <vector>
 
+#include "ring_policy.h"
 #include "xeng_common.h"
 
 namespace xeng {
@@ -74,16 +75,31 @@
     bool recycle_system = false;
     unsigned stream_mask = 0;
     std::atomic<unsigned> declared{0}, users{0};
+    std::vector<unsigned> tokens;
+    unsigned next_token = 1;
     bool writer_seen = false;
     std::atomic<size_t> owned_bytes{0};
+    std::atomic<size_t> own_cap{0};
     std::atomic<unsigned long long> n_alloc{0}, n_free{0}, n_reuse{0}, n_stamp_wait{0}, n_skipped{0};
+    static constexpr int NWAIT_READERS = 4;
+    std::atomic<unsigned long long> ns_stamp_wait{0}, n_room_wait{0}, ns_room_wait{0}, n_grow{0}, ns_alloc{0}, n_scan_hit{0};
+    std::atomic<unsigned long long> n_acq_wait[NWAIT_READERS] = {}, ns_acq_wait[NWAIT_READERS] = {};
 };
+
+static unsigned long long now_ns() {
+    struct timespec ts;
+    clock_gettime(CLOCK_MONOTONIC, &ts);
+    return (unsigned long long)ts.tv_sec * 1000000000ull + (unsigned long long)ts.tv_nsec;
+}
 
 static void ring_unref(RingCore* r) {
     if (r->refs.fetch_sub(1) == 1) delete r;
 }
 
-static size_t own_limit(const RingCore* r, size_t nbytes) { return 8 * std::max(r->capacity, 2 * nbytes); }
+static size_t own_limit(const RingCore* r, size_t nbytes) {
+    if (const size_t cap = r->own_cap.load()) return cap;
+    return 8 * std::max(r->capacity, 2 * nbytes);
+}
 
 static bool pooled_space(const RingCore* r) { return r->space != XENG_SPACE_SYSTEM || r->hook_now || r->recycle_system; }
 
@@ -138,9 +154,12 @@
 static int buf_wait(Buf* b) {
     RingCore* r = b->ring;
     r->n_stamp_wait++;
-    if (r->hook_wait) { r->hook_wait(r->hook_user, b->hook_stamp); return XENG_STATUS_SUCCESS; }
-    if (b->space == XENG_SPACE_SYSTEM) return XENG_STATUS_SUCCESS;
-    return stamp_wait(b->stamp);
+    const unsigned long long t0 = now_ns();
+    int rc = XENG_STATUS_SUCCESS;
+    if (r->hook_wait) r->hook_wait(r->hook_user, b->hook_stamp);
+    else if (b->space != XENG_SPACE_SYSTEM) rc = stamp_wait(b->stamp);
+    r->ns_stamp_wait += now_ns() - t0;
+    return rc;
 }
 
 static void buf_destroy(Buf* b, bool may_wait) {
@@ -192,40 +211,67 @@
 static int buf_obtain(RingCore* r, size_t nbytes, int may_block, Buf** out) {
     *out = nullptr;
     if (pooled_space(r)) {
-        Buf* cand = nullptr;
-        {
-            std::lock_guard<std::mutex> lk(r->pool_mu);
-            auto it = r->pool.find(nbytes);
-            if (it != r->pool.end() && !it->second.empty()) {
-                cand = it->second.front();
-                it->second.pop_front();
-                r->pool_bytes -= nbytes;
+        std::vector<Buf*> busy;
+        std::vector<char> done_v, wait_v;
+        for (;;) {
+            Buf* cand = nullptr;
+            {
+                std::lock_guard<std::mutex> lk(r->pool_mu);
+                auto it = r->pool.find(nbytes);
+                if (it != r->pool.end() && !it->second.empty()) {
+                    cand = it->second.front();
+                    it->second.pop_front();
+                    r->pool_bytes -= nbytes;
+                }
             }
-        }
-        if (cand) {
+            if (!cand) break;
             bool done, waitable;
             buf_poll(cand, &done, &waitable);
-            const bool grow = !done && r->owned_bytes.load() + nbytes <= own_limit(r, nbytes) && !r->hook_now;
-            if (!done && waitable && may_block && !grow) done = buf_wait(cand) == XENG_STATUS_SUCCESS;
-            if (done) {
-                *out = cand;
-            } else {
+            busy.push_back(cand);
+            done_v.push_back(done);
+            wait_v.push_back(waitable);
+            if (done) break;
+        }
+        int rc = XENG_STATUS_SUCCESS;
+        if (!busy.empty()) {
+            const bool may_grow = r->owned_bytes.load() + nbytes <= own_limit(r, nbytes) && (!r->hook_now || r->own_cap.load());
+            ReissueChoice c = reissue_choice((const bool*)done_v.data(), (const bool*)wait_v.data(), (int)busy.size(), may_grow);
+            if (c.what == REISSUE_WAIT) {
+                if (!may_block) rc = XENG_STATUS_WOULD_BLOCK;
+                else if (buf_wait(busy[c.index]) == XENG_STATUS_SUCCESS) c.what = REISSUE_TAKE;
+            }
+            if (c.what == REISSUE_TAKE) {
+                *out = busy[c.index];
+                if (c.index > 0) r->n_scan_hit++;
+                busy.erase(busy.begin() + c.index);
+            } else if (c.what == REISSUE_GROW) {
+                r->n_grow++;
+            }
+            std::vector<Buf*> orphans;
+            {
                 std::lock_guard<std::mutex> lk(r->pool_mu);
-                if (waitable) r->pool[nbytes].push_front(cand);
-                else r->pool[nbytes].push_back(cand);
-                r->pool_bytes += nbytes;
-                if (waitable && !may_block && !grow) return XENG_STATUS_WOULD_BLOCK;
+                if (!r->destroyed) {
+                    auto& dq = r->pool[nbytes];
+                    dq.insert(dq.begin(), busy.begin(), busy.end());
+                    r->pool_bytes += nbytes * busy.size();
+                } else {
+                    orphans.swap(busy);
+                }
             }
+            for (Buf* b : orphans) buf_destroy(b, may_block != 0);
         }
         if (*out) {
             (*out)->refs.store(1);
             r->n_reuse++;
             return XENG_STATUS_SUCCESS;
         }
+        if (rc) return rc;
     }
     if (!may_block && (r->space != XENG_SPACE_SYSTEM || nbytes > (1u << 20))) return XENG_STATUS_WOULD_BLOCK;
     void* p = nullptr;
+    const unsigned long long t0 = now_ns();
     int rc = raw_alloc(r->space, nbytes, &p);
+    r->ns_alloc += now_ns() - t0;
     if (rc) return rc;
     Buf* b = new Buf();
     b->ptr = p; b->nbytes = nbytes; b->space = r->space; b->ring = r;
@@ -285,6 +331,7 @@
 static int wait_for_room(RingCore* r, std::unique_lock<std::mutex>& lk, size_t nbytes, int nonblocking, int may_block) {
     if (r->capacity == 0) r->capacity = 4 * nbytes;
     std::vector<Buf*> released;
+    unsigned long long t_wait = 0;
     for (;;) {
         const size_t cap = std::max(r->capacity, nbytes);
         if (r->live_bytes + nbytes <= cap) break;
@@ -299,12 +346,15 @@
         if (nonblocking || !may_block || r->destroyed) {
             lk.unlock(); release_all(released); lk.lock();
             if (r->destroyed) XENG_FAIL(XENG_STATUS_INVALID_STATE, "ring '%s' was destroyed", r->name.c_str());
+            if (t_wait) r->ns_room_wait += now_ns() - t_wait;
             if (nonblocking) XENG_FAIL(XENG_STATUS_WOULD_BLOCK, "ring '%s' full", r->name.c_str());
             return XENG_STATUS_WOULD_BLOCK;
         }
         if (!released.empty()) { lk.unlock(); release_all(released); lk.lock(); continue; }
+        if (!t_wait) { t_wait = now_ns(); r->n_room_wait++; }
         r->cv.wait_for(lk, std::chrono::milliseconds(100));
     }
+    if (t_wait) r->ns_room_wait += now_ns() - t_wait;
     if (!released.empty()) { lk.unlock(); release_all(released); lk.lock(); }
     return XENG_STATUS_SUCCESS;
 }
@@ -381,11 +431,48 @@
     return XENG_STATUS_SUCCESS;
 }
 
+int xengRingDeclareUser(xengRing* ring, unsigned classes, unsigned* token) {
+    RING_ARG(ring);
+    if (!token) XENG_FAIL(XENG_STATUS_INVALID_ARGUMENT, "RingDeclareUser: null token");
+    std::lock_guard<std::mutex> lk(r->pool_mu);
+    r->stream_mask |= classes & (STAMP_ALL | STAMP_XGPU_OUT);
+    *token = r->next_token++;
+    r->tokens.push_back(*token);
+    return XENG_STATUS_SUCCESS;
+}
+
+static int consume_token(RingCore* r, unsigned token) {
+    if (!token) return XENG_STATUS_SUCCESS;
+    std::lock_guard<std::mutex> lk(r->pool_mu);
+    for (size_t k = 0; k < r->tokens.size(); k++)
+        if (r->tokens[k] == token) {
+            r->tokens.erase(r->tokens.begin() + k);
+            r->declared.fetch_add(1);
+            return XENG_STATUS_SUCCESS;
+        }
+    XENG_FAIL(XENG_STATUS_INVALID_ARGUMENT, "ring '%s': %u is not an unused declaration token", r->name.c_str(), token);
+}
+
 int xengRingGetStampClasses(xengRing* ring, unsigned* classes, unsigned* declared, unsigned* users) {
     RING_ARG(ring);
     if (classes) *classes = effective_mask(r);
     if (declared) *declared = r->declared.load();
     if (users) *users = r->users.load();
+    return XENG_STATUS_SUCCESS;
+}
+
+int xengRingSetPoolLimit(xengRing* ring, size_t owned_bytes) {
+    RING_ARG(ring);
+    r->own_cap.store(owned_bytes);
+    return XENG_STATUS_SUCCESS;
+}
+
+int xengRingGetWaitStats(xengRing* ring, unsigned long long* stats, int n) {
+    RING_ARG(ring);
+    if (!stats || n < 0) XENG_FAIL(XENG_STATUS_INVALID_ARGUMENT, "RingGetWaitStats: bad argument");
+    unsigned long long v[XENG_RING_WAIT_STATS] = {r->n_stamp_wait, r->ns_stamp_wait, r->n_room_wait, r->ns_room_wait, r->n_grow, r->ns_alloc, r->n_scan_hit, 0};
+    for (int k = 0; k < RingCore::NWAIT_READERS; k++) { v[8 + 2 * k] = r->n_acq_wait[k]; v[9 + 2 * k] = r->ns_acq_wait[k]; }
+    for (int k = 0; k < n && k < XENG_RING_WAIT_STATS; k++) stats[k] = v[k];
     return XENG_STATUS_SUCCESS;
 }
 
@@ -429,12 +516,20 @@
 }
 
 int xengRingBeginSequence(xengRing* ring, long long time_tag, const void* header, size_t header_len, int nringlet, long long* seq) {
+    return xengRingBeginSequenceAs(ring, time_tag, header, header_len, nringlet, 0, seq);
+}
+
+int xengRingBeginSequenceAs(xengRing* ring, long long time_tag, const void* header, size_t header_len, int nringlet, unsigned token, long long* seq) {
     RING_ARG(ring);
     if (!seq) XENG_FAIL(XENG_STATUS_INVALID_ARGUMENT, "BeginSequence: null seq");
     std::lock_guard<std::mutex> lk(r->mu);
     if (r->destroyed) XENG_FAIL(XENG_STATUS_INVALID_STATE, "ring '%s' was destroyed", r->name.c_str());
+    if (!r->writer_seen) {
+        if (int rc = consume_token(r, token)) return rc;
+        r->writer_seen = true;
+        r->users.fetch_add(1);
+    }
     if (r->open_seq) r->open_seq->ended = true;
-    if (!r->writer_seen) { r->writer_seen = true; r->users.fetch_add(1); }
     std::unique_ptr<Seq> s(new Seq());
     s->index = r->nseq++;
     s->time_tag = time_tag;
@@ -524,10 +619,13 @@
     return XENG_STATUS_SUCCESS;
 }
 
-int xengRingOpenReader(xengRing* ring, int guarantee, int* reader) {
+int xengRingOpenReader(xengRing* ring, int guarantee, int* reader) { return xengRingOpenReaderAs(ring, guarantee, 0, reader); }
+
+int xengRingOpenReaderAs(xengRing* ring, int guarantee, unsigned token, int* reader) {
     RING_ARG(ring);
     if (!reader) XENG_FAIL(XENG_STATUS_INVALID_ARGUMENT, "OpenReader: null reader");
     std::lock_guard<std::mutex> lk(r->mu);
+    if (int rc = consume_token(r, token)) return rc;
     size_t k = 0;
     while (k < r->readers.size() && r->readers[k].open) k++;
     if (k == r->readers.size()) r->readers.emplace_back();
@@ -605,6 +703,7 @@
     std::vector<Chunk> pieces;
     int rc = XENG_STATUS_SUCCESS;
     size_t n = 0, skip_total = 0;
+    unsigned long long t_wait = 0;
     {
         std::unique_lock<std::mutex> lk(r->mu);
         if (reader < 0 || reader >= (int)r->readers.size() || !r->readers[reader].open || !r->readers[reader].in_seq)
@@ -640,8 +739,10 @@
                 break;
             }
             if (!may_block) { rc = XENG_STATUS_WOULD_BLOCK; break; }
+            if (!t_wait) { t_wait = now_ns(); if (reader < RingCore::NWAIT_READERS) r->n_acq_wait[reader]++; }
             r->cv.wait_for(lk, std::chrono::milliseconds(100));
         }
+        if (t_wait && reader < RingCore::NWAIT_READERS) r->ns_acq_wait[reader] += now_ns() - t_wait;
     }
     release_all(released);
     if (skipped) *skipped = skip_total;
diff --git a/caltech-bifrost-dsp_amd/csrc/ring_policy.h b/caltech-bifrost-dsp_amd/csrc/ring_policy.h
--- /dev/null
+++ b/caltech-bifrost-dsp_amd/csrc/ring_policy.h
@@ -0,0 +1,20 @@
+#pragma once
+
+namespace xeng {
+
+enum ReissueWhat { REISSUE_TAKE = 0, REISSUE_GROW = 1, REISSUE_WAIT = 2 };
+struct ReissueChoice {
+    ReissueWhat what;
+    int index;
+};
+
+inline ReissueChoice reissue_choice(const bool* done, const bool* waitable, int n, bool may_grow) {
+    for (int k = 0; k < n; k++)
+        if (done[k]) return ReissueChoice{REISSUE_TAKE, k};
+    if (may_grow) return ReissueChoice{REISSUE_GROW, -1};
+    for (int k = 0; k < n; k++)
+        if (waitable[k]) return ReissueChoice{REISSUE_WAIT, k};
+    return ReissueChoice{REISSUE_GROW, -1};
+}
+
+}
diff --git a/caltech-bifrost-dsp_amd/csrc/xcorr.hip b/caltech-bifrost-dsp_amd/csrc/xcorr.hip
--- a/caltech-bifrost-dsp_amd/csrc/xcorr.hip
+++ b/caltech-bifrost-dsp_amd/csrc/xcorr.hip
@@ -77,6 +77,7 @@
 static XgpuContext g_ctx;
 static unsigned long long g_epoch = 1;
 static unsigned long long g_ctx_gen = 1;
+static unsigned long long g_launches = 0, g_wait_staging = 0, g_wait_writer[XgpuContext::NMM] = {}, g_wait_writer_done = 0;
 
 static int destroy_locked() {
     XgpuContext& x = g_ctx;
@@ -145,7 +146,12 @@
     XgpuContext& x = g_ctx;
     auto it = x.writers.find(buf);
     if (it == x.writers.end() || it->second.stream == self) return XENG_STATUS_SUCCESS;
-    if (hipEvent_t ev = launch_event(it->second.seq)) XENG_HIP(hipStreamWaitEvent(s, ev, 0));
+    if (hipEvent_t ev = launch_event(it->second.seq)) {
+        if (hipEventQuery(ev) == hipSuccess) { g_wait_writer_done++; return XENG_STATUS_SUCCESS; }
+        (void)hipGetLastError();
+        XENG_HIP(hipStreamWaitEvent(s, ev, 0));
+        if (self >= 0 && it->second.stream >= 0 && it->second.stream < XgpuContext::NMM) g_wait_writer[it->second.stream]++;
+    }
     return XENG_STATUS_SUCCESS;
 }
 
@@ -207,7 +213,9 @@
         XENG_HIP(hipEventRecord(x.ev_ct, x.stream));
         XENG_HIP(hipStreamWaitEvent(smm, x.ev_ct, 0));
         x.staging_seen = ops;
-    }
+        g_wait_staging++;
+    }
+    g_launches++;
     const unsigned long long seq = x.nlaunch;
     {
         const int k = (int)(seq % XgpuContext::NEV);
@@ -663,6 +671,15 @@
     }
     if (nscattered) *nscattered = ns;
     if (nirregular) *nirregular = ni;
+    return XENG_STATUS_SUCCESS;
+}
+
+int xengXgpuGetLaunchWaits(unsigned long long* stats, int n) {
+    if (!stats || n < 0) XENG_FAIL(XENG_STATUS_INVALID_ARGUMENT, "GetLaunchWaits: bad argument");
+    std::lock_guard<std::mutex> lk(g_mu);
+    unsigned long long v[XENG_XGPU_LAUNCH_WAITS] = {g_launches, g_wait_staging, g_wait_writer_done};
+    for (int k = 0; k < XgpuContext::NMM; k++) v[3 + k] = g_wait_writer[k];
+    for (int k = 0; k < n && k < XENG_XGPU_LAUNCH_WAITS; k++) stats[k] = v[k];
     return XENG_STATUS_SUCCESS;
 }
 
diff --git a/caltech-bifrost-dsp_amd/csrc/xeng_util.hip b/caltech-bifrost-dsp_amd/csrc/xeng_util.hip
--- a/caltech-bifrost-dsp_amd/csrc/xeng_util.hip
+++ b/caltech-bifrost-dsp_amd/csrc/xeng_util.hip
@@ -28,6 +28,21 @@
     stream_tick(STREAM_XGPU);
 }
 unsigned long long staging_stream_ops() { return g_staging_ops.load(std::memory_order_relaxed); }
+
+static const StreamId STREAM_CREATE_ORDER[STREAM_COUNT] = {
+    STREAM_XGPU, STREAM_XGPU_MM, STREAM_XGPU_MM2, STREAM_COPY, STREAM_BEAM, STREAM_MAP, STREAM_CONSUMER,
+    STREAM_XGPU_MM3, STREAM_XGPU_MM4, STREAM_XGPU_MM5, STREAM_XGPU_MM6, STREAM_XGPU_MM7, STREAM_XGPU_MM8};
+static constexpr int NEAGER = 6;
+static int g_created[MAXDEV];
+static int g_creation_index[MAXDEV][STREAM_COUNT];
+
+static int g_claimed[MAXDEV];
+
+static int create_upto(int created, StreamId which) {
+    int pos = 0;
+    while (pos < (int)STREAM_COUNT && STREAM_CREATE_ORDER[pos] != which) pos++;
+    return std::max(created, std::max(NEAGER, pos + 1));
+}
 
 int get_stream(StreamId which, hipStream_t* out) {
     int dev = 0;
@@ -37,9 +52,13 @@
     if (!g_stream_ok[dev][which]) {
         int lo = 0, hi = 0;
         XENG_HIP(hipDeviceGetStreamPriorityRange(&lo, &hi));
-        const bool high = which == STREAM_MAP || which == STREAM_BEAM || which == STREAM_CONSUMER || which == STREAM_COPY;
-        XENG_HIP(hipStreamCreateWithPriority(&g_streams[dev][which], hipStreamNonBlocking, high ? hi : 0 < lo ? 0 : lo));
-        g_stream_ok[dev][which] = true;
+        for (const int upto = create_upto(g_created[dev], which); g_created[dev] < upto; g_created[dev]++) {
+            const StreamId id = STREAM_CREATE_ORDER[g_created[dev]];
+            const bool high = id == STREAM_MAP || id == STREAM_BEAM || id == STREAM_CONSUMER || id == STREAM_COPY;
+            XENG_HIP(hipStreamCreateWithPriority(&g_streams[dev][id], hipStreamNonBlocking, high ? hi : 0 < lo ? 0 : lo));
+            g_stream_ok[dev][id] = true;
+            g_creation_index[dev][id] = g_created[dev] + 1;
+        }
     }
     *out = g_streams[dev][which];
     return XENG_STATUS_SUCCESS;
@@ -488,6 +507,29 @@
 }
 int xengStreamSynchronize(void) { return sync_all_streams(); }
 
+int xengGetStreamOrder(int gpu, int* places, int n) {
+    if (gpu < 0 || gpu >= MAXDEV || !places || n < 0) XENG_FAIL(XENG_STATUS_INVALID_ARGUMENT, "GetStreamOrder: bad argument");
+    std::lock_guard<std::mutex> lk(g_stream_mu);
+    for (int k = 0; k < n && k < (int)STREAM_COUNT; k++) places[k] = g_creation_index[gpu][k];
+    return XENG_STATUS_SUCCESS;
+}
+int xengStreamOrderClaim(int slot, int which, int* places, int n) {
+    if (slot < 0 || slot >= MAXDEV || which < 0 || which >= (int)STREAM_COUNT || !places || n < 0)
+        XENG_FAIL(XENG_STATUS_INVALID_ARGUMENT, "StreamOrderClaim: bad argument");
+    std::lock_guard<std::mutex> lk(g_stream_mu);
+    g_claimed[slot] = create_upto(g_claimed[slot], (StreamId)which);
+    for (int k = 0; k < n && k < (int)STREAM_COUNT; k++) places[k] = 0;
+    for (int p = 0; p < g_claimed[slot]; p++)
+        if ((int)STREAM_CREATE_ORDER[p] < n) places[STREAM_CREATE_ORDER[p]] = p + 1;
+    return XENG_STATUS_SUCCESS;
+}
+int xengStreamOrderForget(int slot) {
+    if (slot < 0 || slot >= MAXDEV) XENG_FAIL(XENG_STATUS_INVALID_ARGUMENT, "StreamOrderForget: bad slot");
+    std::lock_guard<std::mutex> lk(g_stream_mu);
+    g_claimed[slot] = 0;
+    return XENG_STATUS_SUCCESS;
+}
+
 static const int PACKED_STREAMS[5] = {STREAM_XGPU, STREAM_MAP, STREAM_BEAM, STREAM_COPY, STREAM_CONSUMER};
 static void stamp_pack(const Stamp& s, xengStamp* o) {
     memset(o, 0, sizeof(*o));
diff --git a/caltech-bifrost-dsp_amd/ffi.py b/caltech-bifrost-dsp_amd/ffi.py
--- a/caltech-bifrost-dsp_amd/ffi.py
+++ b/caltech-bifrost-dsp_amd/ffi.py
@@ -43,6 +43,11 @@
     "xengStampNow": [_pst], "xengStampNowFor": [_pst, _vp, ctypes.c_uint], "xengStampDone": [_pst, _pi, _pi], "xengStampWait": [_pst],
     "xengRingCreate": [_pvp, ctypes.c_char_p, _i], "xengRingDestroy": [_vp], "xengRingResize": [_vp, _sz, _sz], "xengRingSetRecycle": [_vp, _i], "xengRingDeclareStreams": [_vp, ctypes.c_uint], "xengRingGetStampClasses": [_vp, ctypes.POINTER(ctypes.c_uint), ctypes.POINTER(ctypes.c_uint), ctypes.POINTER(ctypes.c_uint)],
     "xengRingGetInfo": [_vp, _psz, _psz, _psz, _pi, _pll, ctypes.POINTER(ctypes.c_ulonglong)],
+    "xengRingDeclareUser": [_vp, ctypes.c_uint, ctypes.POINTER(ctypes.c_uint)], "xengRingOpenReaderAs": [_vp, _i, ctypes.c_uint, _pi],
+    "xengRingBeginSequenceAs": [_vp, _ll, ctypes.c_char_p, _sz, _i, ctypes.c_uint, _pll],
+    "xengRingSetPoolLimit": [_vp, _sz], "xengRingGetWaitStats": [_vp, ctypes.POINTER(ctypes.c_ulonglong), _i],
+    "xengGetStreamOrder": [_i, _pi, _i], "xengStreamOrderClaim": [_i, _i, _pi, _i], "xengStreamOrderForget": [_i],
+    "xengXgpuGetLaunchWaits": [ctypes.POINTER(ctypes.c_ulonglong), _i],
     "xengRingBeginSequence": [_vp, _ll, ctypes.c_char_p, _sz, _i, _pll], "xengRingEndSequence": [_vp, _ll], "xengRingEndWriting": [_vp],
     "xengRingReserve": [_vp, _ll, _sz, _i, _i, _pvp, _pll], "xengRingCommit": [_vp, _ll, _ll, _sz],
     "xengRingCommitExternal": [_vp, _ll, _vp, _sz, _i],
diff --git a/caltech-bifrost-dsp_amd/ring.py b/caltech-bifrost-dsp_amd/ring.py
--- a/caltech-bifrost-dsp_amd/ring.py
+++ b/caltech-bifrost-dsp_amd/ring.py
@@ -738,6 +738,15 @@
     def counters(self):
         return self.info()
 
+    def wait_stats(self):
+        v = (ctypes.c_ulonglong * 16)()
+        ffi.call("xengRingGetWaitStats", self._h, v, 16)
+        return {"stamp_wait": v[0], "stamp_wait_s": v[1] * 1e-9, "room_wait": v[2], "room_wait_s": v[3] * 1e-9, "grow": v[4], "alloc_s": v[5] * 1e-9,
+                "reissued_not_oldest": v[6], "acquire_wait": [v[8 + 2 * k] for k in range(4)], "acquire_wait_s": [v[9 + 2 * k] * 1e-9 for k in range(4)]}
+
+    def set_pool_limit(self, nbytes):
+        ffi.call("xengRingSetPoolLimit", self._h, int(nbytes))
+
     def set_stamp_source(self, src):
         def now(user, out):
             out[0] = int(src.now())
diff --git a/include/xeng.h b/include/xeng.h
--- a/include/xeng.h
+++ b/include/xeng.h
@@ -50,6 +50,10 @@
 int xengMemcpyAsync(void *dst, const void *src, size_t nbytes);
 int xengMemset(void *dst, int value, size_t nbytes);
 int xengStreamSynchronize(void);
+#define XENG_STREAM_IDS 13
+int xengGetStreamOrder(int gpu, int *places, int n);
+int xengStreamOrderClaim(int slot, int which, int *places, int n);
+int xengStreamOrderForget(int slot);
 
 typedef struct xengStamp_ { unsigned long long w[16]; } xengStamp;
 #define XENG_STREAMS_XGPU      1u
@@ -69,17 +73,24 @@
 int xengRingDestroy(xengRing *ring);
 int xengRingResize(xengRing *ring, size_t contig_bytes, size_t total_span);
 int xengRingDeclareStreams(xengRing *ring, unsigned classes);
+int xengRingDeclareUser(xengRing *ring, unsigned classes, unsigned *token);
 int xengRingGetStampClasses(xengRing *ring, unsigned *classes, unsigned *declared, unsigned *users);
 int xengRingSetRecycle(xengRing *ring, int on);
 int xengRingGetInfo(xengRing *ring, size_t *capacity, size_t *live_bytes, size_t *pool_bytes, int *nreaders, long long *nseq,
                     unsigned long long counters[5]);
+int xengRingSetPoolLimit(xengRing *ring, size_t owned_bytes);
+#define XENG_RING_WAIT_STATS 16
+int xengRingGetWaitStats(xengRing *ring, unsigned long long *stats, int n);
 int xengRingBeginSequence(xengRing *ring, long long time_tag, const void *header, size_t header_len, int nringlet, long long *seq);
+int xengRingBeginSequenceAs(xengRing *ring, long long time_tag, const void *header, size_t header_len, int nringlet, unsigned token,
+                            long long *seq);
 int xengRingEndSequence(xengRing *ring, long long seq);
 int xengRingEndWriting(xengRing *ring);
 int xengRingReserve(xengRing *ring, long long seq, size_t nbytes, int nonblocking, int may_block, void **data, long long *span);
 int xengRingCommit(xengRing *ring, long long seq, long long span, size_t nbytes);
 int xengRingCommitExternal(xengRing *ring, long long seq, void *data, size_t nbytes, int may_block);
 int xengRingOpenReader(xengRing *ring, int guarantee, int *reader);
+int xengRingOpenReaderAs(xengRing *ring, int guarantee, unsigned token, int *reader);
 int xengRingCloseReader(xengRing *ring, int reader);
 int xengRingNextSequence(xengRing *ring, int reader, int may_block, long long *seq, long long *time_tag, int *nringlet,
                          const void **header, size_t *header_len);
@@ -111,6 +122,8 @@
                                int doDump, void *acc_dev, int acc_mode);
 int xengXgpuGetSlabFallbacks(int *nfallback);
 int xengXgpuGetSlabStats(int *nscattered, int *nirregular);
+#define XENG_XGPU_LAUNCH_WAITS 11
+int xengXgpuGetLaunchWaits(unsigned long long *stats, int n);
 int xengXgpuSync(void);
 int xengXgpuSyncLag(int lag);
 int xengXgpuDumpDone(int lag, int *done);
diff --git a/profiles/blocks_gap.py b/profiles/blocks_gap.py
--- /dev/null
+++ b/profiles/blocks_gap.py
@@ -0,0 +1,242 @@
+#!/usr/bin/env python3
+import ctypes
+import json
+import os
+import sys
+import threading
+import time
+
+ROOT = os.path.dirname(os.path.dirname(os.path.abspath(__file__)))
+sys.path.insert(0, ROOT)
+
+
+def trace_windows(path, first=0):
+    import csv
+    rows = list(csv.DictReader(open(path)))
+    ev = sorted((int(r["Start_Timestamp"]), int(r["End_Timestamp"]), r["Kernel_Name"].split("(")[0].split("::")[-1][:28], r.get("Queue_Id", "")) for r in rows)
+    xc = [e for e in ev if e[2].startswith("xcorr_")]
+    print("# %d kernels, %d contractions; windows of 100 contractions" % (len(ev), len(xc)))
+    for k in range(first * 100, len(xc) - 100, 100):
+        w0, w1 = xc[k][0], xc[k + 100][0]
+        sel = [e for e in ev if w0 <= e[0] < w1]
+        cur, idle, longest, last, split = w0, 0, 0, None, {}
+        for e in sel:
+            if e[0] > cur:
+                g = e[0] - cur
+                idle += g
+                longest = max(longest, g)
+                key = (last[2] if last else "-", e[2])
+                split[key] = split.get(key, 0) + g
+                cur = e[0]
+            if e[1] > cur:
+                cur, last = e[1], e
+        queues = {}
+        for e in sel:
+            queues.setdefault(e[3], []).append(e)
+        qtxt = []
+        for q, v in sorted(queues.items()):
+            b, ce, lg = 0, w0, 0
+            for s, e_, _, _ in v:
+                if s > ce:
+                    lg = max(lg, s - ce)
+                    ce = s
+                if e_ > ce:
+                    b += e_ - ce
+                    ce = e_
+            qtxt.append("q%s %4.1f%% busy, idle <= %5.0f us (%s)" % (q, 100 * b / (w1 - w0), lg / 1e3, "+".join(sorted(set(x[2][:10] for x in v)))))
+        nox = 0
+        ce = w0
+        for s, e_, _, _ in xc[k:k + 100]:
+            if s > ce:
+                nox += s - ce
+                ce = s
+            ce = max(ce, e_)
+        print("window %2d: %.4f ms/int  no kernel at all %4.1f %% (longest %4.0f us)  no contraction running %4.1f %%" %
+              (k // 100, (w1 - w0) / 100 / 1e6, 100 * idle / (w1 - w0), longest / 1e3, 100 * nox / (w1 - w0)))
+        for t in qtxt:
+            print("      " + t)
+        for key, g in sorted(split.items(), key=lambda kv: -kv[1])[:3]:
+            print("      idle after %-24s before %-24s %6.1f us per integration" % (key[0], key[1], g / 100 / 1e3))
+
+
+if len(sys.argv) > 2 and sys.argv[1] == "--trace":
+    trace_windows(sys.argv[2], int(sys.argv[3]) if len(sys.argv) > 3 else 0)
+    sys.exit(0)
+
+import numpy as np
+
+import bench
+import caltech_bifrost_dsp_amd
+from caltech_bifrost_dsp_amd import ffi
+from caltech_bifrost_dsp_amd import ring as ringmod
+
+nint = int(sys.argv[1]) if len(sys.argv) > 1 else 2000
+nwarm = int(sys.argv[2]) if len(sys.argv) > 2 else 400
+legs = (sys.argv[3] if len(sys.argv) > 3 else "cabi,plain,slabs").split(",")
+WIN = 100
+L = ffi.lib()
+HAVE_STATS = hasattr(L, "xengRingGetWaitStats")
+
+ffi.call("xengSetDevice", 0)
+ffi.call("xengXgpuConfigure", bench.NSTAND, bench.NPOL, bench.NCHAN, bench.NTIME_GULP, bench.ACC_LEN // bench.NTIME_GULP)
+ffi.call("xengXgpuInitialize", 0)
+gulp_bytes = bench.NTIME_GULP * bench.NCHAN * bench.NINPUT
+RING = 10
+replay = ffi.DeviceBuffer(RING * gulp_bytes)
+replay.upload(np.random.RandomState(1).randint(0, 256, size=RING * gulp_bytes, dtype=np.uint8))
+
+
+def launch_waits():
+    if not hasattr(L, "xengXgpuGetLaunchWaits"):
+        return None
+    v = (ctypes.c_ulonglong * 11)()
+    ffi.call("xengXgpuGetLaunchWaits", v, 11)
+    return {"launches": v[0], "waited_for_staging": v[1], "writer_done_no_wait": v[2], "waited_for_writer_on_stream": list(v[3:5])}
+
+
+def stream_order():
+    if not hasattr(L, "xengGetStreamOrder"):
+        return None
+    p = (ctypes.c_int * 13)()
+    ffi.call("xengGetStreamOrder", 0, p, 13)
+    names = {0: "staging", 1: "map", 2: "beam", 3: "copy", 4: "mm0", 5: "mm1", 6: "mm2", 7: "mm3", 8: "consumer", 9: "mm4", 10: "mm5", 11: "mm6", 12: "mm7"}
+    return [names[k] for _, k in sorted((p[k], k) for k in range(13) if p[k])]
+
+
+def cabi_leg():
+    G, NB, NS, K = bench.ACC_LEN // bench.NTIME_GULP, 32, 24, 10
+    matbytes = bench.NCHAN * 249216 * 2 * 4
+    P = K + 3
+    outs = [ffi.DeviceBuffer(matbytes) for _ in range(P)]
+    acc = ffi.DeviceBuffer(matbytes)
+    nt_b = 2 * bench.NTIME_GULP
+    ffi.call("xengBeamformInitialize", 0, bench.NINPUT, bench.NCHAN, nt_b, NB, 0)
+    w = bench.beam_weights(0, 0xaabbccdd)
+    dw = ffi.DeviceBuffer(w.nbytes).upload(w)
+    dbeam = ffi.DeviceBuffer(bench.NCHAN * NB * nt_b * 8)
+    dpow = ffi.DeviceBuffer((NB // 2) * (nt_b // NS) * bench.NCHAN * 16)
+    SrcArray = ctypes.c_void_p * K
+    gi, bi = [0], [0]
+
+    def step(n):
+        o = outs[n % P]
+        for g in range(G):
+            ffi.check("k", L.xengXgpuKernelAsync(replay.ptr + (gi[0] % RING) * gulp_bytes, o.ptr, int(g == G - 1)))
+            gi[0] += 1
+        for _ in range(2 + (n & 1)):
+            ffi.check("run", L.xengBeamformRunVersioned(replay.ptr + ((2 * bi[0]) % (RING - 1)) * gulp_bytes, dbeam.ptr, dw.ptr, 1))
+            ffi.check("int", L.xengBeamformIntegrate(dbeam.ptr, dpow.ptr, NS))
+            bi[0] += 1
+        ffi.call("xengXgpuSyncLag", 1)
+        if n >= K and n % K == 0:
+            srcs = SrcArray(*[outs[(n - K + j) % P].ptr for j in range(K)])
+            ffi.check("sum", L.xengMapSumI32(acc.ptr, srcs, K, matbytes // 4, int(n > K)))
+        elif n % K == 1:
+            ffi.call("xengMapSync")
+    for n in range(K, K + 40):
+        step(n)
+    ffi.call("xengDeviceSynchronize")
+    n0 = 10 * K
+    t = [time.perf_counter()]
+    for n in range(n0, n0 + nint):
+        step(n)
+        if (n - n0 + 1) % WIN == 0:
+            t.append(time.perf_counter())
+    ffi.call("xengDeviceSynchronize")
+    el = time.perf_counter() - t[0]
+    ffi.call("xengBeamformDestroy")
+    wins = [round((b - a) / WIN * 1e3, 4) for a, b in zip(t, t[1:])]
+    return {"leg": "cabi_grouped", "ms_per_integration": round(el / nint * 1e3, 4), "window_ms": wins}
+
+
+def blocks_leg(from_slabs):
+    made = []
+    real_ring = ringmod.Ring
+
+    def recording_ring(*a, **kw):
+        r = real_ring(*a, **kw)
+        made.append(r)
+        return r
+    ringmod.Ring = recording_ring
+    samples, stop = [], threading.Event()
+
+    def snap():
+        s = {"t": time.perf_counter(), "launch": launch_waits()}
+        for r in list(made):
+            try:
+                c = dict(r.counters)
+                s[r.name] = {k: int(c[k]) for k in ("alloc", "reuse", "stamp_wait")}
+                if HAVE_STATS:
+                    s[r.name].update(r.wait_stats())
+            except Exception:
+                pass
+        return s
+
+    def sampler():
+        nxt = WIN
+        while not stop.wait(0.004):
+            vis = [r for r in made if r.name == "corr-output"]
+            if not vis:
+                continue
+            c = vis[0].counters
+            if c["alloc"] + c["reuse"] >= nxt:
+                s = snap()
+                s["spans"] = int(c["alloc"] + c["reuse"])
+                samples.append(s)
+                nxt = s["spans"] + WIN
+    th = threading.Thread(target=sampler, daemon=True)
+    th.start()
+    try:
+        res = bench.config5_blocks_leg(ffi, replay, gulp_bytes, RING, 0, nint=nint, nwarm=nwarm, from_slabs=from_slabs)
+    finally:
+        stop.set()
+        th.join()
+        ringmod.Ring = real_ring
+    out = {"leg": "blocks_slabs" if from_slabs else "blocks_plain", "ms_per_integration": res["ms_per_integration"], "window_ms": res["window_ms"],
+           "ring_allocations": res["ring_allocations"], "stream_order": stream_order(), "windows": []}
+
+    def delta(a, b):
+        if isinstance(b, dict):
+            return {k: delta(a.get(k), v) for k, v in b.items()} if isinstance(a, dict) else b
+        if isinstance(b, list):
+            return [delta(x, y) for x, y in zip(a, b)] if isinstance(a, list) else b
+        if isinstance(b, float):
+            return round((b - (a or 0)) * 1e6, 1)
+        return b - (a or 0) if isinstance(b, int) else b
+    for a, b in zip(samples, samples[1:]):
+        n = b["spans"] - a["spans"]
+        w = {"first_span": a["spans"], "integrations": n, "ms_per_integration": round((b["t"] - a["t"]) / n * 1e3, 4)}
+        for k in b:
+            if k not in ("t", "spans"):
+                w[k] = delta(a.get(k), b[k])
+        out["windows"].append(w)
+    return out
+
+
+def show(res):
+    print(json.dumps({k: v for k, v in res.items() if k != "windows"}), flush=True)
+    for w in res.get("windows", []):
+        if w["first_span"] < nwarm:
+            continue
+        line = "  span %5d +%3d: %.4f ms/int" % (w["first_span"], w["integrations"], w["ms_per_integration"])
+        for name in ("gpu-input", "corr-output", "bf-output", "bf-pow-output", "corr-slow-output"):
+            r = w.get(name)
+            if not r:
+                continue
+            line += " | %s a%d r%d sw%d" % (name, r["alloc"], r["reuse"], r["stamp_wait"])
+            if "stamp_wait_s" in r:
+                n = w["integrations"]
+                line += " stamp %.1f room %.1f alloc %.1f acq %s us/int" % (r["stamp_wait_s"] / n, r["room_wait_s"] / n, r["alloc_s"] / n,
+                                                                             "/".join("%.1f" % (v / n) for v in r["acquire_wait_s"][:3]))
+        if w.get("launch"):
+            lw = w["launch"]
+            line += " | launches %d staging-wait %d writer-wait %s skipped %d" % (lw["launches"], lw["waited_for_staging"], lw["waited_for_writer_on_stream"], lw["writer_done_no_wait"])
+        print(line, flush=True)
+
+
+for leg in legs:
+    if leg == "cabi":
+        show(cabi_leg())
+    elif leg in ("plain", "slabs"):
+        show(blocks_leg(leg == "slabs"))
+ffi.call("xengXgpuDestroy")
```

Measured after the change: 6574. About the same (-0.1%).
